# paninski-lab/lightning-pose

Hardware: AMD Instinct MI355X
Metric: training frames/sec (whole node), ResNet-50 384x384 17-kp semi-sup (higher is better)
Workload: dtype bf16; 1 GPU; C2/C3: ResNet-50 SemiSupervisedHeatmapTracker 384x384, K=17, 64 labeled + 128 unlabeled frames per GPU, heatmap_mse + temporal + pca_singleview + unimodal_mse, Adam (backbone lr=0 as at step 0), bf16-mixed; global_batch=192, parallelism=dp1, sync_batchnorm=False, decode_prune=plain kernels (chosen from the maps)

## Files before the change

include/lp_hip.h:

```cpp
#ifndef LP_HIP_H
#define LP_HIP_H

#include <stddef.h>
#include <stdint.h>

#ifdef __cplusplus
extern "C" {
#endif

typedef void* lp_stream_t;

int lp_config_reload_env(void);

enum {
    LP_OK = 0,
    LP_ERR_ARGUMENT = -1,
    LP_ERR_UNSUPPORTED = -2,
};

enum { LP_TF_NONE = 0, LP_TF_SINGLE = 1, LP_TF_PER_FRAME = 2, LP_TF_PER_VIEW = 3 };

#define LP_HIP_ABI_VERSION 148
int lp_version(void);
const char* lp_strerror(int code);


typedef struct lp_decode_tables {
    const int* row_base;
    const float* row_taps;
    const int* col_start;
    const float* col_taps;
    const int* colT_start;
    const float* colT_taps;
    int ty, tx, tc;
} lp_decode_tables;

typedef struct lp_frame_map {
    const float* transforms;
    int tf_mode;
    const float* bbox;
    int bbox_stride;
    int kp_per_view;
    float model_h, model_w;
} lp_frame_map;

int lp_decode_window(int downsample_factor, int n);


int lp_decode_fwd(const float* heat, int B, int K, int h, int w, int downsample_factor, float temperature,
                  const lp_decode_tables* tables, const lp_frame_map* frame_map, float* kp_aug, float* kp_frame, float* conf,
                  float* stats, int prune, lp_stream_t stream);

int lp_decode_bwd(const float* heat, int B, int K, int h, int w, int downsample_factor, float temperature,
                  const lp_decode_tables* tables, const lp_frame_map* frame_map, const float* stats, const float* g_kp_aug,
                  const float* g_kp_frame, float* g_heat, int accumulate, int prune, lp_stream_t stream);

int lp_frame_map_apply(const float* kp_in, int B, int K, const lp_frame_map* frame_map, int backward, float* kp_out,
                       lp_stream_t stream);


int lp_heatmap_gen(const float* keypoints, const int* visibility, int B, int K, int img_h, int img_w, int h, int w, float sigma,
                   float* out, lp_stream_t stream);
int lp_heatmap_gen_bwd(const float* keypoints, const int* visibility, int B, int K, int img_h, int img_w, int h, int w, float sigma,
                       const float* grad_out, float* grad_keypoints, lp_stream_t stream);

size_t lp_temporal_heatmap_workspace_bytes(int S, int K);
int lp_temporal_heatmap_fwd(int kind, const float* pred, const float* conf, int S, int K, int h, int w, const float* epsilon,
                            float prob_threshold, float* loss, void* workspace, lp_stream_t stream);
int lp_temporal_heatmap_bwd(int kind, const float* pred, int S, int K, int h, int w, const void* workspace, const float* gout,
                            float* gpred, int accumulate, lp_stream_t stream);

int lp_heatmap_confidence(const float* heat, const float* locs, int B, int K, int h, int w, int radius, float* out, lp_stream_t stream);

size_t lp_heatmap_mse_workspace_bytes(int B, int K);
int lp_heatmap_mse_fwd(const float* targ, const float* pred, int B, int K, int h, int w, float* loss, void* workspace,
                       lp_stream_t stream);
int lp_heatmap_mse_bwd(const float* targ, const float* pred, int B, int K, int h, int w, const void* workspace, const float* gout,
                       float* gpred, int accumulate, lp_stream_t stream);
enum { LP_HM_MSE = 0, LP_HM_KL = 1, LP_HM_JS = 2 };
int lp_heatmap_loss_fwd(int kind, const float* targ, const float* pred, int B, int K, int h, int w, float* loss, void* workspace,
                        lp_stream_t stream);
int lp_heatmap_loss_bwd(int kind, const float* targ, const float* pred, int B, int K, int h, int w, const void* workspace,
                        const float* gout, float* gpred, int accumulate, lp_stream_t stream);

int lp_unimodal_mse_fwd(const float* kp_aug, const float* pred, const float* conf, int S, int K, int img_h, int img_w, int h, int w,
                        float sigma, float prob_threshold, float* loss, void* workspace, lp_stream_t stream);
int lp_unimodal_mse_bwd(const float* kp_aug, const float* pred, int S, int K, int img_h, int img_w, int h, int w, float sigma,
                        const void* workspace, const float* gout, float* gpred, int accumulate, lp_stream_t stream);

int lp_softmax2d_fwd(const float* in, long stride_b, long stride_i, long stride_k, int B, int K, int n, float* out,
                     lp_stream_t stream);
int lp_softmax2d_bwd(const float* prob, const float* gprob, int B, int K, int n, void* gin_bf16, long stride_b, long stride_i,
                     long stride_k, lp_stream_t stream);


int lp_temporal_fwd_bwd(const float* kp, const float* conf, int S, int K, const float* eps_per_kp, float prob_threshold,
                        float* loss, float* grad_unit, lp_stream_t stream);

int lp_pca_fwd_bwd(const float* kp, int S, int K, const int* index, int rows, int points, const float* mean,
                   const float* kept_eigenvectors, int ncomp, float epsilon, float* loss, float* grad_unit, lp_stream_t stream);

int lp_rmse_fwd(const float* kp_targ, const float* kp_pred, int n_points, float* loss, lp_stream_t stream);
int lp_loss_combine(const float* const* x, const float* w, const float* a, int n, float* weighted, float* total, lp_stream_t stream);
int lp_loss_combine_bwd(const float* w, const float* a, int n, const float* g_weighted, const float* g_total, float* gx, lp_stream_t stream);

typedef struct lp_conv_geom {
    int B, Hi, Wi, Ci;
    int Ho, Wo, Co;
    int R, S, stride, pad;
} lp_conv_geom;

#define LP_CONV_KERNEL_IGEMM 0
#define LP_CONV_KERNEL_PIPE 1
#define LP_CONV_KERNEL_WGRAD 2
#define LP_CONV_KERNEL_WGRAD_PIPE 3
#define LP_CONV_KERNEL_PIPE_HALO 4
#define LP_CONV_KERNEL_STEM_WGRAD_NB 8
#define LP_CONV_KERNEL_WGRAD_NB 9
#define LP_CONV_KERNEL_RES2D 5
int lp_conv_last_kernel(void);

int lp_conv_fwd(const void* x, const void* w, const lp_conv_geom* geom, const float* bias, void* out_bf16, float* out_f32, int ldo,
                int n_store, lp_stream_t stream);
int lp_conv_dgrad(const void* dy, const void* wd, const lp_conv_geom* geom, const float* bias, const void* addend,
                  const void* relu_mask, void* dx_bf16, float* dx_f32, int ldo, int n_store, int skip_empty_classes,
                  lp_stream_t stream);
typedef struct lp_gemm_batch {
    int nb, nh;
    long long a_b, a_h, b_b, b_h, c_b, c_h;
} lp_gemm_batch;
int lp_gemm_nt(const void* a, int lda, const void* b, int ldb, void* c_bf16, float* c_f32, int ldc, int M, int N, int K, int n_store,
               const float* bias, const lp_gemm_batch* batch, lp_stream_t stream);
int lp_gemm_tn(const void* x, int ldx, const void* y, int ldy, void* out_bf16, int ldo, int M, int J, int N, const lp_gemm_batch* batch,
               lp_stream_t stream);
int lp_attn_fwd(const void* qkv_bf16, int ld_qkv, int k_off, int v_off, int B, int nh, int T, float scale, void* p_bf16, int ldp,
                void* out_bf16, int ldo, lp_stream_t stream);
int lp_attn_bwd_kv(const void* qkv_bf16, int ld_qkv, int v_off, const void* d_out_bf16, int ld_do, const void* p_bf16, int ldp, const float* d_rows,
                   int B, int nh, int T, float scale, void* ds_bf16, void* dqkv_bf16, int ld_dqkv, int dk_off, int dv_off, lp_stream_t stream);
int lp_attn_rowdot(const void* a_bf16, const void* b_bf16, int rows, int nh, int ld, float* out, lp_stream_t stream);
int lp_attn_dscores(const void* d_out, int ld_do, const void* v, int ldv, const void* p_bf16, const float* d_rows, int d_row_stride,
                    long long d_b, long long d_h, float scale, void* ds_bf16, int ldc, int M, int N, int K, const lp_gemm_batch* batch,
                    lp_stream_t stream);
typedef struct lp_fxsum {
    long long hi, lo;
} lp_fxsum;
int lp_gemm_nt_gelu_bwd(const void* a, const void* b, const void* u_bf16, void* c_bf16, int M, int N, int K, lp_fxsum* colsum,
                        lp_stream_t stream);
int lp_gemm_nt_gelu_fwd(const void* a, const void* b, const float* bias, void* c_bf16, void* act_bf16, int M, int N, int K,
                        lp_stream_t stream);
typedef struct lp_bn_fuse {
    const void* z;
    const float* mean;
    const float* invstd;
    const float* gamma;
    const float* beta;
    int mask_from_z;
    const void* relu_bits;
    lp_fxsum* sums;
    int seg_images;
    int addend_half;
} lp_bn_fuse;
int lp_conv_dgrad_bits(const void* dy, const void* wd, const lp_conv_geom* geom, const void* addend, const void* relu_bits, void* dx_bf16,
                       int skip_empty_classes, lp_stream_t stream);
int lp_bn_fold(const float* w, const float* gamma, const float* beta, const float* running_mean, const float* running_var, float eps,
               int Co, int per_co, void* w_bf16, float* bias, lp_stream_t stream);
int lp_conv_fwd_act(const void* x, const void* w, const lp_conv_geom* geom, const float* bias, const void* residual_bf16, int relu,
                    void* out_bf16, lp_stream_t stream);
int lp_conv_fwd_bn(const void* x, const void* w, const lp_conv_geom* geom, void* out_bf16, const lp_bn_fuse* bn, lp_stream_t stream);
int lp_stem_fwd_bn(const void* x4, const void* w, const lp_conv_geom* geom, void* out_bf16, const lp_bn_fuse* bn, lp_stream_t stream);
int lp_conv_dgrad_bn(const void* dy, const void* wd, const lp_conv_geom* geom, const void* addend, const void* relu_mask,
                     void* dx_bf16, const lp_bn_fuse* bn, lp_stream_t stream);
size_t lp_conv_wgrad_workspace_bytes(const lp_conv_geom* geom, int split_hint);
int lp_conv_wgrad(const void* x, const void* dy, const lp_conv_geom* geom, float* dw, int split_hint, void* workspace,
                  size_t workspace_bytes, lp_stream_t stream);
int lp_conv_wgrad_bias(const void* x, const void* dy, const lp_conv_geom* geom, float* dw, float* dbias, int split_hint, void* workspace,
                       size_t workspace_bytes, lp_stream_t stream);
int lp_stem_fwd(const void* x4, const void* w, const lp_conv_geom* geom, void* out_bf16, lp_stream_t stream);
int lp_stem_wgrad(const void* x4, const void* dy, const lp_conv_geom* geom, float* dw, int split_hint, void* workspace,
                  size_t workspace_bytes, lp_stream_t stream);

int lp_f32_conv_fwd(const float* x, const float* w, const lp_conv_geom* geom, int KH, int KW, int CiS, const float* bias,
                    const float* addend, float* out, lp_stream_t stream);
int lp_f32_conv_dgrad(const float* dy, const float* w, const lp_conv_geom* geom, int KH, int KW, int CiS, const float* bias,
                      const float* addend, float* dx, lp_stream_t stream);
int lp_f32_conv_wgrad(const float* x, const float* dy, const lp_conv_geom* geom, int KH, int KW, int CiS, float* dw, lp_stream_t stream);
int lp_f32_bn_stats(const float* x, int M, int C, float* sums, lp_stream_t stream);
size_t lp_f32_bn_stats_workspace_bytes(int M, int C);
int lp_f32_bn_stats_ordered(const float* x, int M, int C, float* sums, void* workspace, size_t workspace_bytes, lp_stream_t stream);
int lp_f32_bn_apply(const float* x, const float* mean, const float* invstd, const float* gamma, const float* beta, const float* residual,
                    int relu, int M, int C, float* y, lp_stream_t stream);
int lp_f32_bn_bwd_reduce(const float* dy, const float* y_out, const float* x, const float* mean, const float* invstd, int M, int C,
                         float* sums, float* dbeta_acc, float* dgamma_acc, lp_stream_t stream);
int lp_f32_bn_bwd_apply(const float* dy, const float* y_out, const float* x, const float* mean, const float* invstd, const float* gamma,
                        const float* sums, float count, int M, int C, float* dx, float* dres, lp_stream_t stream);
int lp_f32_maxpool_fwd(const float* x, int B, int Hi, int Wi, int C, float* y, void* argmax_u8, lp_stream_t stream);
int lp_f32_maxpool_bwd(const void* argmax_u8, const float* dy, int B, int Hi, int Wi, int C, float* dx, lp_stream_t stream);
int lp_f32_images_to_nhwc4(const float* images, int B, int H, int W, float* out, lp_stream_t stream);
int lp_f32_pixel_shuffle(const float* in, int B, int h, int w, int c_out, int ld, int inverse, float* out, lp_stream_t stream);
int lp_f32_softmax2d_bwd(const float* prob, const float* gprob, int B, int K, int n, float* gin, long stride_b, long stride_i, long stride_k,
                         lp_stream_t stream);
int lp_f32_vit_patchify(const float* images, int B, int H, int W, int patch, float* out, lp_stream_t stream);
int lp_f32_vit_tokens_fwd(const float* patch, const float* cls, const float* pos, int B, int Np, int D, float* x, lp_stream_t stream);
int lp_f32_vit_tokens_bwd(const float* dx, int B, int Np, int D, float* dpatch, float* dpos, lp_stream_t stream);
int lp_f32_vit_mv_tokens_fwd(const float* patch, const float* pos, const float* view, int B, int V, int Np, int D, float* x, lp_stream_t stream);
int lp_f32_vit_mv_tokens_bwd(const float* dx, int B, int V, int Np, int D, float* dpatch, float* dpos, float* dview, void* workspace,
                             size_t workspace_bytes, lp_stream_t stream);
int lp_f32_layernorm_fwd(const float* x, const float* delta, float* x_out, const float* gamma, const float* beta, float eps, int M, int D,
                         int drop_T, float* y, float* mean, float* rstd, lp_stream_t stream);
int lp_f32_layernorm_bwd(const float* dy, const float* x, const float* mean, const float* rstd, const float* gamma, int M, int D, int drop_T,
                         float* dx_acc, float* dgamma_acc, float* dbeta_acc, lp_stream_t stream);
int lp_f32_layernorm_ls_fwd(const float* x, const float* delta, const float* ls, float* x_out, const float* gamma, const float* beta, float eps,
                            int M, int D, int drop_T, float* y, float* mean, float* rstd, lp_stream_t stream);
int lp_f32_layernorm_ls_bwd(const float* dy, const float* x, const float* mean, const float* rstd, const float* gamma, const float* ls,
                            const float* branch, int M, int D, int drop_T, float* dx_acc, float* dx_out, float* dgamma_acc, float* dbeta_acc,
                            float* colsum_acc, float* dls_acc, lp_stream_t stream);
int lp_f32_gelu_fwd(const float* x, size_t n, float* y, lp_stream_t stream);
int lp_f32_gelu_bwd(const float* x, const float* dy, size_t n, float* dx, lp_stream_t stream);
int lp_f32_attn_fwd(const float* qkv, int ld, int k_off, int v_off, int B, int nh, int T, float scale, float* p, float* o, int ldo,
                    lp_stream_t stream);
int lp_f32_attn_bwd(const float* qkv, int ld, int k_off, int v_off, const float* dout, int ldo, const float* p, int B, int nh, int T,
                    float scale, float* ds_workspace, float* dqkv, int ldd, lp_stream_t stream);

size_t lp_bn_reduce_workspace_bytes(int M, int C);
int lp_bn_stats(const void* x, int M, int C, lp_fxsum* sums, void* workspace, size_t workspace_bytes, lp_stream_t stream);
int lp_fxsum_accumulate(const lp_fxsum* sums, int n, float* dst, lp_stream_t stream);
int lp_bn_finalize(const lp_fxsum* sums, float count, int C, float eps, float momentum, float* mean, float* invstd,
                   float* running_mean, float* running_var, lp_stream_t stream);
int lp_bn_finalize_f32(const float* sums, float count, int C, float eps, float momentum, float* mean, float* invstd,
                       float* running_mean, float* running_var, lp_stream_t stream);
int lp_bn_finalize2(const lp_fxsum* sums, float count0, float count1, int C, float eps, float momentum, float* mean, float* invstd,
                    float* running_mean, float* running_var, lp_stream_t stream);
int lp_bn_apply(const void* x, const float* mean, const float* invstd, const float* gamma, const float* beta, const void* residual,
                int relu, int M, int C, void* y, void* relu_bits, lp_stream_t stream);
int lp_bn_apply_seg(const void* x, const float* mean, const float* invstd, const float* gamma, const float* beta, const void* residual,
                    int relu, int M, int C, int seg_rows, void* y, void* relu_bits, lp_stream_t stream);
int lp_bn_apply_seg_lo(const void* x, const float* mean, const float* invstd, const float* gamma, const float* beta, const void* residual,
                       const void* residual_lo, const void* zd, const float* mean_d, const float* invstd_d, const float* gamma_d,
                       const float* beta_d, int relu, int M, int C, int seg_rows, void* y, void* y_lo, void* relu_bits, lp_stream_t stream);
int lp_bn_apply_seg_rbn(const void* x, const float* mean, const float* invstd, const float* gamma, const float* beta, const void* zd,
                        const float* mean_d, const float* invstd_d, const float* gamma_d, const float* beta_d, int relu, int M, int C,
                        int seg_rows, void* y, void* relu_bits, lp_stream_t stream);
int lp_bn_bwd_reduce(const void* dy, const void* y_out, const void* x, const float* mean, const float* invstd, int M, int C,
                     lp_fxsum* sums, void* workspace, size_t workspace_bytes, lp_stream_t stream);
int lp_bn_bwd_apply(const void* dy, const void* y_out, const void* x, const float* mean, const float* invstd, const float* gamma,
                    const lp_fxsum* sums, float count, int M, int C, void* dx, void* dres, const lp_fxsum* sums_local, float* dbeta_acc,
                    float* dgamma_acc, float* terms_ws, lp_stream_t stream);
int lp_bn_bwd_apply_seg(const void* dy, const void* y_out, const void* x, const float* mean, const float* invstd, const float* gamma,
                        const lp_fxsum* sums, float count0, float count1, int M, int C, int seg_rows, void* dx, void* dres,
                        const lp_fxsum* sums_local, float* dbeta_acc, float* dgamma_acc, float* terms_ws, lp_stream_t stream);
size_t lp_bn_bwd_ds_workspace_bytes(int M, int C);
int lp_bn_bwd_apply_seg_ds(const void* dy, const void* y_out, const void* x, const float* mean, const float* invstd, const float* gamma,
                           const lp_fxsum* sums, float count0, float count1, int M, int C, int seg_rows, void* dx, void* dres,
                           const lp_fxsum* sums_local, float* dbeta_acc, float* dgamma_acc, float* terms_ws, const void* zd,
                           const float* mean_d, const float* invstd_d, lp_fxsum* sums_d, void* workspace, size_t workspace_bytes,
                           lp_stream_t stream);
int lp_maxpool_fwd(const void* x, int B, int Hi, int Wi, int C, void* y, void* argmax_u8, lp_stream_t stream);
int lp_maxpool_bwd(const void* argmax_u8, const void* dy, int B, int Hi, int Wi, int C, void* dx, lp_stream_t stream);
int lp_bn_relu_maxpool_fwd(const void* z, const float* mean, const float* invstd, const float* gamma, const float* beta, int B, int Hi, int Wi,
                           int C, void* y, void* argmax_u8, lp_stream_t stream);
int lp_bn_pool_bwd_reduce(const void* argmax_u8, const void* dy, const void* z, const float* mean, const float* invstd, const float* gamma,
                          const float* beta, int B, int Hi, int Wi, int C, lp_fxsum* sums, lp_stream_t stream);
int lp_bn_pool_bwd_apply(const void* argmax_u8, const void* dy, const void* z, const float* mean, const float* invstd, const float* gamma,
                         const float* beta, const lp_fxsum* sums, float count, int B, int Hi, int Wi, int C, void* dx,
                         const lp_fxsum* sums_local, float* dbeta_acc, float* dgamma_acc, lp_stream_t stream);
int lp_images_to_nhwc4(const float* images_nchw, int B, int H, int W, void* out_bf16, lp_stream_t stream);
int lp_pixel_shuffle(const void* in, int B, int h, int w, int c_out, int ld, int inverse, void* out, lp_stream_t stream);

int lp_vit_patchify(const float* images_nchw, int B, int H, int W, int patch, void* out_bf16, lp_stream_t stream);
int lp_vit_tokens_fwd(const void* patch_bf16, const float* cls, const float* pos, int B, int Np, int D, float* x, lp_stream_t stream);
int lp_vit_tokens_bwd(const float* dx, int B, int Np, int D, void* dpatch_bf16, float* dpos, lp_stream_t stream);
int lp_vit_mv_tokens_fwd(const void* patch_bf16, const float* pos, const float* view, int B, int V, int Np, int D, float* x,
                         lp_stream_t stream);
size_t lp_vit_mv_tokens_bwd_workspace_bytes(int B, int V, int Np, int D);
int lp_vit_mv_tokens_bwd(const float* dx, int B, int V, int Np, int D, void* dpatch_bf16, float* dpos, float* dview, void* workspace,
                         size_t workspace_bytes, lp_stream_t stream);
#define LP_CAM_MAX_VIEWS 32
size_t lp_cam_chain_workspace_bytes(int B, int V, int K);
int lp_cam_chain_fwd(const float* points, const float* intrinsics, const float* extrinsics, const float* dist12, const float* bbox, float model_h,
                     float model_w, int B, int V, int K, float* p3d, float* p2d, lp_stream_t stream);
int lp_cam_chain_bwd(const float* points, const float* intrinsics, const float* extrinsics, const float* dist12, const float* bbox, float model_h,
                     float model_w, int B, int V, int K, const float* p3d, const float* g3d, const float* g2d, void* workspace,
                     size_t workspace_bytes, float* gpoints, lp_stream_t stream);
int lp_cam_project_fwd(const float* points_3d, const float* intrinsics, const float* extrinsics, const float* dist12, const float* bbox,
                       float model_h, float model_w, int B, int V, int K, float* p2d, lp_stream_t stream);
int lp_cam_project_bwd(const float* points_3d, const float* intrinsics, const float* extrinsics, const float* dist12, const float* bbox,
                       float model_h, float model_w, int B, int V, int K, const float* g2d, float* g3d, lp_stream_t stream);
int lp_cam_pairwise_fwd_bwd(const float* targ_3d, const float* pred_3d, int B, int P, int K, float* loss, float* grad_unit, lp_stream_t stream);
int lp_small_matmul(const float* w, const float* x, int R, int Q, int D, int transpose_w, int accumulate, float* y, lp_stream_t stream);
int lp_layernorm_fwd(const float* x, const void* delta_bf16, float* x_out, const float* gamma, const float* beta, float eps, int M,
                     int D, int drop_T, void* y_bf16, float* mean, float* rstd, lp_stream_t stream);
int lp_layernorm_bwd(const void* dy_bf16, const float* x, const float* mean, const float* rstd, const float* gamma, int M, int D,
                     int drop_T, float* dx_acc, float* dgamma_acc, float* dbeta_acc, lp_stream_t stream);
int lp_layernorm_bwd_bf16(const void* dy_bf16, const float* x, const float* mean, const float* rstd, const float* gamma, int M, int D,
                          int drop_T, float* dx_acc, void* dx_bf16, float* dgamma_acc, float* dbeta_acc, lp_stream_t stream);
int lp_gelu_fwd(const void* x_bf16, size_t n, void* y_bf16, lp_stream_t stream);
int lp_gelu_bwd(const void* x_bf16, const void* dy_bf16, size_t n, void* dx_bf16, lp_stream_t stream);
int lp_gelu_bwd_colsum(const void* x_bf16, const void* dy_bf16, int rows, int cols, void* dx_bf16, float* colsum_acc, lp_stream_t stream);
int lp_layernorm_bwd_bf16_colsum(const void* dy_bf16, const float* x, const float* mean, const float* rstd, const float* gamma, int M, int D,
                                 int drop_T, float* dx_acc, void* dx_bf16, float* dgamma_acc, float* dbeta_acc, float* colsum_acc,
                                 lp_stream_t stream);
int lp_layernorm_ls_fwd(const float* x, const void* delta_bf16, const float* ls, float* x_out, const float* gamma, const float* beta, float eps,
                        int M, int D, int drop_T, void* y_bf16, float* mean, float* rstd, lp_stream_t stream);
int lp_layernorm_ls_bwd(const void* dy_bf16, const float* x, const float* mean, const float* rstd, const float* gamma, const float* ls,
                        const void* branch_bf16, int M, int D, int drop_T, float* dx_acc, void* dx_bf16, float* dgamma_acc, float* dbeta_acc,
                        float* colsum_acc, float* dls_acc, lp_stream_t stream);
int lp_softmax_rows_fwd(void* s_bf16, int rows, int n, int ld, float scale, lp_stream_t stream);
int lp_softmax_rows_bwd(const void* p_bf16, void* dp_bf16, int rows, int n, int ld, float scale, lp_stream_t stream);
int lp_transpose_batched(const void* in_bf16, int R, int Cc, int ldi, long long in_b, long long in_h, void* out_bf16, int ldo,
                         long long out_b, long long out_h, int nb, int nh, lp_stream_t stream);

enum { LP_BORDER_RENORM = 0,
       LP_BORDER_CLAMP = 1    };

typedef struct lp_frame_norm {
    float mean[3], std[3];
} lp_frame_norm;

typedef struct lp_frame_augment {
    int has_matrix;
    float matrix[6];
    float brightness, contrast, contrast_center;
    float shot_factor;
    unsigned long long seed;
} lp_frame_augment;

int lp_frames_resize(const void* src_u8, int S, int Hs, int Ws, long long frame_stride, int row_stride, int H, int W, int border,
                     const lp_frame_norm* finish_norm, float* dst, lp_stream_t stream);
int lp_frames_resize_cubic(const void* src_u8, int S, int Hs, int Ws, long long frame_stride, int row_stride, int H, int W, int round_u8,
                           const lp_frame_norm* finish_norm, float* dst, lp_stream_t stream);
int lp_frames_augment(const float* src_hwc, int S, int H, int W, const lp_frame_augment* aug, const lp_frame_norm* norm,
                      float* dst_nchw, lp_stream_t stream);
int lp_labeled_keypoints(const float* kp_src, const float* src_hw, const float* affine, const int* hflip, const int* swap,
                         const int* vis_in, int uniform_heatmaps, int B, int K, int H, int W, float* kp_out, int* vis_out,
                         lp_stream_t stream);

enum { LP_AUG_GEOM = 1, LP_AUG_BLUR = 2, LP_AUG_DROPOUT = 4, LP_AUG_DROP_PER_CHANNEL = 8, LP_AUG_SALT = 16, LP_AUG_PEPPER = 32,
       LP_AUG_ELASTIC = 64, LP_AUG_HISTEQ = 128, LP_AUG_CLAHE = 256, LP_AUG_EMBOSS = 512, LP_AUG_CROPPAD = 1024, LP_AUG_HFLIP = 2048 };
enum { LP_AUG_OP_DROPOUT = 0, LP_AUG_OP_SALT = 1, LP_AUG_OP_PEPPER = 2, LP_AUG_OP_ELASTIC = 3 };
enum { LP_AUG_LOCAL_BLUR_COARSE = 0, LP_AUG_LOCAL_EMBOSS = 1 };
#define LP_AUG_ELASTIC_MAX_RADIUS 20

typedef struct lp_labelaug_image {
    int flags;
    int image_id;
    float geom[6];
    float blur[25];
    float emboss[9];
    int coarse_gh[3], coarse_gw[3];
    unsigned coarse_thr[3];
    float elastic_alpha;
    int clahe_clip, clahe_tiles_y, clahe_tiles_x, clahe_slot;
    int pad[4];
} lp_labelaug_image;

int lp_labelaug_geom(const void* src_u8, int B, int H, int W, const lp_labelaug_image* params, void* dst_u8, lp_stream_t stream);
int lp_labelaug_local(const void* src_u8, int B, int H, int W, const lp_labelaug_image* params, int which, const void* salt_lut,
                      unsigned long long seed, void* dst_u8, lp_stream_t stream);
int lp_labelaug_elastic_field(int B, int H, int W, const lp_labelaug_image* params, float sigma, unsigned long long seed, float* tmp,
                              float* field, lp_stream_t stream);
int lp_labelaug_elastic_apply(const void* src_u8, int B, int H, int W, const lp_labelaug_image* params, const float* field, void* dst_u8,
                              lp_stream_t stream);
int lp_labelaug_histeq(const void* src_u8, int B, int H, int W, const lp_labelaug_image* params, unsigned* ws, void* lut_out, void* dst_u8,
                       lp_stream_t stream);
int lp_labelaug_clahe(const void* src_u8, int B, int H, int W, const lp_labelaug_image* params, const int* slot_image, int n_slots,
                      int max_ty, int max_tx, void* luts, void* dst_u8, lp_stream_t stream);
int lp_labelaug_finish(const void* src_u8, int B, int Hs, int Ws, const lp_labelaug_image* params, int H, int W, const lp_frame_norm* norm,
                       float* dst, lp_stream_t stream);
int lp_labelaug_keypoints(const float* kp, int B, int K, const float* affine, const lp_labelaug_image* params, const float* field, int H,
                          int W, float* kp_out, lp_stream_t stream);

int lp_patch_mask_f32(const float* images, int BV, int C, int H, int W, int patch, int count, unsigned long long key, const float* mask_in,
                      float* out, float* mask_out, lp_stream_t stream);

#define LP_MV3D_MAX_VIEWS 8
#define LP_MV3D_MAX_KEYPOINTS 128
int lp_mv3d_plan(const float* kp, const float* src_hw, const float* bbox, const float* intrinsics, const float* extrinsics,
                 const float* dist12, const float* draws, int augment, float shift_param, int H, int W, int B, int V, int K, float* kp3d,
                 float* kp2d, float* affine, int* status, lp_stream_t stream);
int lp_mv3d_fill(const void* src_u8, int B, int Hs, int Ws, const lp_frame_norm* norm, float* fill, lp_stream_t stream);
int lp_mv3d_finish(const void* src_u8, int B, int Hs, int Ws, const float* affine, const float* fill, const lp_frame_norm* norm, int V,
                   int v, int H, int W, float* dst, lp_stream_t stream);

int lp_adam_step(float* params, const float* grads, float* exp_avg, float* exp_avg_sq, size_t n, float lr, float beta1, float beta2,
                 float eps, float weight_decay, int decoupled, int step, float grad_scale, void* params_bf16, lp_stream_t stream);
int lp_cast_bf16(const float* src, size_t n, void* dst, lp_stream_t stream);
int lp_permute_cba(const void* src, int A, int B, int C, void* dst, lp_stream_t stream);

#ifdef __cplusplus
}
#endif
#endif
```

lightning-pose_amd/_lib.py:

```python

from __future__ import annotations

import ctypes as C
import os

_HERE = os.path.dirname(os.path.abspath(__file__))
LIB_PATH = os.environ.get("LP_HIP_LIB") or os.path.join(_HERE, "liblp_hip.so")


class LpHipUnavailable(RuntimeError):
    """liblp_hip.so could not be loaded, or an op was given a non-ROCm tensor.  There is no fallback path."""


class LpHipError(RuntimeError):
    pass


class DecodeTables(C.Structure):
    _fields_ = [("row_base", C.c_void_p), ("row_taps", C.c_void_p), ("col_start", C.c_void_p),
                ("col_taps", C.c_void_p), ("colT_start", C.c_void_p), ("colT_taps", C.c_void_p),
                ("ty", C.c_int), ("tx", C.c_int), ("tc", C.c_int)]


class FrameMap(C.Structure):
    _fields_ = [("transforms", C.c_void_p), ("tf_mode", C.c_int), ("bbox", C.c_void_p), ("bbox_stride", C.c_int),
                ("kp_per_view", C.c_int), ("model_h", C.c_float), ("model_w", C.c_float)]


class ConvGeom(C.Structure):
    _fields_ = [(n, C.c_int) for n in ("B", "Hi", "Wi", "Ci", "Ho", "Wo", "Co", "R", "S", "stride", "pad")]


class BnFuse(C.Structure):
    _fields_ = [("z", C.c_void_p), ("mean", C.c_void_p), ("invstd", C.c_void_p), ("gamma", C.c_void_p), ("beta", C.c_void_p),
                ("mask_from_z", C.c_int), ("relu_bits", C.c_void_p), ("sums", C.c_void_p), ("seg_images", C.c_int), ("addend_half", C.c_int)]


class FrameNorm(C.Structure):
    _fields_ = [("mean", C.c_float * 3), ("std", C.c_float * 3)]


class FrameAugment(C.Structure):
    _fields_ = [("has_matrix", C.c_int), ("matrix", C.c_float * 6), ("brightness", C.c_float), ("contrast", C.c_float),
                ("contrast_center", C.c_float), ("shot_factor", C.c_float), ("seed", C.c_ulonglong)]


class GemmBatch(C.Structure):
    _fields_ = [("nb", C.c_int), ("nh", C.c_int)] + [(n, C.c_longlong) for n in ("a_b", "a_h", "b_b", "b_h", "c_b", "c_h")]


HM_MSE, HM_KL, HM_JS = 0, 1, 2
(CONV_KERNEL_IGEMM, CONV_KERNEL_PIPE, CONV_KERNEL_WGRAD, CONV_KERNEL_WGRAD_PIPE, CONV_KERNEL_PIPE_HALO, CONV_KERNEL_RES2D, _CONV_KERNEL_6,
 _CONV_KERNEL_7, CONV_KERNEL_STEM_WGRAD_NB, CONV_KERNEL_WGRAD_NB) = range(10)
CONV_KERNEL_LABEL = {
    CONV_KERNEL_PIPE: (("conv_igemm_kernel", "conv_pipe_kernel"),),
    CONV_KERNEL_PIPE_HALO: (("conv_igemm_kernel", "conv_pipe_kernel"), (">", ",halo>")),
    CONV_KERNEL_RES2D: (("conv_igemm_kernel<64,", "conv_res2d_kernel<"), ("conv_igemm_kernel<64>", "conv_res2d_kernel<fwd>")),
    CONV_KERNEL_WGRAD_PIPE: (("conv_wgrad_kernel", "conv_wgrad_pipe_kernel"),),
    CONV_KERNEL_WGRAD_NB: (("conv_wgrad_kernel", "conv_wgrad_nb_kernel"),),
}
BORDER_RENORM, BORDER_CLAMP = 0, 1
AUG_GEOM, AUG_BLUR, AUG_DROPOUT, AUG_DROP_PER_CHANNEL, AUG_SALT, AUG_PEPPER = 1, 2, 4, 8, 16, 32
AUG_ELASTIC, AUG_HISTEQ, AUG_CLAHE, AUG_EMBOSS, AUG_CROPPAD, AUG_HFLIP = 64, 128, 256, 512, 1024, 2048
AUG_OP_DROPOUT, AUG_OP_SALT, AUG_OP_PEPPER, AUG_OP_ELASTIC = 0, 1, 2, 3
AUG_LOCAL_BLUR_COARSE, AUG_LOCAL_EMBOSS = 0, 1
AUG_ELASTIC_MAX_RADIUS = 20
TF_NONE, TF_SINGLE, TF_PER_FRAME, TF_PER_VIEW = 0, 1, 2, 3

ABI_VERSION = 148

_P, _I, _F, _L, _Z = C.c_void_p, C.c_int, C.c_float, C.c_long, C.c_size_t

PROTOTYPES = {
    "lp_version": (_I, []),
    "lp_strerror": (C.c_char_p, [_I]),
    "lp_config_reload_env": (_I, []),
    "lp_decode_window": (_I, [_I, _I]),
    "lp_decode_fwd": (_I, [_P, _I, _I, _I, _I, _I, _F, C.POINTER(DecodeTables), C.POINTER(FrameMap), _P, _P, _P, _P, _I, _P]),
    "lp_decode_bwd": (_I, [_P, _I, _I, _I, _I, _I, _F, C.POINTER(DecodeTables), C.POINTER(FrameMap), _P, _P, _P, _P, _I, _I, _P]),
    "lp_frame_map_apply": (_I, [_P, _I, _I, C.POINTER(FrameMap), _I, _P, _P]),
    "lp_heatmap_gen": (_I, [_P, _P, _I, _I, _I, _I, _I, _I, _F, _P, _P]),
    "lp_heatmap_gen_bwd": (_I, [_P, _P, _I, _I, _I, _I, _I, _I, _F, _P, _P, _P]),
    "lp_temporal_heatmap_workspace_bytes": (_Z, [_I, _I]),
    "lp_temporal_heatmap_fwd": (_I, [_I, _P, _P, _I, _I, _I, _I, _P, _F, _P, _P, _P]),
    "lp_temporal_heatmap_bwd": (_I, [_I, _P, _I, _I, _I, _I, _P, _P, _P, _I, _P]),
    "lp_heatmap_confidence": (_I, [_P, _P, _I, _I, _I, _I, _I, _P, _P]),
    "lp_heatmap_mse_workspace_bytes": (_Z, [_I, _I]),
    "lp_heatmap_mse_fwd": (_I, [_P, _P, _I, _I, _I, _I, _P, _P, _P]),
    "lp_heatmap_mse_bwd": (_I, [_P, _P, _I, _I, _I, _I, _P, _P, _P, _I, _P]),
    "lp_heatmap_loss_fwd": (_I, [_I, _P, _P, _I, _I, _I, _I, _P, _P, _P]),
    "lp_heatmap_loss_bwd": (_I, [_I, _P, _P, _I, _I, _I, _I, _P, _P, _P, _I, _P]),
    "lp_unimodal_mse_fwd": (_I, [_P, _P, _P, _I, _I, _I, _I, _I, _I, _F, _F, _P, _P, _P]),
    "lp_unimodal_mse_bwd": (_I, [_P, _P, _I, _I, _I, _I, _I, _I, _F, _P, _P, _P, _I, _P]),
    "lp_softmax2d_fwd": (_I, [_P, _L, _L, _L, _I, _I, _I, _P, _P]),
    "lp_softmax2d_bwd": (_I, [_P, _P, _I, _I, _I, _P, _L, _L, _L, _P]),
    "lp_temporal_fwd_bwd": (_I, [_P, _P, _I, _I, _P, _F, _P, _P, _P]),
    "lp_pca_fwd_bwd": (_I, [_P, _I, _I, _P, _I, _I, _P, _P, _I, _F, _P, _P, _P]),
    "lp_rmse_fwd": (_I, [_P, _P, _I, _P, _P]),
    "lp_loss_combine": (_I, [_P, _P, _P, _I, _P, _P, _P]),
    "lp_loss_combine_bwd": (_I, [_P, _P, _I, _P, _P, _P, _P]),
    "lp_conv_fwd": (_I, [_P, _P, C.POINTER(ConvGeom), _P, _P, _P, _I, _I, _P]),
    "lp_conv_dgrad": (_I, [_P, _P, C.POINTER(ConvGeom), _P, _P, _P, _P, _P, _I, _I, _I, _P]),
    "lp_conv_dgrad_bits": (_I, [_P, _P, C.POINTER(ConvGeom), _P, _P, _P, _I, _P]),
    "lp_gemm_nt": (_I, [_P, _I, _P, _I, _P, _P, _I, _I, _I, _I, _I, _P, C.POINTER(GemmBatch), _P]),
    "lp_gemm_nt_gelu_bwd": (_I, [_P, _P, _P, _P, _I, _I, _I, _P, _P]),
    "lp_gemm_nt_gelu_fwd": (_I, [_P, _P, _P, _P, _P, _I, _I, _I, _P]),
    "lp_gemm_tn": (_I, [_P, _I, _P, _I, _P, _I, _I, _I, _I, C.POINTER(GemmBatch), _P]),
    "lp_attn_fwd": (_I, [_P, _I, _I, _I, _I, _I, _I, C.c_float, _P, _I, _P, _I, _P]),
    "lp_attn_bwd_kv": (_I, [_P, _I, _I, _P, _I, _P, _I, _P, _I, _I, _I, C.c_float, _P, _P, _I, _I, _I, _P]),
    "lp_attn_rowdot": (_I, [_P, _P, _I, _I, _I, _P, _P]),
    "lp_attn_dscores": (_I, [_P, _I, _P, _I, _P, _P, _I, C.c_longlong, C.c_longlong, C.c_float, _P, _I, _I, _I, _I, C.POINTER(GemmBatch), _P]),
    "lp_conv_fwd_bn": (_I, [_P, _P, C.POINTER(ConvGeom), _P, C.POINTER(BnFuse), _P]),
    "lp_conv_last_kernel": (_I, []),
    "lp_stem_fwd_bn": (_I, [_P, _P, C.POINTER(ConvGeom), _P, C.POINTER(BnFuse), _P]),
    "lp_conv_dgrad_bn": (_I, [_P, _P, C.POINTER(ConvGeom), _P, _P, _P, C.POINTER(BnFuse), _P]),
    "lp_bn_fold": (_I, [_P, _P, _P, _P, _P, _F, _I, _I, _P, _P, _P]),
    "lp_conv_fwd_act": (_I, [_P, _P, C.POINTER(ConvGeom), _P, _P, _I, _P, _P]),
    "lp_conv_wgrad_workspace_bytes": (_Z, [C.POINTER(ConvGeom), _I]),
    "lp_conv_wgrad": (_I, [_P, _P, C.POINTER(ConvGeom), _P, _I, _P, _Z, _P]),
    "lp_conv_wgrad_bias": (_I, [_P, _P, C.POINTER(ConvGeom), _P, _P, _I, _P, C.c_size_t, _P]),
    "lp_stem_fwd": (_I, [_P, _P, C.POINTER(ConvGeom), _P, _P]),
    "lp_stem_wgrad": (_I, [_P, _P, C.POINTER(ConvGeom), _P, _I, _P, _Z, _P]),
    "lp_bn_reduce_workspace_bytes": (_Z, [_I, _I]),
    "lp_bn_stats": (_I, [_P, _I, _I, _P, _P, _Z, _P]),
    "lp_bn_finalize": (_I, [_P, _F, _I, _F, _F, _P, _P, _P, _P, _P]),
    "lp_fxsum_accumulate": (_I, [_P, _I, _P, _P]),
    "lp_bn_finalize_f32": (_I, [_P, _F, _I, _F, _F, _P, _P, _P, _P, _P]),
    "lp_bn_finalize2": (_I, [_P, _F, _F, _I, _F, _F, _P, _P, _P, _P, _P]),
    "lp_bn_apply": (_I, [_P, _P, _P, _P, _P, _P, _I, _I, _I, _P, _P, _P]),
    "lp_bn_apply_seg": (_I, [_P, _P, _P, _P, _P, _P, _I, _I, _I, _I, _P, _P, _P]),
    "lp_bn_apply_seg_lo": (_I, [_P, _P, _P, _P, _P, _P, _P, _P, _P, _P, _P, _P, _I, _I, _I, _I, _P, _P, _P, _P]),
    "lp_bn_apply_seg_rbn": (_I, [_P, _P, _P, _P, _P, _P, _P, _P, _P, _P, _I, _I, _I, _I, _P, _P, _P]),
    "lp_bn_bwd_apply_seg": (_I, [_P, _P, _P, _P, _P, _P, _P, _F, _F, _I, _I, _I, _P, _P, _P, _P, _P, _P, _P]),
    "lp_bn_bwd_ds_workspace_bytes": (_Z, [_I, _I]),
    "lp_bn_bwd_apply_seg_ds": (_I, [_P, _P, _P, _P, _P, _P, _P, _F, _F, _I, _I, _I, _P, _P, _P, _P, _P, _P, _P, _P, _P, _P, _P, _Z, _P]),
    "lp_bn_bwd_reduce": (_I, [_P, _P, _P, _P, _P, _I, _I, _P, _P, _Z, _P]),
    "lp_bn_bwd_apply": (_I, [_P, _P, _P, _P, _P, _P, _P, _F, _I, _I, _P, _P, _P, _P, _P, _P, _P]),
    "lp_maxpool_fwd": (_I, [_P, _I, _I, _I, _I, _P, _P, _P]),
    "lp_maxpool_bwd": (_I, [_P, _P, _I, _I, _I, _I, _P, _P]),
    "lp_bn_relu_maxpool_fwd": (_I, [_P, _P, _P, _P, _P, _I, _I, _I, _I, _P, _P, _P]),
    "lp_bn_pool_bwd_reduce": (_I, [_P, _P, _P, _P, _P, _P, _P, _I, _I, _I, _I, _P, _P]),
    "lp_bn_pool_bwd_apply": (_I, [_P, _P, _P, _P, _P, _P, _P, _P, C.c_float, _I, _I, _I, _I, _P, _P, _P, _P, _P]),
    "lp_images_to_nhwc4": (_I, [_P, _I, _I, _I, _P, _P]),
    "lp_pixel_shuffle": (_I, [_P, _I, _I, _I, _I, _I, _I, _P, _P]),
    "lp_vit_patchify": (_I, [_P, _I, _I, _I, _I, _P, _P]),
    "lp_vit_tokens_fwd": (_I, [_P, _P, _P, _I, _I, _I, _P, _P]),
    "lp_vit_tokens_bwd": (_I, [_P, _I, _I, _I, _P, _P, _P]),
    "lp_vit_mv_tokens_fwd": (_I, [_P, _P, _P, _I, _I, _I, _I, _P, _P]),
    "lp_vit_mv_tokens_bwd_workspace_bytes": (_Z, [_I, _I, _I, _I]),
    "lp_vit_mv_tokens_bwd": (_I, [_P, _I, _I, _I, _I, _P, _P, _P, _P, _Z, _P]),
    "lp_cam_chain_workspace_bytes": (_Z, [_I, _I, _I]),
    "lp_cam_chain_fwd": (_I, [_P, _P, _P, _P, _P, _F, _F, _I, _I, _I, _P, _P, _P]),
    "lp_cam_chain_bwd": (_I, [_P, _P, _P, _P, _P, _F, _F, _I, _I, _I, _P, _P, _P, _P, _Z, _P, _P]),
    "lp_cam_project_fwd": (_I, [_P, _P, _P, _P, _P, _F, _F, _I, _I, _I, _P, _P]),
    "lp_cam_project_bwd": (_I, [_P, _P, _P, _P, _P, _F, _F, _I, _I, _I, _P, _P, _P]),
    "lp_cam_pairwise_fwd_bwd": (_I, [_P, _P, _I, _I, _I, _P, _P, _P]),
    "lp_small_matmul": (_I, [_P, _P, _I, _I, _I, _I, _I, _P, _P]),
    "lp_layernorm_fwd": (_I, [_P, _P, _P, _P, _P, _F, _I, _I, _I, _P, _P, _P, _P]),
    "lp_layernorm_bwd": (_I, [_P, _P, _P, _P, _P, _I, _I, _I, _P, _P, _P, _P]),
    "lp_layernorm_bwd_bf16": (_I, [_P, _P, _P, _P, _P, _I, _I, _I, _P, _P, _P, _P, _P]),
    "lp_gelu_fwd": (_I, [_P, _Z, _P, _P]),
    "lp_gelu_bwd": (_I, [_P, _P, _Z, _P, _P]),
    "lp_gelu_bwd_colsum": (_I, [_P, _P, _I, _I, _P, _P, _P]),
    "lp_layernorm_bwd_bf16_colsum": (_I, [_P, _P, _P, _P, _P, _I, _I, _I, _P, _P, _P, _P, _P, _P]),
    "lp_layernorm_ls_fwd": (_I, [_P, _P, _P, _P, _P, _P, _F, _I, _I, _I, _P, _P, _P, _P]),
    "lp_layernorm_ls_bwd": (_I, [_P, _P, _P, _P, _P, _P, _P, _I, _I, _I, _P, _P, _P, _P, _P, _P, _P]),
    "lp_softmax_rows_fwd": (_I, [_P, _I, _I, _I, _F, _P]),
    "lp_softmax_rows_bwd": (_I, [_P, _P, _I, _I, _I, _F, _P]),
    "lp_transpose_batched": (_I, [_P, _I, _I, _I, C.c_longlong, C.c_longlong, _P, _I, C.c_longlong, C.c_longlong, _I, _I, _P]),
    "lp_frames_resize": (_I, [_P, _I, _I, _I, C.c_longlong, _I, _I, _I, _I, C.POINTER(FrameNorm), _P, _P]),
    "lp_frames_resize_cubic": (_I, [_P, _I, _I, _I, C.c_longlong, _I, _I, _I, _I, C.POINTER(FrameNorm), _P, _P]),
    "lp_frames_augment": (_I, [_P, _I, _I, _I, C.POINTER(FrameAugment), C.POINTER(FrameNorm), _P, _P]),
    "lp_labeled_keypoints": (_I, [_P, _P, _P, _P, _P, _P, _I, _I, _I, _I, _I, _P, _P, _P]),
    "lp_labelaug_geom": (_I, [_P, _I, _I, _I, _P, _P, _P]),
    "lp_labelaug_local": (_I, [_P, _I, _I, _I, _P, _I, _P, C.c_ulonglong, _P, _P]),
    "lp_labelaug_elastic_field": (_I, [_I, _I, _I, _P, _F, C.c_ulonglong, _P, _P, _P]),
    "lp_labelaug_elastic_apply": (_I, [_P, _I, _I, _I, _P, _P, _P, _P]),
    "lp_labelaug_histeq": (_I, [_P, _I, _I, _I, _P, _P, _P, _P, _P]),
    "lp_labelaug_clahe": (_I, [_P, _I, _I, _I, _P, _P, _I, _I, _I, _P, _P, _P]),
    "lp_labelaug_finish": (_I, [_P, _I, _I, _I, _P, _I, _I, C.POINTER(FrameNorm), _P, _P]),
    "lp_labelaug_keypoints": (_I, [_P, _I, _I, _P, _P, _P, _I, _I, _P, _P]),
    "lp_patch_mask_f32": (_I, [_P, _I, _I, _I, _I, _I, _I, C.c_ulonglong, _P, _P, _P, _P]),
    "lp_mv3d_plan": (_I, [_P, _P, _P, _P, _P, _P, _P, _I, _F, _I, _I, _I, _I, _I, _P, _P, _P, _P, _P]),
    "lp_mv3d_fill": (_I, [_P, _I, _I, _I, C.POINTER(FrameNorm), _P, _P]),
    "lp_mv3d_finish": (_I, [_P, _I, _I, _I, _P, _P, C.POINTER(FrameNorm), _I, _I, _I, _I, _P, _P]),
    "lp_f32_conv_fwd": (_I, [_P, _P, C.POINTER(ConvGeom), _I, _I, _I, _P, _P, _P, _P]),
    "lp_f32_conv_dgrad": (_I, [_P, _P, C.POINTER(ConvGeom), _I, _I, _I, _P, _P, _P, _P]),
    "lp_f32_conv_wgrad": (_I, [_P, _P, C.POINTER(ConvGeom), _I, _I, _I, _P, _P]),
    "lp_f32_bn_stats": (_I, [_P, _I, _I, _P, _P]),
    "lp_f32_bn_stats_workspace_bytes": (C.c_size_t, [_I, _I]),
    "lp_f32_bn_stats_ordered": (_I, [_P, _I, _I, _P, _P, C.c_size_t, _P]),
    "lp_f32_bn_apply": (_I, [_P, _P, _P, _P, _P, _P, _I, _I, _I, _P, _P]),
    "lp_f32_bn_bwd_reduce": (_I, [_P, _P, _P, _P, _P, _I, _I, _P, _P, _P, _P]),
    "lp_f32_bn_bwd_apply": (_I, [_P, _P, _P, _P, _P, _P, _P, _F, _I, _I, _P, _P, _P]),
    "lp_f32_maxpool_fwd": (_I, [_P, _I, _I, _I, _I, _P, _P, _P]),
    "lp_f32_maxpool_bwd": (_I, [_P, _P, _I, _I, _I, _I, _P, _P]),
    "lp_f32_images_to_nhwc4": (_I, [_P, _I, _I, _I, _P, _P]),
    "lp_f32_pixel_shuffle": (_I, [_P, _I, _I, _I, _I, _I, _I, _P, _P]),
    "lp_f32_softmax2d_bwd": (_I, [_P, _P, _I, _I, _I, _P, _L, _L, _L, _P]),
    "lp_f32_vit_patchify": (_I, [_P, _I, _I, _I, _I, _P, _P]),
    "lp_f32_vit_tokens_fwd": (_I, [_P, _P, _P, _I, _I, _I, _P, _P]),
    "lp_f32_vit_tokens_bwd": (_I, [_P, _I, _I, _I, _P, _P, _P]),
    "lp_f32_vit_mv_tokens_fwd": (_I, [_P, _P, _P, _I, _I, _I, _I, _P, _P]),
    "lp_f32_vit_mv_tokens_bwd": (_I, [_P, _I, _I, _I, _I, _P, _P, _P, _P, _Z, _P]),
    "lp_f32_layernorm_fwd": (_I, [_P, _P, _P, _P, _P, _F, _I, _I, _I, _P, _P, _P, _P]),
    "lp_f32_layernorm_bwd": (_I, [_P, _P, _P, _P, _P, _I, _I, _I, _P, _P, _P, _P]),
    "lp_f32_layernorm_ls_fwd": (_I, [_P, _P, _P, _P, _P, _P, _F, _I, _I, _I, _P, _P, _P, _P]),
    "lp_f32_layernorm_ls_bwd": (_I, [_P, _P, _P, _P, _P, _P, _P, _I, _I, _I, _P, _P, _P, _P, _P, _P, _P]),
    "lp_f32_gelu_fwd": (_I, [_P, _Z, _P, _P]),
    "lp_f32_gelu_bwd": (_I, [_P, _P, _Z, _P, _P]),
    "lp_f32_attn_fwd": (_I, [_P, _I, _I, _I, _I, _I, _I, _F, _P, _P, _I, _P]),
    "lp_f32_attn_bwd": (_I, [_P, _I, _I, _I, _P, _I, _P, _I, _I, _I, _F, _P, _P, _I, _P]),
    "lp_adam_step": (_I, [_P, _P, _P, _P, _Z, _F, _F, _F, _F, _F, _I, _I, _F, _P, _P]),
    "lp_cast_bf16": (_I, [_P, _Z, _P, _P]),
    "lp_permute_cba": (_I, [_P, _I, _I, _I, _P, _P]),
}


def declare(lib: C.CDLL) -> C.CDLL:
    for name, (res, args) in PROTOTYPES.items():
        fn = getattr(lib, name)
        fn.restype = res
        fn.argtypes = args
    have = int(lib.lp_version())
    if have != ABI_VERSION:
        raise LpHipUnavailable(f"{getattr(lib, '_name', 'liblp_hip.so')} was built for ABI {have}, this package binds ABI {ABI_VERSION} "
                               "(include/lp_hip.h: LP_HIP_ABI_VERSION) - rebuild it: python -c 'import __graft_entry__ as g; g.build()'")
    return lib


_lib = None


def lib() -> C.CDLL:
    global _lib
    if _lib is None:
        if not os.path.exists(LIB_PATH):
            raise LpHipUnavailable(
                f"{LIB_PATH} not found - build it with `python -c 'import __graft_entry__ as g; g.build()'` "
                "(lightning-pose_amd/csrc/build.sh).  lightning_pose_amd has no CPU fallback.")
        try:
            _lib = declare(C.CDLL(LIB_PATH))
        except OSError as e:
            raise LpHipUnavailable(f"cannot load {LIB_PATH}: {e}") from e
    return _lib


def check(code: int, what: str) -> None:
    if code == 0:
        return
    msg = lib().lp_strerror(code).decode()
    if code == -1:
        raise ValueError(f"{what}: {msg}")
    if code == -2:
        raise NotImplementedError(f"{what}: {msg}")
    raise LpHipError(f"{what}: HIP error {code}: {msg}")
```

lightning-pose_amd/csrc/api.hip:

```cpp
#include "lp_common.h"

#include <stdlib.h>

#include <atomic>

extern "C" int lp_version(void) { return LP_HIP_ABI_VERSION; }

namespace lp {
static int env_int(const char* name, int dflt) {
    const char* e = getenv(name);
    return (e == nullptr || *e == 0) ? dflt : atoi(e);
}
static LpSwitches read_switches() {
    LpSwitches s;
    s.conv_pipe = env_int("LP_CONV_PIPE", 1);
    s.conv_halo = env_int("LP_CONV_HALO", 1);
    s.conv_res2d = env_int("LP_CONV_RES2D", 1);
    s.infer_pipe = env_int("LP_INFER_PIPE", 1);
    s.gemm_pipe = env_int("LP_GEMM_PIPE", 1);
    s.wgrad_pipe = env_int("LP_WGRAD_PIPE", 1);
    s.wgrad_nb = env_int("LP_WGRAD_NB", 1);
    s.stem_2d = env_int("LP_STEM_2D", 1);
    s.stem_wgrad_nb = env_int("LP_STEM_WGRAD_NB", 1);
    s.pool_v2 = env_int("LP_POOL_V2", 1);
    s.bn_bwd_wgs_per_cu = env_int("LP_BN_BWD_WGS_PER_CU", 5);
    if (s.bn_bwd_wgs_per_cu < 1 || s.bn_bwd_wgs_per_cu > 5) s.bn_bwd_wgs_per_cu = 5;
    s.conv_max_wgs = env_int("LP_CONV_MAX_WGS", 0);
    return s;
}
static std::atomic<const LpSwitches*> g_switches{new LpSwitches(read_switches())};
const LpSwitches& lp_switches() { return *g_switches.load(std::memory_order_acquire); }
}

extern "C" int lp_config_reload_env(void) {
    lp::g_switches.store(new lp::LpSwitches(lp::read_switches()), std::memory_order_release);
    return LP_OK;
}

extern "C" const char* lp_strerror(int code) {
    if (code == LP_OK) return "ok";
    if (code == LP_ERR_ARGUMENT) return "invalid argument (null pointer or non-positive dimension)";
    if (code == LP_ERR_UNSUPPORTED) return "shape not covered by the instantiated kernels";
    if (code > 0) return hipGetErrorString((hipError_t)code);
    return "unknown lp_hip error";
}
```

lightning-pose_amd/csrc/conv.hip:

```cpp
#include <stdlib.h>

#include "lp_common.h"

namespace lp {

constexpr int kBM = 128;
constexpr int kBK = 64;
constexpr int kLD = kBK + 8;

struct ConvGeom {
    int B, Hi, Wi, Ci;
    int Ho, Wo, Co;
    int R, S, stride, pad;
};

struct ConvEpilogue {
    unsigned short* out_bf16;
    float* out_f32;
    int ldo;
    int n_store;
    const float* bias;
    const unsigned short* addend;
    const unsigned short* relu_mask;
    const unsigned char* relu_bits;
// ... 620 lines not shown
    unsigned voffA = ~0u, voffB[RB];
    if (fast) {
        const int p0 = m_begin + pgA * 4;
        const int pc = p0 < M ? p0 : 0;
        const int rem = pc - fdiv(pc, div_hw) * hw;
        fho = fdiv(rem, div_wo);
        fwo = rem - fho * g.Wo;
        if (jv) voffA = (unsigned)((p0 + (tr - g.pad) * g.Wi + (ts - g.pad)) * pitch_x + tcn) * 2u + zx;
        lo_h = max(0, g.pad - tr);
        span_h = min(g.Ho, g.Hi + g.pad - tr) - lo_h;
        lo_w = max(0, g.pad - ts);
        span_w = min(g.Wo, g.Wi + g.pad - ts) - lo_w;
#pragma unroll
        for (int i = 0; i < RB; ++i) voffB[i] = nv ? (unsigned)((m_begin + pgB * RB + i) * pitch_y + nB) * 2u + zy : ~0u;
    }
    const unsigned jinv = jv ? 0u : ~0u;

    auto load_fast = [&](auto nm_c, int mk, u16x8 (&ra)[4], u16x8 (&rb)[RB]) {
        constexpr bool NM = decltype(nm_c)::value;
        const unsigned step = (unsigned)(mk - m_begin);
        const unsigned soffA = step * ci2, soffB = step * (unsigned)pitch_y * 2u;
        if (NM) {
            const bool ragged = mk + kBK > m_end;
#pragma unroll
            for (int i = 0; i < 4; ++i) {
                const unsigned rinv = (ragged && mk + pgA * 4 + i >= m_end) ? ~0u : 0u;
                ra[i] = buf_load16(rsrc_x, (voffA + i * ci2) | jinv | rinv, soffA);
            }
#pragma unroll
            for (int i = 0; i < RB; ++i) {
                const unsigned rinv = (ragged && mk + pgB * RB + i >= m_end) ? ~0u : 0u;
                rb[i] = buf_load16(rsrc_dy, voffB[i] | rinv, soffB);
            }
        } else {
#pragma unroll
            for (int i = 0; i < 4; ++i) {
                int wo = fwo + i, ho = fho;
                if (wo >= g.Wo) {
                    wo -= g.Wo;
                    ho = (ho + 1 == g.Ho) ? 0 : ho + 1;
                }
                const bool ok = (unsigned)(ho - lo_h) < (unsigned)span_h && (unsigned)(wo - lo_w) < (unsigned)span_w;
                ra[i] = buf_load16(rsrc_x, (voffA + soffA + i * ci2) | (ok ? 0u : ~0u) | jinv, 0u);
            }
            fwo += rw;
            fho += qw;
            if (fwo >= g.Wo) {
                fwo -= g.Wo;
                ++fho;
            }
            if (fho >= g.Ho) fho -= g.Ho;
            if (fho >= g.Ho) fho -= g.Ho;
#pragma unroll
            for (int i = 0; i < RB; ++i) rb[i] = buf_load16(rsrc_dy, voffB[i], soffB);
        }
    };

    auto load_generic = [&](int mk, u16x8 (&ra)[4], u16x8 (&rb)[RB]) {
#pragma unroll
        for (int i = 0; i < 4; ++i) {
            const int m = mk + pgA * 4 + i;
            bool ok = jv && m < m_end;
            const int mm = ok ? m : 0;
            const int b = fdiv(mm, div_hw), rem = mm - b * hw;
            const int ho = fdiv(rem, div_wo), wo = rem - ho * g.Wo;
            const int hi = ho * g.stride - g.pad + tr, wi = wo * g.stride - g.pad + ts;
            if (STEM) {
                const bool okr = ok && tr < g.R && hi >= 0 && hi < g.Hi;
                const size_t base = ((size_t)(b * g.Hi + hi) * g.Wi + wi) * 4;
                ra[i] = load4x2(X + base, okr && wi >= 0 && wi < g.Wi, X + base + 4, okr && ts + 1 < g.S && wi + 1 >= 0 && wi + 1 < g.Wi);
            } else {
                ok = ok && hi >= 0 && hi < g.Hi && wi >= 0 && wi < g.Wi;
                ra[i] = ok ? load8(X + ((size_t)(b * g.Hi + hi) * g.Wi + wi) * g.Ci + tcn) : zero8();
            }
        }
#pragma unroll
        for (int i = 0; i < RB; ++i) {
            const int m = mk + pgB * RB + i;
            rb[i] = (nv && m < m_end) ? load8(DY + (size_t)m * g.Co + nB) : zero8();
        }
    };
    auto load_step = [&](int mk) {
        if (fast && (direct || mk + kBK <= m_end)) {
            if (nomask) load_fast(std::true_type{}, mk, ra, rb);
            else load_fast(std::false_type{}, mk, ra, rb);
        } else load_generic(mk, ra, rb);
    };
    auto store_step = [&](int buf, const u16x8 (&ra)[4], const u16x8 (&rb)[RB]) {
#pragma unroll
        for (int i = 0; i < 4; ++i) *reinterpret_cast<u16x8*>(&sA[buf][(pgA * 4 + i) * LDA + jc * 8]) = ra[i];
#pragma unroll
        for (int i = 0; i < RB; ++i) *reinterpret_cast<u16x8*>(&sB[buf][(pgB * RB + i) * LDB + nc * 8]) = rb[i];
        if (want_cs) {
#pragma unroll
            for (int i = 0; i < RB; ++i)
#pragma unroll
                for (int q = 0; q < 8; ++q) cs[q] += bf16_to_f32(rb[i][q]);
        }
    };

    const int fq = lane >> 4, fi = lane & 15;
    const int frow = (fq >> 1) * 8 + (fi >> 2), fcol = (fq & 1) * 16 + (fi & 3) * 4;
    auto frag = [&](const unsigned short* tile_, int ld, int ch0, int kk) -> bf16x8 {
        const unsigned short* p = tile_ + (kk * 16 + frow) * ld + ch0 + fcol;
        const s16x4_t lo = lds_read_tr16(p), hi = lds_read_tr16(p + 4 * ld);
        typedef __attribute__((ext_vector_type(8))) short s16x8_t;
        const s16x8_t v = {lo[0], lo[1], lo[2], lo[3], hi[0], hi[1], hi[2], hi[3]};
        return __builtin_bit_cast(bf16x8, v);
    };
    auto mma_step = [&](int buf) {
        bf16x8 a[2][2], b[2][NT];
        auto fetch = [&](int kk, int set) {
#pragma unroll
            for (int mt = 0; mt < 2; ++mt) a[set][mt] = frag(sA[buf], LDA, wm * 64 + mt * 32, kk);
#pragma unroll
            for (int nt = 0; nt < NT; ++nt) b[set][nt] = frag(sB[buf], LDB, wn * (NT * 32) + nt * 32, kk);
        };
        fetch(0, 0);
#pragma unroll
        for (int kk = 0; kk < kBK / 16; ++kk) {
            if (kk + 1 < kBK / 16) fetch(kk + 1, (kk + 1) & 1);
            __builtin_amdgcn_sched_barrier(0);
#pragma unroll
            for (int mt = 0; mt < 2; ++mt)
#pragma unroll
                for (int nt = 0; nt < NT; ++nt)
                    acc[mt][nt] = __builtin_amdgcn_mfma_f32_32x32x16_bf16(a[kk & 1][mt], b[kk & 1][nt], acc[mt][nt], 0, 0, 0);
            __builtin_amdgcn_sched_barrier(0);
        }
    };

    const int KT = (m_end - m_begin + kBK - 1) / kBK;
    const bool deep = kWgradDeep && fast && KT >= 2 && (direct || (m_end - m_begin) % kBK == 0);
    auto deep_loop = [&](auto nm) {
        load_fast(nm, m_begin, ra, rb);
        load_fast(nm, m_begin + kBK, ra2, rb2);
        store_step(0, ra, rb);
        __syncthreads();
        int kt = 0;
        for (; kt + 3 < KT; kt += 2) {
            load_fast(nm, m_begin + (kt + 2) * kBK, ra, rb);
            mma_step(0);
            store_step(1, ra2, rb2);
            __syncthreads();
            load_fast(nm, m_begin + (kt + 3) * kBK, ra2, rb2);
            mma_step(1);
            store_step(0, ra, rb);
            __syncthreads();
        }
        const bool three = kt + 2 < KT;
        if (three) load_fast(nm, m_begin + (kt + 2) * kBK, ra, rb);
        mma_step(0);
        store_step(1, ra2, rb2);
        __syncthreads();
        mma_step(1);
        if (three) {
            store_step(0, ra, rb);
            __syncthreads();
            mma_step(0);
        }
        __syncthreads();
    };
    if (deep) {
        if (nomask) deep_loop(std::true_type{});
        else deep_loop(std::false_type{});
    } else if (KT > 0) {
        load_step(m_begin);
        store_step(0, ra, rb);
        __syncthreads();
        for (int kt = 0; kt < KT; ++kt) {
            const int cur = kt & 1;
            if (kt + 1 < KT) load_step(m_begin + (kt + 1) * kBK);
            mma_step(cur);
            if (kt + 1 < KT) store_step(cur ^ 1, ra, rb);
            __syncthreads();
        }
    }

    if (want_cs) {
        float* red = reinterpret_cast<float*>(&sA[0][0]);
#pragma unroll
        for (int q = 0; q < 8; ++q) red[pgB * BN + nc * 8 + q] = cs[q];
        __syncthreads();
        if (tid < BN && n0 + tid < g.Co) {
            float t = 0.f;
            for (int r = 0; r < 256 / NCH; ++r) t += red[r * BN + tid];
            atomicAdd(&tn.col_sums[n0 + tid], t);
        }
    }
    if (direct) {
        const int col = lane & 31, rg = lane >> 5;
#pragma unroll
        for (int mt = 0; mt < 2; ++mt)
#pragma unroll
            for (int nt = 0; nt < NT; ++nt) {
                const int n = n0 + wn * (NT * 32) + nt * 32 + col;
#pragma unroll
                for (int e = 0; e < 16; ++e) {
                    const int jr = j0 + wm * 64 + mt * 32 + (e & 3) + 8 * (e >> 2) + 4 * rg;
                    if (jr < Kw && n < g.Co) tn.out[zo + (size_t)jr * tn.ldo + n] = f32_to_bf16(acc[mt][nt][e]);
                }
            }
        return;
    }
    float* dst = ws + ((((size_t)slice * tiles + tile) * 4 + wave) * (2 * NT * 16)) * 64 + lane;
#pragma unroll
    for (int mt = 0; mt < 2; ++mt)
#pragma unroll
        for (int nt = 0; nt < NT; ++nt)
#pragma unroll
            for (int e = 0; e < 16; ++e) dst[((mt * NT + nt) * 16 + e) * 64] = acc[mt][nt][e];
}

template <int BN>
__global__ __launch_bounds__(256) void wgrad_reduce_kernel(const float* __restrict__ ws, int slices, int tiles, int tiles_n, int Kw,
                                                           int Co, float* __restrict__ dW) {
    constexpr int NT = BN / 64;
    constexpr int PER_TILE = 4 * 2 * NT * 16 * 64;
    const size_t total = (size_t)tiles * PER_TILE;
    for (size_t i = (size_t)blockIdx.x * 256 + threadIdx.x; i < total; i += (size_t)gridDim.x * 256) {
        float sum = 0.f;
        for (int sl = 0; sl < slices; ++sl) sum += ws[(size_t)sl * total + i];
        const int lane = (int)(i & 63);
        size_t t = i >> 6;
        const int e = (int)(t & 15);
        t >>= 4;
        const int nt = (int)(t % NT);
        t /= NT;
        const int mt = (int)(t & 1);
        t >>= 1;
        const int wave = (int)(t & 3);
        const int tile = (int)(t >> 2);
        const int wm = wave >> 1, wn = wave & 1;
        const int j = (tile / tiles_n) * kBM + wm * 64 + mt * 32 + (e & 3) + 8 * (e >> 2) + 4 * (lane >> 5);
        const int n = (tile % tiles_n) * BN + wn * (NT * 32) + nt * 32 + (lane & 31);
        if (j < Kw && n < Co) dW[(size_t)n * Kw + j] += sum;
    }
}

template <int BN>
__global__ __launch_bounds__(256) void wgrad_reduce_sliced_kernel(const float* __restrict__ ws, int slices, int tiles, int tiles_n,
                                                                  int Kw, int Co, float* __restrict__ dW) {
    constexpr int NT = BN / 64;
    constexpr int PER_TILE = 4 * 2 * NT * 16 * 64;
    __shared__ float part[4][64];
    const size_t total = (size_t)tiles * PER_TILE;
    const int lane = threadIdx.x & 63, w = threadIdx.x >> 6;
    const size_t i = (size_t)blockIdx.x * 64 + lane;
    float s0 = 0.f, s1 = 0.f, s2 = 0.f, s3 = 0.f;
    int sl = w;
    for (; sl + 12 < slices; sl += 16) {
        s0 += ws[(size_t)sl * total + i];
        s1 += ws[(size_t)(sl + 4) * total + i];
        s2 += ws[(size_t)(sl + 8) * total + i];
        s3 += ws[(size_t)(sl + 12) * total + i];
    }
    for (; sl < slices; sl += 4) s0 += ws[(size_t)sl * total + i];
    part[w][lane] = (s0 + s1) + (s2 + s3);
    __syncthreads();
    if (w == 0) {
        const float sum = (part[0][lane] + part[1][lane]) + (part[2][lane] + part[3][lane]);
        size_t t = i >> 6;
        const int e = (int)(t & 15);
        t >>= 4;
        const int nt = (int)(t % NT);
        t /= NT;
        const int mt = (int)(t & 1);
        t >>= 1;
        const int wave = (int)(t & 3);
        const int tile = (int)(t >> 2);
        const int wm = wave >> 1, wn = wave & 1;
        const int j = (tile / tiles_n) * kBM + wm * 64 + mt * 32 + (e & 3) + 8 * (e >> 2) + 4 * (lane >> 5);
        const int n = (tile % tiles_n) * BN + wn * (NT * 32) + nt * 32 + (lane & 31);
        if (j < Kw && n < Co) dW[(size_t)n * Kw + j] += sum;
    }
}

template <int BN>
static void launch_wgrad_reduce(const float* ws, int slices, int tiles, int tiles_n, int Kw, int Co, float* dw, hipStream_t st) {
    constexpr int PER_TILE = 4 * 2 * (BN / 64) * 16 * 64;
    if (slices >= 16) {
        hipLaunchKernelGGL((wgrad_reduce_sliced_kernel<BN>), dim3(tiles * (PER_TILE / 64)), dim3(256), 0, st, ws, slices, tiles, tiles_n, Kw,
                           Co, dw);
    } else {
        const int blocks = tiles * (PER_TILE / 256);
        hipLaunchKernelGGL((wgrad_reduce_kernel<BN>), dim3(blocks < 4096 ? blocks : 4096), dim3(256), 0, st, ws, slices, tiles, tiles_n, Kw,
                           Co, dw);
    }
}

static long long seg_split_rows(int seg_images, int B, long long rows_per_image, long long M) {
    if (seg_images <= 0) return M;
    if (seg_images >= B) return -1;
    const long long r = (long long)seg_images * rows_per_image;
    return (r % kBM == 0) ? r : -1;
}

static void bn_fuse_begin(ConvEpilogue& ep, const lp_bn_fuse* bn) {
    ep.stats_sums = bn->sums;
    ep.seg_images = bn->seg_images;
}

static thread_local int g_last_conv_kernel = LP_CONV_KERNEL_IGEMM;

struct ConvRoute {
    int kernel;
    int bn;
    int mode;
    int ek;
};
constexpr int kNoKernel = -1;

struct ConvProblem {
    int mode;
    int ek;
    const void *x, *w;
    ConvGeom g;
    Lattice lat;
    int M, N, K;
    long long seg_rows;
    ConvEpilogue ep;
    int LpSwitches::*gate;
    bool dense;
    bool igemm_form;
    int igemm_cols;
    bool gemm;
    GemmExt gx;
    int nz;
    unsigned x_bytes, w_bytes;
};

static int conv_ck(const ConvProblem& p) { return p.mode == kModeDgrad ? p.g.Co : p.g.Ci; }

static bool pipe_shape_ok(const ConvEpilogue& ep, int M, int N, int K, int ck, long long seg_rows, bool bias_ok) {
    if (ep.out_bf16 == nullptr || ep.out_f32 != nullptr || (ep.bias != nullptr && !bias_ok) || ep.ldo != N || ep.n_store != N) return false;
    if (K <= 0 || ck % kBK != 0 || N % (N > 64 ? 128 : 64) != 0 || M <= 0) return false;
    if (ep.seg_images > 0 && seg_rows % kPM != 0) return false;
    return true;
}

static int pipe_dgrad_kind(const ConvEpilogue& ep) {
    if (ep.bn_z != nullptr) {
        if (ep.stats_sums == nullptr || ep.relu_mask != nullptr) return -1;
        if (ep.mask_from_z && !ep.addend && !ep.relu_bits) return kEkZ;
        if (!ep.mask_from_z && ep.addend && ep.relu_bits) return kEkAZB;
        return -1;
    }
    if (ep.stats_sums != nullptr) return -1;
    if (ep.relu_bits != nullptr) return ep.relu_mask == nullptr ? kEkPB : -1;
    return kEkPlain;
}

static bool halo_shape_ok(const ConvGeom& g, int M, int ck, int cap_rows) {
    if (g.R != 3 || g.S != 3 || g.stride != 1 || g.pad != 1 || g.Hi != g.Ho || g.Wi != g.Wo || ck % kBK != 0) return false;
    struct Memo { int B, H, W, cap; bool ok; };
    static thread_local Memo memo[8];
    static thread_local int memo_n = 0;
    for (int i = 0; i < memo_n; ++i)
        if (memo[i].B == g.B && memo[i].H == g.Hi && memo[i].W == g.Wi && memo[i].cap == cap_rows) return memo[i].ok;
    const long long W = g.Wi, H = g.Hi, Wp = W + 2;
    auto padded = [&](long long m) {
        const long long r = m / W, b = r / H;
        return (r + 1 + 2 * b) * Wp + (m - r * W) + 1;
    };
    bool ok = true;
    for (long long m0 = 0; m0 < M && ok; m0 += kPM) {
        const long long last = m0 + kPM - 1 < M ? m0 + kPM - 1 : M - 1;
        ok = padded(last) - padded(m0) + 2 * (W + 3) + 1 <= cap_rows;
    }
    if (memo_n < 8) memo[memo_n++] = Memo{g.B, g.Hi, g.Wi, cap_rows, ok};
    return ok;
}

static bool res2d_shape_ok(const ConvGeom& g, int ck, int N) {
    return g.R == 3 && g.S == 3 && g.stride == 1 && g.pad == 1 && g.Hi == g.Ho && g.Wi == g.Wo && ck == 64 && N == 64 && g.Hi % 16 == 0 &&
           g.Wi % 16 == 0;
}

static bool stem2d_shape_ok(const ConvGeom& g) { return g.Ho % 16 == 0 && g.Wo % 16 == 0 && g.Hi == 2 * g.Ho && g.Wi == 2 * g.Wo; }

static bool admits_pipe(const ConvProblem& p) {
    if (p.ek < 0 || !p.dense) return false;
    if (p.ek == kEkAZB && !(p.lat.hstep == 1 && p.lat.wstep == 1)) return false;
    if ((p.ek == kEkGeluFwd || p.ek == kEkGeluBwd) && p.N % 128 != 0) return false;
    return pipe_shape_ok(p.ep, p.M, p.N, p.K, conv_ck(p), p.seg_rows, p.mode != kModeDgrad);
}

static bool admits_halo(const ConvProblem& p) {
    return (p.ek == kEkNone || p.ek == kEkInfer || p.ek == kEkZ) && halo_shape_ok(p.g, p.M, conv_ck(p), p.N > 64 ? 384 : 512);
}

static bool admits_res2d(const ConvProblem& p) {
    if (!res2d_shape_ok(p.g, conv_ck(p), p.N)) return false;
    if (p.mode == kModeInfer) return p.ep.addend == nullptr;
    return (p.ek == kEkNone || p.ek == kEkZ) && p.ep.bias == nullptr && admits_pipe(p);
}

static ConvRoute route_conv(const ConvProblem& p, const LpSwitches& sw) {
    const bool pipe = sw.conv_pipe != 0 && (p.gate == nullptr || sw.*p.gate != 0);
    if (p.mode == kModeStem) return ConvRoute{pipe && stem2d_shape_ok(p.g) ? LP_CONV_KERNEL_RES2D : LP_CONV_KERNEL_IGEMM, 64, p.mode, p.ek};
    if (pipe && sw.conv_res2d != 0 && admits_res2d(p)) return ConvRoute{LP_CONV_KERNEL_RES2D, 64, p.mode, p.ek};
    if (pipe && admits_pipe(p))
        return ConvRoute{sw.conv_halo != 0 && admits_halo(p) ? LP_CONV_KERNEL_PIPE_HALO : LP_CONV_KERNEL_PIPE, p.N > 64 ? 128 : 64, p.mode, p.ek};
    return ConvRoute{p.igemm_form ? LP_CONV_KERNEL_IGEMM : kNoKernel, p.igemm_cols > 64 ? 128 : 64, p.mode, p.ek};
}

static int conv_max_wgs(int per_cu) {
    if (lp_switches().conv_max_wgs > 0) return lp_switches().conv_max_wgs;
    static int cus = [] {
        int dev = 0, c = 0;
        if (hipGetDevice(&dev) != hipSuccess || hipDeviceGetAttribute(&c, hipDeviceAttributeMultiprocessorCount, dev) != hipSuccess || c <= 0) c = 256;
        return c;
    }();
    return per_cu * cus;
}

template <int BN, int MODE>
static void launch_igemm(const ConvProblem& p, hipStream_t st) {
    const ConvGeom& g = p.g;
    const int tm = (p.M + kBM - 1) / kBM, tn = (p.N + BN - 1) / BN, per_z = tm * tn, ntiles = per_z * p.nz;
    const int grid = ntiles < conv_max_wgs(2) ? ntiles : conv_max_wgs(2);
    const int ck = MODE == kModeDgrad ? g.Co : g.Ci;
    unsigned x_bytes = (unsigned)(2ull * (MODE == kModeDgrad ? (size_t)g.B * g.Ho * g.Wo * g.Co : (size_t)g.B * g.Hi * g.Wi * g.Ci));
    unsigned w_bytes = (unsigned)(2ull * (size_t)p.N * (MODE == kModeStem ? (size_t)p.K : (size_t)g.R * g.S * ck));
    GemmExt gx{ck, MODE == kModeStem ? p.K : g.R * g.S * ck, 1, per_z, 0u, 0u, 0u, 0u, 0u, 0u};
    if (p.gemm) {
        gx = p.gx;
        gx.tiles_per_z = per_z;
        x_bytes = p.x_bytes;
        w_bytes = p.w_bytes;
    }
    hipLaunchKernelGGL((conv_igemm_kernel<BN, MODE>), dim3(grid), dim3(256), 0, st, (const unsigned short*)p.x, (const unsigned short*)p.w,
                       x_bytes, w_bytes, g, p.lat, gx, make_fastdiv(p.lat.nh * p.lat.nw), make_fastdiv(p.lat.nw), p.M, p.N, p.K, tn, ntiles, p.ep);
}

template <int MODE, bool INFER = false>
static void launch_res2d(const ConvProblem& p, hipStream_t st) {
    const ConvGeom& g = p.g;
    const int ntiles = g.B * (g.Hi / 16) * (g.Wi / 16);
    const int grid = ntiles < conv_max_wgs(1) ? ntiles : conv_max_wgs(1);
    const unsigned x_bytes = (unsigned)(2ull * g.B * g.Hi * g.Wi * 64), w_bytes = (unsigned)(2ull * 64 * 9 * 64);
    hipLaunchKernelGGL((conv_res2d_kernel<MODE, INFER>), dim3(grid), dim3(512), 0, st, (const unsigned short*)p.x, (const unsigned short*)p.w, x_bytes,
                       w_bytes, g.B, g.Hi, g.Wi, ntiles, p.ep);
}

static void launch_stem2d(const ConvProblem& p, hipStream_t st) {
    const ConvGeom& g = p.g;
    const int ntiles = g.B * (g.Ho / 16) * (g.Wo / 16);
    const int grid = ntiles < 2 * conv_max_wgs(1) ? ntiles : 2 * conv_max_wgs(1);
    hipLaunchKernelGGL(conv_stem2d_kernel, dim3(grid), dim3(512), 0, st, (const unsigned short*)p.x, (const unsigned short*)p.w,
                       (unsigned)(2ull * g.B * g.Hi * g.Wi * 4), g.B, g.Ho, g.Wo, ntiles, p.ep);
}

template <int BN, int MODE, int EK, bool HALO = false>
static void launch_pipe(const ConvProblem& p, hipStream_t st) {
    const ConvGeom& g = p.g;
    const int tm = (p.M + kPM - 1) / kPM, tn = p.N / BN, ntiles = tm * tn;
    const int grid = ntiles < conv_max_wgs(1) ? ntiles : conv_max_wgs(1);
    const int ck = MODE == kModeDgrad ? g.Co : g.Ci;
    const unsigned x_bytes = (unsigned)(2ull * (MODE == kModeDgrad ? (size_t)g.B * g.Ho * g.Wo * g.Co : (size_t)g.B * g.Hi * g.Wi * g.Ci));
    const unsigned w_bytes = (unsigned)(2ull * (size_t)p.N * g.R * g.S * ck);
    const HaloDivs hd{make_fastdiv(g.Hi), make_fastdiv(g.Wi + 2), make_fastdiv(g.Hi + 2)};
    hipLaunchKernelGGL((conv_pipe_kernel<BN, MODE, EK, HALO>), dim3(grid), dim3(512), 0, st, (const unsigned short*)p.x, (const unsigned short*)p.w,
                       x_bytes, w_bytes, g, p.lat, make_fastdiv(p.lat.nh * p.lat.nw), make_fastdiv(p.lat.nw), p.M, p.N, p.K, tn, ntiles, p.ep, hd);
}

template <int BN>
static void launch_conv_bn(const ConvRoute& r, const ConvProblem& p, hipStream_t st) {
    if (r.kernel == LP_CONV_KERNEL_IGEMM) {
        switch (r.mode) {
            case kModeFwd: return launch_igemm<BN, kModeFwd>(p, st);
            case kModeDgrad: return launch_igemm<BN, kModeDgrad>(p, st);
            case kModeInfer: return launch_igemm<BN, kModeInfer>(p, st);
            default: return launch_igemm<BN, kModeAttn>(p, st);
        }
    }
    const bool halo = r.kernel == LP_CONV_KERNEL_PIPE_HALO;
    switch (r.ek) {
        case kEkNone: return halo ? launch_pipe<BN, kModeFwd, kEkNone, true>(p, st) : launch_pipe<BN, kModeFwd, kEkNone>(p, st);
        case kEkInfer: return halo ? launch_pipe<BN, kModeFwd, kEkInfer, true>(p, st) : launch_pipe<BN, kModeFwd, kEkInfer>(p, st);
        case kEkZ: return halo ? launch_pipe<BN, kModeDgrad, kEkZ, true>(p, st) : launch_pipe<BN, kModeDgrad, kEkZ>(p, st);
        case kEkAZB: return launch_pipe<BN, kModeDgrad, kEkAZB>(p, st);
        case kEkPB: return launch_pipe<BN, kModeDgrad, kEkPB>(p, st);
        default: return launch_pipe<BN, kModeDgrad, kEkPlain>(p, st);
    }
}

static void launch_conv(const ConvRoute& r, const ConvProblem& p, hipStream_t st) {
    g_last_conv_kernel = r.kernel;
    if (r.kernel == LP_CONV_KERNEL_RES2D) {
        switch (r.mode) {
            case kModeStem: return launch_stem2d(p, st);
            case kModeInfer: return launch_res2d<kModeFwd, true>(p, st);
            case kModeDgrad: return launch_res2d<kModeDgrad>(p, st);
            default: return launch_res2d<kModeFwd>(p, st);
        }
    }
    if (r.mode == kModeStem) return launch_igemm<64, kModeStem>(p, st);
    if (r.ek == kEkGeluFwd) return launch_pipe<128, kModeFwd, kEkGeluFwd>(p, st);
    if (r.ek == kEkGeluBwd) return launch_pipe<128, kModeFwd, kEkGeluBwd>(p, st);
    if (r.bn == 128) launch_conv_bn<128>(r, p, st);
    else launch_conv_bn<64>(r, p, st);
}

static int run_conv(const ConvProblem& p, lp_stream_t stream) {
    const ConvRoute r = route_conv(p, lp_switches());
    if (r.kernel == kNoKernel) return LP_ERR_UNSUPPORTED;
    launch_conv(r, p, (hipStream_t)stream);
    return launch_status();
}

static ConvProblem conv_problem(int mode, const void* x, const void* w, const ConvGeom& g, int rows_h, int rows_w, int N, int K) {
    ConvProblem p{};
    p.mode = mode, p.ek = -1, p.x = x, p.w = w, p.g = g;
    p.lat = Lattice{0, 1, rows_h, 0, 1, rows_w, 0, 1, g.R, 0, 1, g.S};
    p.M = g.B * rows_h * rows_w, p.N = N, p.K = K, p.seg_rows = p.M;
    p.dense = true, p.igemm_form = true, p.igemm_cols = N, p.nz = 1;
    return p;
}

static int gemm_problem(ConvProblem& p, int mode, const void* a, int lda, const void* b, int ldb, int ldc, int c_align, int M, int N, int K,
                        const lp_gemm_batch* batch) {
    if (K % kBK != 0 || lda % 8 != 0 || ldb % 8 != 0 || ldc % c_align != 0) return LP_ERR_UNSUPPORTED;
    const lp_gemm_batch z = batch ? *batch : lp_gemm_batch{1, 1, 0, 0, 0, 0, 0, 0};
    LP_REQUIRE(z.nb > 0 && z.nh > 0 && z.a_b >= 0 && z.a_h >= 0 && z.b_b >= 0 && z.b_h >= 0 && z.c_b >= 0 && z.c_h >= 0);
    const long long a_elems = (z.nb - 1) * z.a_b + (z.nh - 1) * z.a_h + (long long)(M - 1) * lda + K;
    const long long b_elems = (z.nb - 1) * z.b_b + (z.nh - 1) * z.b_h + (long long)(N - 1) * ldb + K;
    const long long c_elems = (z.nb - 1) * z.c_b + (z.nh - 1) * z.c_h + (long long)M * ldc;
    if (a_elems >= (1LL << 31) || b_elems >= (1LL << 31) || c_elems >= (1LL << 32)) return LP_ERR_UNSUPPORTED;
    if ((z.a_b | z.a_h | z.b_b | z.b_h) % 8 != 0 || (z.c_b | z.c_h) % c_align != 0) return LP_ERR_UNSUPPORTED;
    p = conv_problem(mode, a, b, ConvGeom{1, 1, M, K, 1, M, N, 1, 1, 1, 0}, 1, M, N, K);
    p.dense = z.nb * z.nh == 1 && lda == K && ldb == K && ldc == N;
    p.gemm = true, p.nz = z.nb * z.nh, p.x_bytes = (unsigned)(2 * a_elems), p.w_bytes = (unsigned)(2 * b_elems);
    p.gx = GemmExt{lda, ldb, z.nh, 0, (unsigned)(2 * z.a_b), (unsigned)(2 * z.a_h), (unsigned)(2 * z.b_b), (unsigned)(2 * z.b_h), (unsigned)z.c_b,
                   (unsigned)z.c_h};
    return LP_OK;
}

}
#include "conv_stem_wgrad.h"
#include "conv_wgrad_nb.h"
namespace lp {

constexpr int kWgradWgs = 512;

struct WgradRoute {
    bool ok;
    int kernel;
    int split, per;
    size_t ws_floats;
    int bn, tiles_a, tiles_b;
    bool swap, tuned;
    int Ka, Cb;
    int kh, PT, lead;
};

static void slice_pixels(WgradRoute& p, int units, int ksteps, int split, int cap) {
    if (split > cap) split = cap;
    if (split < 1) split = 1;
    p.per = ((ksteps + split - 1) / split) * kBK;
    p.split = (units + p.per - 1) / p.per;
}

static WgradRoute plan_wgrad(int M, int Kw, int Co, int split_hint) {
    WgradRoute p{};
    p.kernel = LP_CONV_KERNEL_WGRAD;
    p.bn = Co > 64 ? 128 : 64;
    p.tiles_a = (Kw + kBM - 1) / kBM;
    p.tiles_b = p.bn == 128 ? (Co + 127) / 128 : 1;
    const int tiles = p.tiles_a * p.tiles_b, ksteps = (M + kBK - 1) / kBK;
    slice_pixels(p, M, ksteps, split_hint > 0 ? split_hint : kWgradWgs / tiles, ksteps < 65535 ? ksteps : 65535);
    p.ws_floats = (size_t)p.split * tiles * 4 * 2 * (p.bn / 64) * 16 * 64;
    p.ok = true;
    return p;
}

static WgradRoute plan_stem_wgrad_nb(const ConvGeom& g, int split_hint) {
    WgradRoute p{};
    if (g.Wo % 64 != 0 || g.Hi != 2 * g.Ho || g.Wi != 2 * g.Wo || 128ull * g.B * g.Ho * g.Wo >= (1ull << 31) ||
        8ull * g.B * g.Hi * g.Wi >= (1ull << 31))
        return p;
    p.kernel = LP_CONV_KERNEL_STEM_WGRAD_NB;
    p.bn = 64, p.tiles_a = 2, p.tiles_b = 1;
    const int M = g.B * g.Ho * g.Wo, ksteps = M / kBK;
    slice_pixels(p, M, ksteps, split_hint > 0 ? split_hint : 768, ksteps);
    p.ws_floats = (size_t)p.split * 2 * 4 * 2 * 16 * 64;
    p.ok = true;
    return p;
}

static WgradRoute plan_wgrad_pipe(const ConvGeom& g, int split_hint) {
    WgradRoute p{};
    const int M = g.B * g.Ho * g.Wo, Kw = g.R * g.S * g.Ci;
    const bool one = g.R == 1 && g.S == 1 && g.stride == 1 && g.pad == 0 && g.Hi == g.Ho && g.Wi == g.Wo;
    if (g.Ci % 8 != 0 || g.Co % 64 != 0 || M < 4 * kBK) return p;
    p.kernel = LP_CONV_KERNEL_WGRAD_PIPE;
    p.swap = one && Kw % 256 != 0 && g.Co % 256 == 0 && Kw % 64 == 0;
    p.Ka = p.swap ? g.Co : Kw;
    p.Cb = p.swap ? Kw : g.Co;
    p.bn = p.Cb % 128 == 0 ? 128 : 64;
    if (p.Cb % p.bn != 0) return p;
    p.tiles_a = (p.Ka + 255) / 256;
    p.tiles_b = p.Cb / p.bn;
    p.tuned = (long long)p.tiles_a * 256 * 8 <= (long long)p.Ka * 9 && (long long)p.Ka * p.Cb >= 120LL * (p.Ka + p.Cb);
    const int tiles = p.tiles_a * p.tiles_b;
    const int cus = conv_max_wgs(1);
    const int ksteps = (M + kBK - 1) / kBK;
    int split = split_hint;
    if (split <= 0) {
        double best = 1e30;
        for (int s = 1; s <= 2 * cus && s <= ksteps / 2; ++s) {
            if (s != 1 && (tiles * s) % cus > 0 && (tiles * (s + 1) + cus - 1) / cus == (tiles * s + cus - 1) / cus) continue;
            const double rounds = (double)((tiles * s + cus - 1) / cus), per = (double)((ksteps + s - 1) / s);
            const double cost = rounds * per + 0.04 * (p.bn / 128.0) * s * tiles + 2.0 * rounds;
            if (cost < best) best = cost, split = s;
        }
    }
    slice_pixels(p, M, ksteps, split, ksteps / 2);
    p.ws_floats = (size_t)p.split * tiles * 256 * p.bn;
    p.ok = true;
    return p;
}

static WgradRoute plan_wgrad_nb(const ConvGeom& g, int split_hint) {
    WgradRoute p{};
    if (g.R != 3 || g.S != 3 || g.stride != 1 || g.pad != 1 || g.Hi != g.Ho || g.Wi != g.Wo || g.Ci % 64 != 0 || g.Co % 64 != 0) return p;
    if (g.Wi > 126) return p;
    const long long pt = (long long)g.B * (g.Hi + 1) * (g.Wi + 1);
    if (pt + 64 * 8 >= (1LL << 31)) return p;
    p.kernel = LP_CONV_KERNEL_WGRAD_NB;
    p.PT = (int)pt;
    p.lead = 1 + (g.Wi + 1) / 64;
    p.bn = g.Co % 128 == 0 ? 128 : 64;
    p.kh = p.bn == 64 ? 2 : 1;
    p.tiles_a = g.Ci / 64;
    p.tiles_b = g.Co / p.bn;
    const int tiles = p.tiles_a * p.tiles_b;
    const int ksteps = (p.PT + kBK - 1) / kBK;
    int split = split_hint;
    if (split <= 0) {
        const int cus = conv_max_wgs(1);
        const double step_us = 0.96 * p.bn / 128.0;
        double best = 1e30;
        for (int s = 1; s <= ksteps && s * tiles <= 2 * cus; ++s) {
            const double rounds = (double)((tiles * s + cus - 1) / cus), per = (double)((ksteps + s - 1) / s);
            const double cost = rounds * (per * step_us + 15.0) + 0.06 * s * tiles;
            if (cost < best) best = cost, split = s;
        }
    }
    slice_pixels(p, p.PT, ksteps, split, ksteps < 65535 ? ksteps : 65535);
    p.ws_floats = (size_t)p.split * p.kh * tiles * 9 * 64 * p.bn;
    p.ok = true;
    return p;
}

static bool is_stem(const ConvGeom& g) { return g.R == 7 && g.S == 7 && g.stride == 2 && g.pad == 3 && g.Ci == 4 && g.Co == 64; }

struct WgradCandidates {
    int n;
    WgradRoute r[3];
};

static WgradCandidates wgrad_candidates(const ConvGeom& g, bool stem, int split_hint) {
    WgradCandidates c{};
    const int M = g.B * g.Ho * g.Wo;
    auto add = [&c](const WgradRoute& p) {
        if (p.ok) c.r[c.n++] = p;
    };
    if (stem) {
        if (lp_switches().stem_wgrad_nb != 0) add(plan_stem_wgrad_nb(g, split_hint));
        add(plan_wgrad(M, 256, 64, split_hint));
    } else {
        add(plan_wgrad_nb(g, split_hint));
        add(plan_wgrad_pipe(g, split_hint));
        add(plan_wgrad(M, g.R * g.S * g.Ci, g.Co, split_hint));
    }
    return c;
}

static const WgradRoute& route_wgrad(const WgradCandidates& c, const LpSwitches& sw, bool dbias) {
    const bool pipe = !dbias && sw.conv_pipe != 0;
    for (int i = 0; i < c.n - 1; ++i) {
        const WgradRoute& r = c.r[i];
        if (r.kernel == LP_CONV_KERNEL_WGRAD_NB && !(pipe && sw.wgrad_pipe == 1 && sw.wgrad_nb != 0)) continue;
        if (r.kernel == LP_CONV_KERNEL_WGRAD_PIPE && !(pipe && sw.wgrad_pipe != 0 && (sw.wgrad_pipe == 2 || r.tuned))) continue;
        return r;
    }
    return c.r[c.n - 1];
}

template <int BN>
static void launch_wgrad(const WgradRoute& p, const void* x, const void* dy, const ConvGeom& g, float* dw, float* dbias, float* ws, hipStream_t st) {
    const int M = g.B * g.Ho * g.Wo, Kw = g.R * g.S * g.Ci, tiles = p.tiles_a * p.tiles_b;
    const unsigned x_bytes = (unsigned)(2ull * g.B * g.Hi * g.Wi * g.Ci), dy_bytes = (unsigned)(2ull * M * g.Co);
    TnExt ext{};
    ext.col_sums = dbias;
    const auto kernel = dbias ? conv_wgrad_kernel<BN, false, true> : conv_wgrad_kernel<BN, false, false>;
    hipLaunchKernelGGL(kernel, dim3(tiles * p.split), dim3(256), 0, st, (const unsigned short*)x, (const unsigned short*)dy, x_bytes, dy_bytes, g,
                       M, Kw, tiles, p.tiles_b, p.per, make_fastdiv(g.Ho * g.Wo), make_fastdiv(g.Wo), ws, ext);
    launch_wgrad_reduce<BN>(ws, p.split, tiles, p.tiles_b, Kw, g.Co, dw, st);
}

template <int BN>
static void launch_wgrad_pipe(const WgradRoute& p, const void* x, const void* dy, const ConvGeom& g, float* dw, float* ws, hipStream_t st) {
    const int M = g.B * g.Ho * g.Wo, Kw = g.R * g.S * g.Ci;
    const unsigned x_bytes = (unsigned)(2ull * g.B * g.Hi * g.Wi * g.Ci), dy_bytes = (unsigned)(2ull * M * g.Co);
    WgradPipeGeom wg{};
    const void *pa = x, *qb = dy;
    unsigned pa_bytes = x_bytes, qb_bytes = dy_bytes;
    if (p.swap) {
        wg = WgradPipeGeom{g.B, g.Ho, g.Wo, g.Ho, g.Wo, g.Co, 1, 1, 1, 0, p.Ka, p.Cb, 1};
        pa = dy, qb = x, pa_bytes = dy_bytes, qb_bytes = x_bytes;
    } else {
        const int plain = g.R == 1 && g.S == 1 && g.stride == 1 && g.pad == 0 && g.Hi == g.Ho && g.Wi == g.Wo;
        wg = WgradPipeGeom{g.B, g.Hi, g.Wi, g.Ho, g.Wo, g.Ci, g.R, g.S, g.stride, g.pad, p.Ka, p.Cb, plain};
    }
    const int tiles = p.tiles_a * p.tiles_b;
    const int sa = p.swap ? Kw : 1, sb = p.swap ? 1 : Kw;
    hipLaunchKernelGGL((conv_wgrad_pipe_kernel<BN>), dim3(tiles * p.split), dim3(512), 0, st, (const unsigned short*)pa, (const unsigned short*)qb,
                       pa_bytes, qb_bytes, wg, M, tiles, p.tiles_b, p.per, make_fastdiv(g.Ho * g.Wo), make_fastdiv(g.Wo), ws);
    hipLaunchKernelGGL((wgrad_pipe_reduce_kernel<BN>), dim3(tiles * 256 * BN / 64), dim3(256), 0, st, ws, p.split, tiles, p.tiles_b, p.Ka, p.Cb,
                       sa, sb, dw);
}

template <int BN>
static void launch_wgrad_nb(const WgradRoute& p, const void* x, const void* dy, const ConvGeom& g, float* dw, float* ws, hipStream_t st) {
    const unsigned x_bytes = (unsigned)(2ull * g.B * g.Hi * g.Wi * g.Ci), dy_bytes = (unsigned)(2ull * g.B * g.Ho * g.Wo * g.Co);
    const WgradNbGeom ng{g.B, g.Hi, g.Wi, g.Ci, g.Co, p.PT, p.lead};
    const int tiles = p.tiles_a * p.tiles_b;
    hipLaunchKernelGGL((conv_wgrad_nb_kernel<BN>), dim3(tiles * p.split), dim3(512), 0, st, (const unsigned short*)x, (const unsigned short*)dy,
                       x_bytes, dy_bytes, ng, tiles, p.tiles_b, p.per, make_fastdiv(g.Wi + 1), make_fastdiv(g.Hi + 1), ws);
    hipLaunchKernelGGL((wgrad_nb_reduce_kernel<BN>), dim3(tiles * 9 * BN), dim3(256), 0, st, ws, p.split * p.kh, tiles, p.tiles_b, g.Ci, dw);
}

static bool geom_ok(const lp_conv_geom* c) {
    return c && c->B > 0 && c->Hi > 0 && c->Wi > 0 && c->Ci > 0 && c->Ho > 0 && c->Wo > 0 && c->Co > 0 && c->R > 0 && c->S > 0 &&
           c->stride > 0 && c->pad >= 0;
}

static ConvGeom to_geom(const lp_conv_geom* c) {
    ConvGeom g{c->B, c->Hi, c->Wi, c->Ci, c->Ho, c->Wo, c->Co, c->R, c->S, c->stride, c->pad};
    return g;
}

}

static int conv_fwd_impl(const void* x, const void* w, const lp_conv_geom* geom, const float* bias, void* out_bf16, float* out_f32, int ldo,
                         int n_store, const lp_bn_fuse* bn, lp_stream_t stream) {
    using namespace lp;
    LP_REQUIRE(x && w && geom_ok(geom) && (out_bf16 || out_f32) && ldo > 0);
    ConvGeom g = to_geom(geom);
    if (g.Ci % kBK != 0 || g.R * g.S > 32 || (long long)g.B * g.Hi * g.Wi * g.Ci >= (1LL << 31) ||
        (long long)g.B * g.Ho * g.Wo * ldo >= (1LL << 32))
        return LP_ERR_UNSUPPORTED;
    ConvProblem p = conv_problem(kModeFwd, x, w, g, g.Ho, g.Wo, g.Co, g.R * g.S * g.Ci);
    p.ek = kEkNone;
    p.ep = ConvEpilogue{(unsigned short*)out_bf16, out_f32, ldo, n_store > 0 ? n_store : p.N, bias};
    if (bn) {
        LP_REQUIRE(bn->sums && bn->seg_images >= 0);
        if (p.N % 8 != 0) return LP_ERR_UNSUPPORTED;
        p.seg_rows = seg_split_rows(bn->seg_images, g.B, (long long)g.Ho * g.Wo, p.M);
        if (p.seg_rows < 0) return LP_ERR_UNSUPPORTED;
        bn_fuse_begin(p.ep, bn);
    }
    return run_conv(p, stream);
}

extern "C" int lp_conv_last_kernel(void) { return lp::g_last_conv_kernel; }

extern "C" int lp_conv_fwd(const void* x, const void* w, const lp_conv_geom* geom, const float* bias, void* out_bf16, float* out_f32,
                           int ldo, int n_store, lp_stream_t stream) {
    return conv_fwd_impl(x, w, geom, bias, out_bf16, out_f32, ldo, n_store, nullptr, stream);
}

extern "C" int lp_conv_fwd_act(const void* x, const void* w, const lp_conv_geom* geom, const float* bias, const void* residual_bf16, int relu,
                               void* out_bf16, lp_stream_t stream) {
    using namespace lp;
    LP_REQUIRE(x && w && geom_ok(geom) && out_bf16);
    ConvGeom g = to_geom(geom);
    if (g.Ci % kBK != 0 || g.Co % 8 != 0 || g.R * g.S > 32 || (long long)g.B * g.Hi * g.Wi * g.Ci >= (1LL << 31) ||
        (long long)g.B * g.Ho * g.Wo * g.Co >= (1LL << 32))
        return LP_ERR_UNSUPPORTED;
    ConvProblem p = conv_problem(kModeInfer, x, w, g, g.Ho, g.Wo, g.Co, g.R * g.S * g.Ci);
    p.ek = kEkInfer, p.gate = &LpSwitches::infer_pipe;
    p.ep.out_bf16 = (unsigned short*)out_bf16, p.ep.ldo = p.N, p.ep.n_store = p.N, p.ep.bias = bias;
    p.ep.addend = (const unsigned short*)residual_bf16, p.ep.relu_fwd = relu != 0;
    return run_conv(p, stream);
}

extern "C" int lp_conv_fwd_bn(const void* x, const void* w, const lp_conv_geom* geom, void* out_bf16, const lp_bn_fuse* bn,
                              lp_stream_t stream) {
    LP_REQUIRE(bn && geom && out_bf16);
    return conv_fwd_impl(x, w, geom, nullptr, out_bf16, nullptr, geom->Co, 0, bn, stream);
}

extern "C" int lp_gemm_nt(const void* a, int lda, const void* b, int ldb, void* c_bf16, float* c_f32, int ldc, int M, int N, int K,
                          int n_store, const float* bias, const lp_gemm_batch* batch, lp_stream_t stream) {
    using namespace lp;
    LP_REQUIRE(a && b && (c_bf16 || c_f32) && M > 0 && N > 0 && K > 0 && lda >= K && ldb >= K && ldc > 0);
    ConvProblem p;
    if (const int rc = gemm_problem(p, kModeFwd, a, lda, b, ldb, ldc, 1, M, N, K, batch)) return rc;
    p.ek = kEkNone, p.gate = &LpSwitches::gemm_pipe;
    p.ep = ConvEpilogue{(unsigned short*)c_bf16, c_f32, ldc, n_store > 0 ? n_store : N, bias};
    p.igemm_cols = p.ep.n_store;
    return run_conv(p, stream);
}

extern "C" int lp_gemm_nt_gelu_fwd(const void* a, const void* b, const float* bias, void* c_bf16, void* act_bf16, int M, int N, int K,
                                   lp_stream_t stream) {
    using namespace lp;
    LP_REQUIRE(a && b && c_bf16 && act_bf16 && M > 0 && N > 0 && K > 0);
    ConvProblem p;
    if (const int rc = gemm_problem(p, kModeFwd, a, K, b, K, N, 1, M, N, K, nullptr)) return rc;
    p.ek = kEkGeluFwd, p.igemm_form = false;
    p.ep = ConvEpilogue{(unsigned short*)c_bf16, nullptr, N, N, bias};
    p.ep.out2_bf16 = (unsigned short*)act_bf16;
    return run_conv(p, stream);
}

extern "C" int lp_gemm_nt_gelu_bwd(const void* a, const void* b, const void* u_bf16, void* c_bf16, int M, int N, int K, lp_fxsum* colsum,
                                   lp_stream_t stream) {
    using namespace lp;
    LP_REQUIRE(a && b && u_bf16 && c_bf16 && M > 0 && N > 0 && K > 0);
    ConvProblem p;
    if (const int rc = gemm_problem(p, kModeFwd, a, K, b, K, N, 1, M, N, K, nullptr)) return rc;
    p.ek = kEkGeluBwd, p.igemm_form = false;
    p.ep = ConvEpilogue{(unsigned short*)c_bf16, nullptr, N, N, nullptr};
    p.ep.addend = (const unsigned short*)u_bf16;
    p.ep.stats_sums = colsum;
    return run_conv(p, stream);
}

extern "C" int lp_attn_dscores(const void* d_out, int ld_do, const void* v, int ldv, const void* p_bf16, const float* d_rows, int d_row_stride,
                               long long d_b, long long d_h, float scale, void* ds_bf16, int ldc, int M, int N, int K,
                               const lp_gemm_batch* batch, lp_stream_t stream) {
    using namespace lp;
    LP_REQUIRE(d_out && v && p_bf16 && d_rows && ds_bf16 && batch && M > 0 && N > 0 && K > 0 && ld_do >= K && ldv >= K && ldc >= N &&
               d_row_stride > 0 && d_b >= 0 && d_h >= 0);
    ConvProblem p;
    if (const int rc = gemm_problem(p, kModeAttn, d_out, ld_do, v, ldv, ldc, 8, M, N, K, batch)) return rc;
    const long long d_elems = (batch->nb - 1) * d_b + (batch->nh - 1) * d_h + (long long)(M - 1) * d_row_stride + 1;
    if (d_elems >= (1LL << 32)) return LP_ERR_UNSUPPORTED;
    p.ep.out_bf16 = (unsigned short*)ds_bf16;
    p.ep.ldo = ldc;
    p.ep.n_store = ldc;
    p.ep.attn_p = (const unsigned short*)p_bf16;
    p.ep.attn_d = d_rows;
    p.ep.attn_scale = scale;
    p.igemm_cols = ldc;
    p.gx.d_zb = (unsigned)d_b, p.gx.d_zh = (unsigned)d_h, p.gx.d_row = (unsigned)d_row_stride;
    return run_conv(p, stream);
}

static int conv_dgrad_impl(const void* dy, const void* wd, const lp_conv_geom* geom, const float* bias, const void* addend,
                           const void* relu_mask, void* dx_bf16, float* dx_f32, int ldo, int n_store, int skip_empty_classes,
                           const lp_bn_fuse* bn, lp_stream_t stream, const void* relu_bits = nullptr) {
    using namespace lp;
    LP_REQUIRE(dy && wd && geom_ok(geom) && (dx_bf16 || dx_f32) && ldo > 0);
    ConvGeom g = to_geom(geom);
    if (g.Co % kBK != 0 || (g.stride != 1 && g.stride != 2) || g.R * g.S > 32 || (long long)g.B * g.Ho * g.Wo * g.Co >= (1LL << 31) ||
        (long long)g.B * g.Hi * g.Wi * ldo >= (1LL << 32))
        return LP_ERR_UNSUPPORTED;
    const int N = g.Ci;
    ConvProblem p = conv_problem(kModeDgrad, dy, wd, g, g.Hi, g.Wi, N, g.R * g.S * g.Co);
    ConvEpilogue& ep = p.ep;
    ep = ConvEpilogue{(unsigned short*)dx_bf16, dx_f32, ldo, n_store > 0 ? n_store : N, bias, (const unsigned short*)addend,
                      (const unsigned short*)relu_mask};
    if (relu_bits != nullptr) {
        LP_REQUIRE(bn == nullptr && relu_mask == nullptr && dx_bf16 && !dx_f32 && ldo == N && ep.n_store == N);
        if (N % 8 != 0) return LP_ERR_UNSUPPORTED;
        ep.relu_bits = (const unsigned char*)relu_bits;
    }
    if (bn) {
        LP_REQUIRE(bn->z && bn->mean && bn->invstd && bn->sums && dx_bf16 && !dx_f32 && !skip_empty_classes &&
                   ldo == N && ep.n_store == N && (!bn->mask_from_z || (bn->gamma && bn->beta)));
        if (N % 8 != 0) return LP_ERR_UNSUPPORTED;
        LP_REQUIRE(!(bn->relu_bits && (relu_mask || bn->mask_from_z)) && bn->seg_images >= 0);
        bn_fuse_begin(ep, bn);
        ep.bn_z = (const unsigned short*)bn->z;
        ep.bn_mean = bn->mean;
        ep.bn_invstd = bn->invstd;
        ep.bn_gamma = bn->gamma;
        ep.bn_beta = bn->beta;
        ep.mask_from_z = bn->mask_from_z;
        ep.relu_bits = (const unsigned char*)bn->relu_bits;
        ep.addend_half = bn->addend_half;
        LP_REQUIRE(!ep.addend_half || (addend && bn->relu_bits && g.stride == 1));
    }
    p.ek = pipe_dgrad_kind(ep);
    struct DgradLaunch {
        Lattice lat;
        int M, K;
        long long seg_rows;
        ConvRoute route;
    };
    DgradLaunch plan[4];
    int n = 0;
    auto add = [&](const Lattice& lat) {
        const int M = g.B * lat.nh * lat.nw;
        if (M <= 0) return;
        plan[n++] = DgradLaunch{lat, M, lat.nr * lat.ns * g.Co, bn ? seg_split_rows(bn->seg_images, g.B, (long long)lat.nh * lat.nw, M) : M, {}};
    };
    if (g.stride == 1) {
        add(p.lat);
    } else {
        for (int ph = 0; ph < 2; ++ph)
            for (int pw = 0; pw < 2; ++pw) {
                const int h0 = ((ph - g.pad) % 2 + 2) % 2, w0 = ((pw - g.pad) % 2 + 2) % 2;
                const int nh = h0 < g.Hi ? (g.Hi - h0 + 1) / 2 : 0, nw = w0 < g.Wi ? (g.Wi - w0 + 1) / 2 : 0;
                const int nr = ph < g.R ? (g.R - ph + 1) / 2 : 0, ns = pw < g.S ? (g.S - pw + 1) / 2 : 0;
                if (skip_empty_classes && nr * ns == 0) continue;
                add(Lattice{h0, 2, nh, w0, 2, nw, ph, 2, nr, pw, 2, ns});
            }
    }
    auto problem_of = [&p](const DgradLaunch& e) {
        p.lat = e.lat, p.M = e.M, p.K = e.K, p.seg_rows = e.seg_rows;
    };
    for (int i = 0; i < n; ++i) {
        if (plan[i].seg_rows < 0) return LP_ERR_UNSUPPORTED;
        problem_of(plan[i]);
        plan[i].route = route_conv(p, lp_switches());
    }
    for (int i = 0; i < n; ++i) {
        problem_of(plan[i]);
        launch_conv(plan[i].route, p, (hipStream_t)stream);
    }
    return launch_status();
}

extern "C" int lp_conv_dgrad(const void* dy, const void* wd, const lp_conv_geom* geom, const float* bias, const void* addend,
                             const void* relu_mask, void* dx_bf16, float* dx_f32, int ldo, int n_store, int skip_empty_classes,
                             lp_stream_t stream) {
    return conv_dgrad_impl(dy, wd, geom, bias, addend, relu_mask, dx_bf16, dx_f32, ldo, n_store, skip_empty_classes, nullptr, stream);
}

extern "C" int lp_conv_dgrad_bits(const void* dy, const void* wd, const lp_conv_geom* geom, const void* addend, const void* relu_bits,
                                  void* dx_bf16, int skip_empty_classes, lp_stream_t stream) {
    LP_REQUIRE(relu_bits && geom);
    return conv_dgrad_impl(dy, wd, geom, nullptr, addend, nullptr, dx_bf16, nullptr, geom->Ci, 0, skip_empty_classes, nullptr, stream, relu_bits);
}

extern "C" int lp_conv_dgrad_bn(const void* dy, const void* wd, const lp_conv_geom* geom, const void* addend, const void* relu_mask,
                                void* dx_bf16, const lp_bn_fuse* bn, lp_stream_t stream) {
    LP_REQUIRE(bn && geom);
    return conv_dgrad_impl(dy, wd, geom, nullptr, addend, relu_mask, dx_bf16, nullptr, geom->Ci, 0, 0, bn, stream);
}

extern "C" size_t lp_conv_wgrad_workspace_bytes(const lp_conv_geom* geom, int split_hint) {
    using namespace lp;
    if (!geom_ok(geom)) return 0;
    const ConvGeom g = to_geom(geom);
    const WgradCandidates c = wgrad_candidates(g, is_stem(g), split_hint);
    size_t fl = 0;
    for (int i = 0; i < c.n; ++i)
        if (c.r[i].ws_floats > fl) fl = c.r[i].ws_floats;
    return fl * sizeof(float);
}

static int conv_wgrad_impl(const void* x, const void* dy, const lp_conv_geom* geom, float* dw, float* dbias, int split_hint, void* workspace,
                           size_t workspace_bytes, lp_stream_t stream) {
    using namespace lp;
    LP_REQUIRE(x && dy && geom_ok(geom) && dw && workspace);
    ConvGeom g = to_geom(geom);
    if (g.Ci % 8 != 0 || g.Co % 8 != 0 || (long long)g.B * g.Hi * g.Wi * g.Ci >= (1LL << 31) ||
        (long long)g.B * g.Ho * g.Wo * g.Co >= (1LL << 31))
        return LP_ERR_UNSUPPORTED;
    const WgradCandidates c = wgrad_candidates(g, false, split_hint);
    const WgradRoute& p = route_wgrad(c, lp_switches(), dbias != nullptr);
    LP_REQUIRE(workspace_bytes >= p.ws_floats * sizeof(float));
    hipStream_t st = (hipStream_t)stream;
    float* ws = (float*)workspace;
    g_last_conv_kernel = p.kernel;
    if (p.kernel == LP_CONV_KERNEL_WGRAD_NB) {
        if (p.bn == 128) launch_wgrad_nb<128>(p, x, dy, g, dw, ws, st);
        else launch_wgrad_nb<64>(p, x, dy, g, dw, ws, st);
    } else if (p.kernel == LP_CONV_KERNEL_WGRAD_PIPE) {
        if (p.bn == 128) launch_wgrad_pipe<128>(p, x, dy, g, dw, ws, st);
        else launch_wgrad_pipe<64>(p, x, dy, g, dw, ws, st);
    } else {
        if (p.bn == 128) launch_wgrad<128>(p, x, dy, g, dw, dbias, ws, st);
        else launch_wgrad<64>(p, x, dy, g, dw, dbias, ws, st);
    }
    return launch_status();
}

extern "C" int lp_conv_wgrad(const void* x, const void* dy, const lp_conv_geom* geom, float* dw, int split_hint, void* workspace,
                             size_t workspace_bytes, lp_stream_t stream) {
    return conv_wgrad_impl(x, dy, geom, dw, nullptr, split_hint, workspace, workspace_bytes, stream);
}

extern "C" int lp_conv_wgrad_bias(const void* x, const void* dy, const lp_conv_geom* geom, float* dw, float* dbias, int split_hint,
                                  void* workspace, size_t workspace_bytes, lp_stream_t stream) {
    LP_REQUIRE(dbias);
    return conv_wgrad_impl(x, dy, geom, dw, dbias, split_hint, workspace, workspace_bytes, stream);
}

extern "C" int lp_gemm_tn(const void* x, int ldx, const void* y, int ldy, void* out_bf16, int ldo, int M, int J, int N,
                          const lp_gemm_batch* batch, lp_stream_t stream) {
    using namespace lp;
    LP_REQUIRE(x && y && out_bf16 && M > 0 && J > 0 && N > 0 && ldx >= J && ldy >= N && ldo >= N);
    if (ldx % 8 != 0 || ldy % 8 != 0 || N % 8 != 0) return LP_ERR_UNSUPPORTED;
    const int nb = batch ? batch->nb : 1, nh = batch ? batch->nh : 1;
    LP_REQUIRE(nb > 0 && nh > 0);
    const long long a_b = batch ? batch->a_b : 0, a_h = batch ? batch->a_h : 0, b_b = batch ? batch->b_b : 0, b_h = batch ? batch->b_h : 0;
    const long long c_b = batch ? batch->c_b : 0, c_h = batch ? batch->c_h : 0;
    LP_REQUIRE(a_b >= 0 && a_h >= 0 && b_b >= 0 && b_h >= 0 && c_b >= 0 && c_h >= 0);
    if ((a_b | a_h | b_b | b_h) % 8 != 0) return LP_ERR_UNSUPPORTED;
    const int Jr = (J + 7) / 8 * 8;
    LP_REQUIRE(Jr <= ldx);
    const long long x_elems = (nb - 1) * a_b + (nh - 1) * a_h + (long long)(M - 1) * ldx + Jr;
    const long long y_elems = (nb - 1) * b_b + (nh - 1) * b_h + (long long)(M - 1) * ldy + N;
    const long long o_elems = (nb - 1) * c_b + (nh - 1) * c_h + (long long)J * ldo;
    if (x_elems >= (1LL << 31) || y_elems >= (1LL << 31) || o_elems >= (1LL << 32)) return LP_ERR_UNSUPPORTED;
    ConvGeom g{1, 1, M, Jr, 1, M, N, 1, 1, 1, 0};
    const int tj = (Jr + kBM - 1) / kBM;
    TnExt tn{(unsigned short*)out_bf16, ldx, ldy, ldo, nh, (unsigned)(2 * a_b), (unsigned)(2 * a_h), (unsigned)(2 * b_b), (unsigned)(2 * b_h),
             (unsigned)c_b, (unsigned)c_h};
    hipStream_t st = (hipStream_t)stream;
    const int nz = nb * nh;
    if (N > 64) {
        const int tn_ = (N + 127) / 128;
        hipLaunchKernelGGL((conv_wgrad_kernel<128, false>), dim3(tj * tn_ * nz), dim3(256), 0, st, (const unsigned short*)x,
                           (const unsigned short*)y, (unsigned)(2 * x_elems), (unsigned)(2 * y_elems), g, M, J, tj * tn_, tn_, M,
                           make_fastdiv(M), make_fastdiv(M), (float*)nullptr, tn);
    } else {
        hipLaunchKernelGGL((conv_wgrad_kernel<64, false>), dim3(tj * nz), dim3(256), 0, st, (const unsigned short*)x,
                           (const unsigned short*)y, (unsigned)(2 * x_elems), (unsigned)(2 * y_elems), g, M, J, tj, 1, M, make_fastdiv(M),
                           make_fastdiv(M), (float*)nullptr, tn);
    }
    return launch_status();
}

static int stem_fwd_impl(const void* x4, const void* w, const lp_conv_geom* geom, void* out_bf16, const lp_bn_fuse* bn,
                         lp_stream_t stream) {
    using namespace lp;
    LP_REQUIRE(x4 && w && geom_ok(geom) && out_bf16);
    ConvGeom g = to_geom(geom);
    if (!is_stem(g)) return LP_ERR_UNSUPPORTED;
    ConvProblem p = conv_problem(kModeStem, x4, w, g, g.Ho, g.Wo, 64, 256);
    p.gate = &LpSwitches::stem_2d;
    p.ep = ConvEpilogue{(unsigned short*)out_bf16, nullptr, 64, 64};
    if (bn) {
        LP_REQUIRE(bn->sums && bn->seg_images >= 0);
        if (seg_split_rows(bn->seg_images, g.B, (long long)g.Ho * g.Wo, p.M) < 0) return LP_ERR_UNSUPPORTED;
        bn_fuse_begin(p.ep, bn);
    }
    return run_conv(p, stream);
}

extern "C" int lp_stem_fwd(const void* x4, const void* w, const lp_conv_geom* geom, void* out_bf16, lp_stream_t stream) {
    return stem_fwd_impl(x4, w, geom, out_bf16, nullptr, stream);
}

extern "C" int lp_stem_fwd_bn(const void* x4, const void* w, const lp_conv_geom* geom, void* out_bf16, const lp_bn_fuse* bn,
                              lp_stream_t stream) {
    LP_REQUIRE(bn);
    return stem_fwd_impl(x4, w, geom, out_bf16, bn, stream);
}

extern "C" int lp_stem_wgrad(const void* x4, const void* dy, const lp_conv_geom* geom, float* dw, int split_hint, void* workspace,
                             size_t workspace_bytes, lp_stream_t stream) {
    using namespace lp;
    LP_REQUIRE(x4 && dy && geom_ok(geom) && dw && workspace);
    ConvGeom g = to_geom(geom);
    if (!is_stem(g)) return LP_ERR_UNSUPPORTED;
    const WgradCandidates c = wgrad_candidates(g, true, split_hint);
    const WgradRoute& p = route_wgrad(c, lp_switches(), false);
    LP_REQUIRE(workspace_bytes >= p.ws_floats * sizeof(float));
    const int M = g.B * g.Ho * g.Wo, Kw = 256;
    const unsigned short *xs = (const unsigned short*)x4, *dys = (const unsigned short*)dy;
    const FastDiv dhw = make_fastdiv(g.Ho * g.Wo), dwo = make_fastdiv(g.Wo);
    hipStream_t st = (hipStream_t)stream;
    float* ws = (float*)workspace;
    g_last_conv_kernel = p.kernel;
    if (p.kernel == LP_CONV_KERNEL_STEM_WGRAD_NB)
        hipLaunchKernelGGL(stem_wgrad_nb_kernel, dim3(p.split), dim3(256), 0, st, xs, dys, (unsigned)(8ull * g.B * g.Hi * g.Wi),
                           (unsigned)(128ull * M), g, M, p.per, dhw, dwo, ws);
    else
        hipLaunchKernelGGL((conv_wgrad_kernel<64, true>), dim3(p.tiles_a * p.split), dim3(256), 0, st, xs, dys, 0u, 0u, g, M, Kw, p.tiles_a, 1,
                           p.per, dhw, dwo, ws, TnExt{});
    launch_wgrad_reduce<64>(ws, p.split, p.tiles_a, 1, Kw, 64, dw, st);
    return launch_status();
}
```

lightning-pose_amd/csrc/conv_pipe.h:

```cpp
#pragma once

#include <type_traits>

namespace lp {

#ifndef LP_HALO_KEY_ROW
#define LP_HALO_KEY_ROW 0
#endif
#ifndef LP_HALO_STAGES
#define LP_HALO_STAGES 3
#endif
#ifndef LP_FWD_CORNER_PAD
#define LP_FWD_CORNER_PAD 0
#endif
#ifndef LP_PIPE_SPREAD
#define LP_PIPE_SPREAD 1
#endif
constexpr bool kSpread = LP_PIPE_SPREAD != 0;
constexpr int kPM = 256;
constexpr int kPRowB = 128;

#if defined(__HIP_DEVICE_COMPILE__)
#define LP_WAIT_VM(n) asm volatile("s_waitcnt vmcnt(" #n ")" ::: "memory")
#define LP_RAW_BARRIER()                   \
    do {                                   \
        asm volatile("" ::: "memory");     \
        __builtin_amdgcn_s_barrier();      \
        asm volatile("" ::: "memory");     \
    } while (0)
#define LP_WAIT_LGKM_TOUCH3(n, a, b, c) asm volatile("s_waitcnt lgkmcnt(" #n ")" : "+v"(a), "+v"(b), "+v"(c)::"memory")
#define LP_WAIT_LGKM_TOUCH4(n, a, b, c, d) asm volatile("s_waitcnt lgkmcnt(" #n ")" : "+v"(a), "+v"(b), "+v"(c), "+v"(d)::"memory")
#else
#define LP_WAIT_VM(n) ((void)0)
#define LP_RAW_BARRIER() __syncthreads()
#define LP_WAIT_LGKM_TOUCH3(n, a, b, c) ((void)0)
#define LP_WAIT_LGKM_TOUCH4(n, a, b, c, d) ((void)0)
#endif

__device__ __forceinline__ void store8(unsigned short* p, u16x8 v) { *reinterpret_cast<u16x8*>(p) = v; }

enum { kEkNone = 0, kEkZ = 1, kEkAZB = 2, kEkPlain = 3, kEkInfer = 4, kEkPB = 5, kEkGeluBwd = 6, kEkGeluFwd = 7 };

struct HaloDivs {
    FastDiv h, wp, hp;
};

template <int BN, int MODE, int EK, bool HALO = false>
__global__ __launch_bounds__(512) void conv_pipe_kernel(const unsigned short* __restrict__ X, const unsigned short* __restrict__ Wt,
                                                        unsigned x_bytes, unsigned w_bytes, ConvGeom g, Lattice lat, FastDiv div_img,
                                                        FastDiv div_row, int M, int N, int K, int tiles_n, int ntiles, ConvEpilogue ep,
                                                        HaloDivs hd) {
    static_assert((MODE == kModeFwd && (EK == kEkNone || EK == kEkInfer || EK == kEkGeluBwd || EK == kEkGeluFwd)) ||
                      (MODE == kModeDgrad && EK != kEkNone && EK != kEkInfer && EK != kEkGeluBwd && EK != kEkGeluFwd),
                  "trunk convolutions only");
    constexpr int NT = BN / 64;
    constexpr int NBL = BN / 64;
    constexpr int kStageA = HALO ? 0 : kPM * kPRowB, kStageB = BN * kPRowB, kStage = kStageA + kStageB;
    constexpr int kHaloRows = BN == 64 ? 512 : 384;
    constexpr int kHaloB = kHaloRows * kPRowB, NA = kHaloRows / 64;
    constexpr int NST = HALO ? LP_HALO_STAGES : 3;
    static_assert(NST == 3 || NST == 4, "ring depth");
    __shared__ __attribute__((aligned(16))) unsigned char smem[NST * kStage + (HALO ? 2 * kHaloB : 0)];
    unsigned char* const halo0 = smem + NST * kStage;

    const int tid = threadIdx.x, lane = tid & 63;
    const int wave = __builtin_amdgcn_readfirstlane(tid >> 6);
    const int wm = wave & 3, wn = wave >> 2;

    const buf_rsrc rsrc_x = make_buf_rsrc(X, x_bytes), rsrc_w = make_buf_rsrc(Wt, w_bytes);
    const int rows_y = lat.nh, rows_x = lat.nw;
    const int full_h = (MODE == kModeDgrad) ? g.Hi : g.Ho;
    const int full_w = (MODE == kModeDgrad) ? g.Wi : g.Wo;
    const int ck = (MODE == kModeDgrad) ? g.Co : g.Ci;
    const int src_h = (MODE == kModeDgrad) ? g.Ho : g.Hi;
    const int src_w = (MODE == kModeDgrad) ? g.Wo : g.Wi;
    const bool halved = (MODE == kModeDgrad) && g.stride == 2;
    const int KT = K / kBK;
    const int ldw = g.R * g.S * ck;

    const int rloc = lane >> 3, slot = lane & 7;
    const int lrow = wave * 8 + rloc;
    const int lchunk = slot ^ ((lrow >> 1) & 7);
    int py[4], px[4];
    unsigned rowoff[4], vmask[4], voff[4], wrow[NBL];
    int tir = 0, tis = 0, tc = 0;
    unsigned wtap = 0;
    int ld_vt = blockIdx.x, ld_kt = 0;

    auto setup = [&](int vt) {
        if (vt >= ntiles) {
#pragma unroll
            for (int i = 0; i < 4; ++i) vmask[i] = 0u, rowoff[i] = 0u;
#pragma unroll
            for (int i = 0; i < NBL; ++i) wrow[i] = ~0u;
            tir = tis = tc = 0;
            return;
        }
        const int tile = xcd_remap(vt, ntiles);
        const int tm_ = tile / tiles_n;
        const int m0 = tm_ * kPM, n0 = (tile - tm_ * tiles_n) * BN;
#pragma unroll
        for (int i = 0; i < (HALO ? 0 : 4); ++i) {
            const int m = m0 + lrow + 64 * i;
            const bool pv = m < M;
            const int mm = pv ? m : 0;
            const int b = fdiv(mm, div_img);
            const int rem = mm - b * rows_y * rows_x;
            const int iy = fdiv(rem, div_row);
            const int y = lat.h0 + lat.hstep * iy, xq = lat.w0 + lat.wstep * (rem - iy * rows_x);
            if (MODE == kModeDgrad) {
                py[i] = y + g.pad;
                px[i] = xq + g.pad;
            } else {
                py[i] = y * g.stride - g.pad;
                px[i] = xq * g.stride - g.pad;
            }
            const int oy = halved ? (py[i] >> 1) : py[i], ox = halved ? (px[i] >> 1) : px[i];
            rowoff[i] = (unsigned)(((b * src_h + oy) * src_w + ox) * ck + lchunk * 8) * 2u;
            unsigned mask = 0;
            if (pv) {
                for (int ir = 0; ir < lat.nr; ++ir)
                    for (int it = 0; it < lat.ns; ++it) {
                        const int r = lat.r0 + lat.rstep * ir, t = lat.s0 + lat.sstep * it;
                        bool ok;
                        if (MODE == kModeDgrad) {
                            const int th = py[i] - r, tw = px[i] - t;
                            if (halved) ok = th >= 0 && tw >= 0 && !((th | tw) & 1) && (th >> 1) < g.Ho && (tw >> 1) < g.Wo;
                            else ok = th >= 0 && th < g.Ho && tw >= 0 && tw < g.Wo;
                        } else {
                            const int sy = py[i] + r, sx = px[i] + t;
                            ok = sy >= 0 && sy < g.Hi && sx >= 0 && sx < g.Wi;
                        }
                        mask |= (ok ? 1u : 0u) << (ir * lat.ns + it);
                    }
            }
            vmask[i] = mask;
        }
#pragma unroll
        for (int i = 0; i < NBL; ++i) wrow[i] = (unsigned)((n0 + lrow + 64 * i) * ldw + lchunk * 8) * 2u;
        tir = tis = tc = 0;
    };

    unsigned is_soff_a = 0, is_soff_b = 0, is_w[NBL];
    unsigned char* is_dst = smem;
    auto prep_step = [&](int st) {
        if (HALO) {
            const int tr = tir / 3, ts = tir - tr * 3;
            is_soff_b = (unsigned)(((tr * g.S + ts) * ck + tc) * 2);
#pragma unroll
            for (int i = 0; i < NBL; ++i) is_w[i] = wrow[i];
            is_dst = smem + st * kStage + wave * (8 * kPRowB);
            if (++tir == 9) tir = 0, tc += kBK;
            return;
        }
        if (tc == 0) {
            const int tr = lat.r0 + lat.rstep * tir, ts = lat.s0 + lat.sstep * tis;
            const int qr = halved ? (tr >> 1) : tr, qs = halved ? (ts >> 1) : ts;
            const unsigned tapoff_b = (unsigned)(((MODE == kModeDgrad) ? -(qr * src_w + qs) : (qr * src_w + qs)) * ck) * 2u;
            const int tap = tir * lat.ns + tis;
            wtap = (unsigned)((tr * g.S + ts) * ck) * 2u;
#pragma unroll
            for (int i = 0; i < 4; ++i) {
                const unsigned ok = (vmask[i] >> tap) & 1u;
                voff[i] = (rowoff[i] + tapoff_b) | (ok - 1u);
            }
        }
        is_soff_a = (unsigned)tc * 2u;
        is_soff_b = wtap + is_soff_a;
#pragma unroll
        for (int i = 0; i < NBL; ++i) is_w[i] = wrow[i];
        is_dst = smem + st * kStage + wave * (8 * kPRowB);
        tc += kBK;
        if (tc >= ck) {
            tc = 0;
            if (++tis == lat.ns) {
                tis = 0;
                ++tir;
            }
        }
    };
    auto issue_load = [&](int i) {
        if (HALO) buf_load16_lds(rsrc_w, is_dst + (i % NBL) * (64 * kPRowB), is_w[i % NBL], is_soff_b);
        else if (i < 4) buf_load16_lds(rsrc_x, is_dst + i * (64 * kPRowB), voff[i], is_soff_a);
        else buf_load16_lds(rsrc_w, is_dst + kStageA + (i - 4) * (64 * kPRowB), is_w[i - 4], is_soff_b);
    };
    auto advance_tile = [&]() {
        if (++ld_kt == KT) {
            ld_kt = 0;
            ld_vt += gridDim.x;
            setup(ld_vt);
        }
    };
    auto load_step = [&](int st) {
        prep_step(st);
#pragma unroll
        for (int i = 0; i < (HALO ? NBL : 4 + NBL); ++i) issue_load(i);
        advance_tile();
    };

    const int hW = g.Wi, hH = g.Hi, hWp = g.Wi + 2, hHp = g.Hi + 2;
    unsigned hvoff[HALO ? NA : 1];
    int hl_vt = blockIdx.x, hl_slice = 0, hl_buf = 0;
    auto padded = [&](int m) {
        const int rm = fdiv(m, div_row), bm = fdiv(rm, hd.h);
        return (rm + 1 + 2 * bm) * hWp + (m - rm * hW) + 1;
    };
    auto padded_row = [&](int m) {
        const int rm = fdiv(m, div_row), bm = fdiv(rm, hd.h);
        return rm + 1 + 2 * bm;
    };
    auto halo_setup = [&](int vt) {
        if (vt >= ntiles) {
#pragma unroll
            for (int i = 0; i < (HALO ? NA : 0); ++i) hvoff[i] = ~0u;
            return;
        }
        const int tile = xcd_remap(vt, ntiles);
        const int m0h = (tile / tiles_n) * kPM;
        const int pbase = padded(m0h) - (hW + 3), rr0 = padded_row(m0h) - 1;
#pragma unroll
        for (int i = 0; i < (HALO ? NA : 0); ++i) {
            const int j = i * 64 + lrow, pp = pbase + j, pc = pp < 0 ? 0 : pp;
            const int rr = fdiv(pc, hd.wp), xx = pc - rr * hWp;
            const int bb = fdiv(rr, hd.hp), yy = rr - bb * hHp;
            const bool ok = pp >= 0 && xx >= 1 && xx <= hW && yy >= 1 && yy <= hH && bb < g.B;
            const int u = LP_HALO_KEY_ROW ? j : j - 2 * (rr - rr0);
            const int chunk = slot ^ ((u >> 1) & 7);
            hvoff[i] = ok ? (unsigned)((((bb * hH + yy - 1) * hW + xx - 1) * ck + chunk * 8) * 2) : ~0u;
        }
    };
    auto halo_issue = [&](int i) {
        buf_load16_lds(rsrc_x, halo0 + hl_buf * kHaloB + i * (64 * kPRowB) + wave * (8 * kPRowB), hvoff[HALO ? i : 0], (unsigned)(hl_slice * (kBK * 2)));
    };
    auto halo_advance = [&]() {
        hl_buf ^= 1;
        if ((hl_slice + 1) * kBK >= ck) {
            hl_slice = 0;
            hl_vt += gridDim.x;
            halo_setup(hl_vt);
        } else {
            ++hl_slice;
        }
    };

    const int fr = lane & 31, fg = lane >> 5;
    const int fsw = (fr >> 1) & 7;
    unsigned koff[4];
#pragma unroll
    for (int kk = 0; kk < 4; ++kk) koff[kk] = (unsigned)(((kk * 2 + fg) ^ fsw) * 16);
    const unsigned a_row = (unsigned)((wm * 64 + fr) * kPRowB);
    const unsigned b_row = (unsigned)(kStageA + (wn * (NT * 32) + fr) * kPRowB);

    f32x16 acc[2][NT];
#ifndef LP_PIPE_FRAG_SETS
#define LP_PIPE_FRAG_SETS 2
#endif
    constexpr int NS = (MODE == kModeFwd) ? LP_PIPE_FRAG_SETS : 2;
    int ploc[2] = {0, 0}, uloc[2] = {0, 0}, mh_buf = 0, mh_tap = 0;
    auto mma_stage = [&](int st, const bool spread) {
        const unsigned char* sb = smem + st * kStage;
        bf16x8 a[NS][2], b[NS][NT];
        const unsigned char* ha[2] = {smem, smem};
        unsigned hk[2][4] = {};
        if (HALO) {
            const int tr = mh_tap / 3, ts = mh_tap - tr * 3;
            const int dp = (tr - 1) * hWp + (ts - 1), du = (tr - 1) * hW + (ts - 1);
#pragma unroll
            for (int mt = 0; mt < 2; ++mt) {
                const int row = ploc[mt] + (MODE == kModeDgrad ? -dp : dp);
                const int sw = LP_HALO_KEY_ROW ? (row >> 1) & 7 : ((uloc[mt] + (MODE == kModeDgrad ? -du : du)) >> 1) & 7;
                ha[mt] = halo0 + mh_buf * kHaloB + row * kPRowB;
#pragma unroll
                for (int kk = 0; kk < 4; ++kk) hk[mt][kk] = (unsigned)(((kk * 2 + fg) ^ sw) * 16);
            }
        }
        auto fetch = [&](int kk, int set) {
#pragma unroll
            for (int mt = 0; mt < 2; ++mt) {
                if (HALO) a[set][mt] = __builtin_bit_cast(bf16x8, *reinterpret_cast<const u16x8*>(ha[mt] + hk[mt][kk]));
                else a[set][mt] = __builtin_bit_cast(bf16x8, *reinterpret_cast<const u16x8*>(sb + a_row + mt * (32 * kPRowB) + koff[kk]));
            }
#pragma unroll
            for (int nt = 0; nt < NT; ++nt)
                b[set][nt] = __builtin_bit_cast(bf16x8, *reinterpret_cast<const u16x8*>(sb + b_row + nt * (32 * kPRowB) + koff[kk]));
        };
#pragma unroll
        for (int kk = 0; kk < NS - 1; ++kk) fetch(kk, kk);
#pragma unroll
        for (int kk = 0; kk < kBK / 16; ++kk) {
            if (kk + NS - 1 < kBK / 16) fetch(kk + NS - 1, (kk + NS - 1) % NS);
            __builtin_amdgcn_sched_barrier(0);
#pragma unroll
            for (int mt = 0; mt < 2; ++mt)
#pragma unroll
                for (int nt = 0; nt < NT; ++nt)
                    acc[mt][nt] = __builtin_amdgcn_mfma_f32_32x32x16_bf16(b[kk % NS][nt], a[kk % NS][mt], acc[mt][nt], 0, 0, 0);
            if (spread && HALO) {
                if (kk == 0) {
                    switch (mh_tap) {
                    case 0: halo_issue(0); break;
                    case 1: halo_issue(1); break;
                    case 2: halo_issue(2); break;
                    case 3: halo_issue(3); break;
                    case 4: halo_issue(4); break;
                    case 5: halo_issue(5); break;
                    case 6: if (NA > 6) halo_issue(NA > 6 ? 6 : 0); break;
                    case 7: if (NA > 7) halo_issue(NA > 7 ? 7 : 0); break;
                    default: break;
                    }
                } else if (kk == 1) {
                    issue_load(0);
                } else if (kk == 2) {
                    if (NBL == 2) issue_load(1);
                }
            } else if (spread) {
                constexpr int NL = 4 + NBL;
                if (kk == 0) {
                    issue_load(0);
                    issue_load(1);
                } else if (kk == 1) {
                    issue_load(2);
                    if (NL == 6) issue_load(3);
                } else if (kk == 2) {
                    issue_load(NL == 6 ? 4 : 3);
                } else {
                    issue_load(NL - 1);
                }
            }
            __builtin_amdgcn_sched_barrier(0);
        }
    };

    constexpr bool kFwd = (MODE == kModeFwd);
    constexpr int CP = NT * 4;
    constexpr int RP = 64 / CP;
    const int pc = lane % CP, prow = lane / CP;
    float s0[8], s1[8];
#pragma unroll
    for (int q = 0; q < 8; ++q) s0[q] = s1[q] = 0.f;
    int st_n0 = -1, st_seg_off = 0;
    const bool want_stats = ep.stats_sums != nullptr;
    constexpr bool bwd = (EK == kEkZ || EK == kEkAZB);
    auto stats_flush = [&](float* scratch) {
        if (st_n0 >= 0) {
#pragma unroll
            for (int q = 0; q < 8; ++q) {
#pragma unroll
                for (int msk = CP; msk < 64; msk <<= 1) {
                    s0[q] += __shfl_xor(s0[q], msk, 64);
                    s1[q] += __shfl_xor(s1[q], msk, 64);
                }
            }
            __syncthreads();
            if (lane < CP) {
#pragma unroll
                for (int q = 0; q < 8; ++q) {
                    scratch[(wave * 2 + 0) * (NT * 32) + lane * 8 + q] = s0[q];
                    scratch[(wave * 2 + 1) * (NT * 32) + lane * 8 + q] = s1[q];
                }
            }
            __syncthreads();
            if (tid < 2 * BN) {
                const int comp = tid / BN, cl = tid % BN;
                const int wn_ = cl / (NT * 32), c = cl % (NT * 32);
                float t = 0.f;
#pragma unroll
                for (int w4 = 0; w4 < 4; ++w4) t += scratch[((wn_ * 4 + w4) * 2 + comp) * (NT * 32) + c];
                if (bwd && comp == 1) t *= ep.bn_invstd[st_seg_off + st_n0 + cl];
                stats_emit(ep, 2 * st_seg_off + comp * N + st_n0 + cl, t);
            }
            __syncthreads();
        }
#pragma unroll
        for (int q = 0; q < 8; ++q) s0[q] = s1[q] = 0.f;
    };

    auto epilogue_fwd = [&](const int m0, const int n0, unsigned char* stg_all) {
        const int nbase = n0 + wn * (NT * 32);
        constexpr bool infer = EK == kEkInfer;
        constexpr bool gelub = EK == kEkGeluBwd;
        constexpr bool kPad = LP_FWD_CORNER_PAD != 0;
        constexpr int ROWB = NT * 64 + (kPad ? 16 : 0);
        unsigned char* stg = stg_all + wave * (32 * ROWB);
        const int wkey = kPad ? 0 : NT == 2 ? (fr & 15) : ((fr >> 1) & 7);
        u16x8 radd[2][32 / RP] = {};
        if ((infer || gelub) && ep.addend != nullptr) {
#pragma unroll
            for (int mt = 0; mt < 2; ++mt)
#pragma unroll
                for (int ps = 0; ps < 32 / RP; ++ps) {
                    const int m = m0 + wm * 64 + mt * 32 + ps * RP + prow;
                    if (m < M)
                        radd[mt][ps] = load8(ep.addend + (unsigned)out_row(m, lat, div_img, div_row, full_h, full_w) * (unsigned)ep.ldo +
                                             (unsigned)(nbase + pc * 8));
                }
        }
        if (ep.bias != nullptr) {
#pragma unroll
            for (int nt = 0; nt < NT; ++nt)
#pragma unroll
                for (int j = 0; j < 4; ++j) {
                    const f32x4 bv = *reinterpret_cast<const f32x4*>(ep.bias + nbase + nt * 32 + 8 * j + 4 * fg);
#pragma unroll
                    for (int mt = 0; mt < 2; ++mt)
#pragma unroll
                        for (int e = 0; e < 4; ++e) acc[mt][nt][4 * j + e] += bv[e];
                }
        }
#pragma unroll
        for (int mt = 0; mt < 2; ++mt) {
#pragma unroll
            for (int nt = 0; nt < NT; ++nt)
#pragma unroll
                for (int j = 0; j < 4; ++j) {
                    typedef __attribute__((ext_vector_type(2))) unsigned u32x2_t;
                    const u32x2_t p = {pack_bf16x2(acc[mt][nt][4 * j], acc[mt][nt][4 * j + 1]),
                                       pack_bf16x2(acc[mt][nt][4 * j + 2], acc[mt][nt][4 * j + 3])};
                    *reinterpret_cast<u32x2_t*>(stg + fr * ROWB + ((((nt * 4 + j) * 2 + fg) ^ wkey) << 3)) = p;
                }
            __builtin_amdgcn_wave_barrier();
#pragma unroll
            for (int ps = 0; ps < 32 / RP; ++ps) {
                const int row = ps * RP + prow;
                const int rkey = kPad ? 0 : NT == 2 ? (row & 15) : ((row >> 1) & 7);
                u16x8 w;
                {
                    typedef __attribute__((ext_vector_type(4))) unsigned u32x4_t;
                    const u32x4_t q = *reinterpret_cast<const u32x4_t*>(stg + row * ROWB + ((pc ^ (rkey >> 1)) << 4));
                    const bool sw = (rkey & 1) != 0;
                    const u32x4_t o = {sw ? q[2] : q[0], sw ? q[3] : q[1], sw ? q[0] : q[2], sw ? q[1] : q[3]};
                    w = __builtin_bit_cast(u16x8, o);
                }
                const int m = m0 + wm * 64 + mt * 32 + row;
                if (m < M) {
                    const unsigned off = (unsigned)out_row(m, lat, div_img, div_row, full_h, full_w) * (unsigned)ep.ldo + (unsigned)(nbase + pc * 8);
                    if (infer) {
                        float v[8];
#pragma unroll
                        for (int q = 0; q < 8; ++q) v[q] = bf16_to_f32(w[q]);
                        if (ep.addend != nullptr) {
#pragma unroll
                            for (int q = 0; q < 8; ++q) v[q] += bf16_to_f32(radd[mt][ps][q]);
                        }
                        if (ep.relu_fwd) {
#pragma unroll
                            for (int q = 0; q < 8; ++q) v[q] = fmaxf(v[q], 0.f);
                        }
                        w = pack_bf16x8(v);
                    }
                    if (gelub) {
                        float v[8], u8[8];
#pragma unroll
                        for (int q = 0; q < 8; ++q) v[q] = bf16_to_f32(w[q]), u8[q] = bf16_to_f32(radd[mt][ps][q]);
                        gelu8_bwd(v, u8);
                        w = pack_bf16x8(v);
                    }
                    store8(ep.out_bf16 + off, w);
                    if (EK == kEkGeluFwd) {
                        float v[8];
#pragma unroll
                        for (int q = 0; q < 8; ++q) v[q] = bf16_to_f32(w[q]);
                        gelu8(v);
                        store8(ep.out2_bf16 + off, pack_bf16x8(v));
                    }
                    if (want_stats) {
#pragma unroll
                        for (int q = 0; q < 8; ++q) {
                            const float vr = bf16_to_f32(w[q]);
                            s0[q] += vr;
                            s1[q] = fmaf(vr, vr, s1[q]);
                        }
                    }
                }
            }
            __builtin_amdgcn_wave_barrier();
        }
    };

    constexpr int PH = 16 / RP;
    constexpr int NPC = 2 * PH;
    constexpr bool kLa = (EK == kEkAZB || EK == kEkPlain || EK == kEkPB), kLz = (EK != kEkNone && EK != kEkInfer && EK != kEkPB && EK != kEkGeluBwd && EK != kEkGeluFwd),
                   kLb = (EK == kEkAZB || EK == kEkPB);
    constexpr bool kKeepOff = EK != kEkAZB;
    struct ReadBack {
        unsigned off[kKeepOff ? NPC : 1];
        u16x8 la[kLa ? NPC : 1];
        u16x8 lz[kLz ? NPC : 1];
        unsigned lb[kLb ? NPC : 1];
    };
    float mu[8], sc[8], be[8];
    auto rb_issue = [&](ReadBack& rb, const int mt, const int m0, const int n0) {
        const int nbase = n0 + wn * (NT * 32);
#pragma unroll
        for (int p = 0; p < NPC; ++p) {
            const int m = m0 + wm * 64 + mt * 32 + (p / PH) * 16 + (p % PH) * RP + prow;
            const bool rv = m < M;
            const unsigned off_p = rv ? (unsigned)(kKeepOff ? out_row(m, lat, div_img, div_row, full_h, full_w) : m) * (unsigned)ep.ldo + (unsigned)(nbase + pc * 8) : ~0u;
            if (kKeepOff) rb.off[kKeepOff ? p : 0] = off_p;
            const unsigned o = rv ? off_p : (unsigned)(nbase + pc * 8);
            if (EK == kEkAZB && ep.addend_half) {
                const int mm = rv ? m : 0;
                const int bi = fdiv(mm, div_img), rem = mm - bi * div_img.d;
                const int yy = fdiv(rem, div_row), xx = rem - yy * div_row.d;
                const bool on = rv && !((yy | xx) & 1);
                const unsigned oa = (unsigned)((bi * ((full_h + 1) >> 1) + (yy >> 1)) * ((full_w + 1) >> 1) + (xx >> 1)) * (unsigned)ep.ldo + (unsigned)(nbase + pc * 8);
                rb.la[kLa ? p : 0] = on ? load8_stream(ep.addend + oa) : zero8();
            } else if (EK == kEkAZB || ((EK == kEkPlain || EK == kEkPB) && ep.addend)) rb.la[kLa ? p : 0] = load8_stream(ep.addend + o);
            if (bwd) rb.lz[kLz ? p : 0] = load8(ep.bn_z + o);
            if (EK == kEkPlain && ep.relu_mask) rb.lz[kLz ? p : 0] = load8_stream(ep.relu_mask + o);
            if (EK == kEkAZB || EK == kEkPB) rb.lb[kLb ? p : 0] = ep.relu_bits[o >> 3];
        }
    };
    auto rb_process = [&](const ReadBack& rb, const int mt, unsigned char* stg_all, const int m0, const int n0) {
        constexpr int ROWF = NT * 128 + 16;
        unsigned char* stg = stg_all + wave * (16 * ROWF);
#pragma unroll
        for (int h = 0; h < 2; ++h) {
            if ((fr >> 4) == h) {
#pragma unroll
                for (int nt = 0; nt < NT; ++nt)
#pragma unroll
                    for (int j = 0; j < 4; ++j) {
                        const f32x4 p4 = {acc[mt][nt][4 * j], acc[mt][nt][4 * j + 1], acc[mt][nt][4 * j + 2], acc[mt][nt][4 * j + 3]};
                        *reinterpret_cast<f32x4*>(stg + (fr & 15) * ROWF + (nt * 32 + 8 * j + 4 * fg) * 4) = p4;
                    }
            }
            __builtin_amdgcn_wave_barrier();
            f32x4 lo_[PH], hi_[PH];
#pragma unroll
            for (int ps = 0; ps < PH; ++ps) {
                lo_[ps] = *reinterpret_cast<const f32x4*>(stg + (ps * RP + prow) * ROWF + pc * 32);
                hi_[ps] = *reinterpret_cast<const f32x4*>(stg + (ps * RP + prow) * ROWF + pc * 32 + 16);
            }
            __builtin_amdgcn_wave_barrier();
#pragma unroll
            for (int ps = 0; ps < PH; ++ps) {
                const int p = h * PH + ps;
                unsigned off_p;
                if (kKeepOff) {
                    off_p = rb.off[kKeepOff ? p : 0];
                } else {
                    const int m = m0 + wm * 64 + mt * 32 + h * 16 + ps * RP + prow;
                    off_p = m < M ? (unsigned)m * (unsigned)ep.ldo + (unsigned)(n0 + wn * (NT * 32) + pc * 8) : ~0u;
                }
                if (off_p != ~0u) {
                    float v[8] = {lo_[ps][0], lo_[ps][1], lo_[ps][2], lo_[ps][3], hi_[ps][0], hi_[ps][1], hi_[ps][2], hi_[ps][3]};
                    if (EK == kEkAZB || ((EK == kEkPlain || EK == kEkPB) && ep.addend)) {
#pragma unroll
                        for (int q = 0; q < 8; ++q) v[q] += bf16_to_f32(rb.la[kLa ? p : 0][q]);
                    }
                    float zc[8];
                    if (bwd) {
#pragma unroll
                        for (int q = 0; q < 8; ++q) zc[q] = bf16_to_f32(rb.lz[kLz ? p : 0][q]) - mu[q];
                        if (EK == kEkZ) {
#pragma unroll
                            for (int q = 0; q < 8; ++q)
                                if (!(fmaf(zc[q], sc[q], be[q]) > 0x1p-134f)) v[q] = 0.f;
                        }
                    }
                    if (EK == kEkPlain && ep.relu_mask) {
#pragma unroll
                        for (int q = 0; q < 8; ++q)
                            if (!bf16_positive(rb.lz[kLz ? p : 0][q])) v[q] = 0.f;
                    }
                    if (EK == kEkAZB || EK == kEkPB) {
#pragma unroll
                        for (int q = 0; q < 8; ++q)
                            if (!((rb.lb[kLb ? p : 0] >> q) & 1u)) v[q] = 0.f;
                    }
                    const u16x8 w = pack_bf16x8(v);
                    store8(ep.out_bf16 + off_p, w);
                    if (want_stats) {
#pragma unroll
                        for (int q = 0; q < 8; ++q) {
                            const float vr = bf16_to_f32(w[q]);
                            s0[q] += vr;
                            s1[q] = fmaf(vr, bwd ? zc[q] : vr, s1[q]);
                        }
                    }
                }
            }
        }
    };

    if (HALO) {
        halo_setup(hl_vt);
#pragma unroll
        for (int i = 0; i < (HALO ? NA : 0); ++i) halo_issue(i);
        halo_advance();
    }
    setup(ld_vt);
#pragma unroll
    for (int st = 0; st < NST - 1; ++st) load_step(st);
    int cur = 0;
    ReadBack rb0, rb1;
    auto free_lds = [&]() -> unsigned char* { return HALO ? halo0 + (mh_buf ^ 1) * kHaloB : smem + (cur == 0 ? NST - 1 : cur - 1) * kStage; };
    for (int vt = blockIdx.x; vt < ntiles; vt += gridDim.x) {
        const int tile = xcd_remap(vt, ntiles);
        const int tm_ = tile / tiles_n;
        const int m0 = tm_ * kPM, n0 = (tile - tm_ * tiles_n) * BN;
        const int seg_off = (ep.seg_images > 0 && m0 >= ep.seg_images * rows_y * rows_x) ? N : 0;
        if (HALO) {
            const int pbase = padded(m0) - (hW + 3), rr0 = padded_row(m0) - 1;
#pragma unroll
            for (int mt = 0; mt < 2; ++mt) {
                const int m = m0 + wm * 64 + mt * 32 + fr, mc = m < M ? m : M - 1;
                ploc[mt] = padded(mc) - pbase;
                uloc[mt] = ploc[mt] - 2 * (padded_row(mc) - rr0);
            }
        }
        if (n0 != st_n0 || seg_off != st_seg_off) {
            if (want_stats) stats_flush(reinterpret_cast<float*>(free_lds()));
            st_n0 = n0;
            st_seg_off = seg_off;
            if (bwd) {
#pragma unroll
                for (int q = 0; q < 8; ++q) {
                    const int n = n0 + wn * (NT * 32) + pc * 8 + q;
                    mu[q] = ep.bn_mean[seg_off + n];
                    if (EK == kEkZ) {
                        sc[q] = ep.bn_invstd[seg_off + n] * ep.bn_gamma[n];
                        be[q] = ep.bn_beta[n];
                    }
                }
            }
        }
#pragma unroll
        for (int mt = 0; mt < 2; ++mt)
#pragma unroll
            for (int nt = 0; nt < NT; ++nt)
#pragma unroll
                for (int e = 0; e < 16; ++e) acc[mt][nt][e] = 0.f;
        for (int kt = 0; kt < KT; ++kt) {
            if (HALO && NBL == 2 && NST == 4) LP_WAIT_VM(4);
            else if (HALO && NST == 4) LP_WAIT_VM(2);
            else if (HALO && NBL == 2) LP_WAIT_VM(2);
            else if (HALO) LP_WAIT_VM(1);
            else if (NBL == 2) LP_WAIT_VM(6);
            else LP_WAIT_VM(5);
            LP_RAW_BARRIER();
            if (!kFwd && kt == KT - 1) rb_issue(rb0, 0, m0, n0);
            const int nxt = cur == 0 ? NST - 1 : cur - 1;
            if (kSpread || HALO) {
                prep_step(nxt);
                mma_stage(cur, true);
                advance_tile();
            } else {
                load_step(nxt);
                mma_stage(cur, false);
            }
            cur = cur == NST - 1 ? 0 : cur + 1;
            if (HALO && ++mh_tap == 9) {
                mh_tap = 0;
                mh_buf ^= 1;
                halo_advance();
            }
        }
        unsigned char* stg_all = free_lds();
        LP_RAW_BARRIER();
        if (kFwd) {
            epilogue_fwd(m0, n0, stg_all);
        } else {
            rb_issue(rb1, 1, m0, n0);
            rb_process(rb0, 0, stg_all, m0, n0);
            rb_process(rb1, 1, stg_all, m0, n0);
        }
    }
    if (want_stats) stats_flush(reinterpret_cast<float*>(free_lds()));
    LP_WAIT_VM(0);
}

struct WgradPipeGeom {
    int B, Hi, Wi, Ho, Wo;
    int Ca, R, S, stride, pad;
    int Ka, Cb;
    int plain;
};

template <int BN>
__global__ __launch_bounds__(512) void conv_wgrad_pipe_kernel(const unsigned short* __restrict__ Pa, const unsigned short* __restrict__ Qb,
                                                              unsigned pa_bytes, unsigned qb_bytes, WgradPipeGeom g, int M, int tiles,
                                                              int tiles_b, int m_per_split, FastDiv div_hw, FastDiv div_wo,
                                                              float* __restrict__ ws) {
    constexpr int NT = BN / 64;
    constexpr int kRowA = 512, kRowB = BN * 2;
    constexpr int kStageA = kBK * kRowA, kStageB = kBK * kRowB, kStage = kStageA + kStageB;
    constexpr int NLB = BN / 64;
    __shared__ __attribute__((aligned(16))) unsigned char smem[3 * kStage];

    const int tid = threadIdx.x, lane = tid & 63;
    const int wave = __builtin_amdgcn_readfirstlane(tid >> 6);
    const int wm = wave & 3, wn = wave >> 2;
    const int work = xcd_remap(blockIdx.x, gridDim.x);
    const int slice = work / tiles, tile = work - slice * tiles;
    const int a0 = (tile / tiles_b) * 256, b0 = (tile % tiles_b) * BN;
    const int m_begin = slice * m_per_split, m_end = min(M, m_begin + m_per_split);
    const int KT = (m_end - m_begin + kBK - 1) / kBK;
    const buf_rsrc rsrc_a = make_buf_rsrc(Pa, pa_bytes), rsrc_b = make_buf_rsrc(Qb, qb_bytes);

    const int arow = wave * 2 + (lane >> 5);
    const int achunk = (lane & 31) ^ ((arow & 3) << 2);
    const int ja = a0 + achunk * 8;
    const bool ja_ok = ja < g.Ka;
    const int tap = (ja_ok ? ja : 0) / g.Ca;
    const int tcn = (ja_ok ? ja : 0) - tap * g.Ca;
    const int tr = tap / g.S, ts = tap - tr * g.S;
    const int brow = (BN == 128) ? wave * 4 + (lane >> 4) : wave * 8 + (lane >> 3);
    const int bchunk = (BN == 128) ? ((lane & 15) ^ ((brow & 3) << 2)) : ((lane & 7) ^ (((brow >> 1) & 1) << 2));
    const unsigned boff = (unsigned)(b0 + bchunk * 8) * 2u;
    const int hw = g.Ho * g.Wo;

    unsigned is_a[4], is_b[NLB];
    unsigned char* is_dst = smem;
    const bool same = !g.plain && g.stride == 1 && g.Hi == g.Ho && g.Wi == g.Wo && hw >= kBK;
    const int qb64 = kBK / hw, qh64 = (kBK - qb64 * hw) / g.Wo, qw64 = kBK - qb64 * hw - qh64 * g.Wo;
    const int lo_h = max(0, g.pad - tr), span_h = min(g.Ho, g.Hi + g.pad - tr) - lo_h;
    const int lo_w = max(0, g.pad - ts), span_w = min(g.Wo, g.Wi + g.pad - ts) - lo_w;
    const unsigned tap_off = (unsigned)(((tr - g.pad) * g.Wi + (ts - g.pad)) * g.Ca + tcn) * 2u;
    int rho[4], rwo[4];
    if (same) {
#pragma unroll
        for (int p = 0; p < 4; ++p) {
            const int m = m_begin + p * 16 + arow;
            const int mm = m < M ? m : 0;
            const int rem = mm - fdiv(mm, div_hw) * hw;
            rho[p] = fdiv(rem, div_wo);
            rwo[p] = rem - rho[p] * g.Wo;
        }
    }
    auto prep_step = [&](int st, int kt) {
        const int mk = m_begin + kt * kBK;
#pragma unroll
        for (int p = 0; p < 4; ++p) {
            const int m = mk + p * 16 + arow;
            unsigned off;
            bool ok = ja_ok && m < m_end && kt < KT;
            if (g.plain) {
                off = (unsigned)(m * g.Ca + tcn) * 2u;
            } else if (same) {
                ok = ok && (unsigned)(rho[p] - lo_h) < (unsigned)span_h && (unsigned)(rwo[p] - lo_w) < (unsigned)span_w;
                off = (unsigned)m * (unsigned)(g.Ca * 2) + tap_off;
                rwo[p] += qw64;
                const int c = rwo[p] >= g.Wo ? 1 : 0;
                rwo[p] -= c ? g.Wo : 0;
                rho[p] += qh64 + c;
                rho[p] -= rho[p] >= g.Ho ? g.Ho : 0;
            } else {
                const int mm = ok ? m : 0;
                const int b = fdiv(mm, div_hw), rem = mm - b * hw;
                const int ho = fdiv(rem, div_wo), wo = rem - ho * g.Wo;
                const int hi = ho * g.stride - g.pad + tr, wi = wo * g.stride - g.pad + ts;
                ok = ok && hi >= 0 && hi < g.Hi && wi >= 0 && wi < g.Wi;
                off = (unsigned)(((b * g.Hi + hi) * g.Wi + wi) * g.Ca + tcn) * 2u;
            }
            is_a[p] = ok ? off : ~0u;
        }
#pragma unroll
        for (int q = 0; q < NLB; ++q) {
            const int m = mk + q * 32 + brow;
            is_b[q] = (m < m_end && kt < KT) ? (unsigned)m * (unsigned)(g.Cb * 2) + boff : ~0u;
        }
        is_dst = smem + st * kStage;
    };
    auto issue_load = [&](int i) {
        if (i < 4) buf_load16_lds(rsrc_a, is_dst + (i * 16 + wave * 2) * kRowA, is_a[i], 0u);
        else if (BN == 128) buf_load16_lds(rsrc_b, is_dst + kStageA + ((i - 4) * 32 + wave * 4) * kRowB, is_b[i - 4], 0u);
        else buf_load16_lds(rsrc_b, is_dst + kStageA + (wave * 8) * kRowB, is_b[0], 0u);
    };

    const int fq = lane >> 4, fi = lane & 15;
    const int frow = (fq >> 1) * 8 + (fi >> 2), fcol = (fq & 1) * 16 + (fi & 3) * 4;
    const int swa = (frow & 3) << 2;
    const int swb = (BN == 128) ? ((frow & 3) << 2) : (((frow >> 1) & 1) << 2);
    unsigned foa[2], fob[NT];
#pragma unroll
    for (int mt = 0; mt < 2; ++mt) {
        const int e0 = wm * 64 + mt * 32 + fcol;
        foa[mt] = (unsigned)(frow * kRowA + (((e0 >> 3) ^ swa) << 4) + (e0 & 7) * 2);
    }
#pragma unroll
    for (int nt = 0; nt < NT; ++nt) {
        const int e0 = wn * (NT * 32) + nt * 32 + fcol;
        fob[nt] = (unsigned)(kStageA + frow * kRowB + (((e0 >> 3) ^ swb) << 4) + (e0 & 7) * 2);
    }
    f32x16 acc[2][NT];
#pragma unroll
    for (int mt = 0; mt < 2; ++mt)
#pragma unroll
        for (int nt = 0; nt < NT; ++nt)
#pragma unroll
            for (int e = 0; e < 16; ++e) acc[mt][nt][e] = 0.f;

    auto mma_stage = [&](int st) {
        const unsigned char* sb = smem + st * kStage;
        bf16x8 a[2][2], b[2][NT];
        const unsigned char* pa[2];
        const unsigned char* pb[NT];
#pragma unroll
        for (int mt = 0; mt < 2; ++mt) pa[mt] = sb + foa[mt];
#pragma unroll
        for (int nt = 0; nt < NT; ++nt) pb[nt] = sb + fob[nt];
        auto fetch = [&](auto kk_c, int set) {
            constexpr int kk = decltype(kk_c)::value;
            typedef __attribute__((ext_vector_type(8))) short s16x8_t;
#pragma unroll
            for (int mt = 0; mt < 2; ++mt) {
                const s16x4_t lo = lds_read_tr16_async_off<kk * 16 * kRowA>(pa[mt]), hi = lds_read_tr16_async_off<kk * 16 * kRowA + 4 * kRowA>(pa[mt]);
                const s16x8_t v = {lo[0], lo[1], lo[2], lo[3], hi[0], hi[1], hi[2], hi[3]};
                a[set][mt] = __builtin_bit_cast(bf16x8, v);
            }
#pragma unroll
            for (int nt = 0; nt < NT; ++nt) {
                const s16x4_t lo = lds_read_tr16_async_off<kk * 16 * kRowB>(pb[nt]), hi = lds_read_tr16_async_off<kk * 16 * kRowB + 4 * kRowB>(pb[nt]);
                const s16x8_t v = {lo[0], lo[1], lo[2], lo[3], hi[0], hi[1], hi[2], hi[3]};
                b[set][nt] = __builtin_bit_cast(bf16x8, v);
            }
        };
        auto ready = [&](int set, bool last) {
            if (NT == 2) {
                if (last) LP_WAIT_LGKM_TOUCH4(0, a[set][0], a[set][1], b[set][0], b[set][NT - 1]);
                else LP_WAIT_LGKM_TOUCH4(8, a[set][0], a[set][1], b[set][0], b[set][NT - 1]);
            } else {
                if (last) LP_WAIT_LGKM_TOUCH3(0, a[set][0], a[set][1], b[set][0]);
                else LP_WAIT_LGKM_TOUCH3(6, a[set][0], a[set][1], b[set][0]);
            }
        };
        auto slice = [&](auto kk_c) {
            constexpr int kk = decltype(kk_c)::value;
            if constexpr (kk + 1 < kBK / 16) fetch(std::integral_constant<int, kk + 1>{}, (kk + 1) & 1);
            __builtin_amdgcn_sched_barrier(0);
            ready(kk & 1, kk + 1 == kBK / 16);
#pragma unroll
            for (int mt = 0; mt < 2; ++mt)
#pragma unroll
                for (int nt = 0; nt < NT; ++nt)
                    acc[mt][nt] = __builtin_amdgcn_mfma_f32_32x32x16_bf16(a[kk & 1][mt], b[kk & 1][nt], acc[mt][nt], 0, 0, 0);
            constexpr int NL = 4 + NLB;
            if (kk == 0) {
                issue_load(0);
                issue_load(1);
            } else if (kk == 1) {
                issue_load(2);
                if (NL == 6) issue_load(3);
            } else if (kk == 2) {
                issue_load(NL == 6 ? 4 : 3);
            } else {
                issue_load(NL - 1);
            }
            __builtin_amdgcn_sched_barrier(0);
        };
        fetch(std::integral_constant<int, 0>{}, 0);
        slice(std::integral_constant<int, 0>{});
        slice(std::integral_constant<int, 1>{});
        slice(std::integral_constant<int, 2>{});
        slice(std::integral_constant<int, 3>{});
    };

    prep_step(0, 0);
#pragma unroll
    for (int i = 0; i < 4 + NLB; ++i) issue_load(i);
    prep_step(1, 1);
#pragma unroll
    for (int i = 0; i < 4 + NLB; ++i) issue_load(i);
    int cur = 0;
    for (int kt = 0; kt < KT; ++kt) {
        if (NLB == 2) LP_WAIT_VM(6);
        else LP_WAIT_VM(5);
        LP_RAW_BARRIER();
        prep_step(cur == 0 ? 2 : cur - 1, kt + 2);
        mma_stage(cur);
        cur = cur == 2 ? 0 : cur + 1;
    }
    LP_WAIT_VM(0);
    float* dst = ws + ((((size_t)slice * tiles + tile) * 8 + wave) * (2 * NT * 16)) * 64 + lane;
#pragma unroll
    for (int mt = 0; mt < 2; ++mt)
#pragma unroll
        for (int nt = 0; nt < NT; ++nt)
#pragma unroll
            for (int e = 0; e < 16; ++e) dst[((mt * NT + nt) * 16 + e) * 64] = acc[mt][nt][e];
}

template <int BN>
__global__ __launch_bounds__(256) void wgrad_pipe_reduce_kernel(const float* __restrict__ ws, int slices, int tiles, int tiles_b, int Ka, int Cb,
                                                                int sa, int sb, float* __restrict__ dW) {
    constexpr int NT = BN / 64;
    constexpr int PER_TILE = 8 * 2 * NT * 16 * 64;
    __shared__ float part[4][64];
    const size_t total = (size_t)tiles * PER_TILE;
    const int lane = threadIdx.x & 63, w = threadIdx.x >> 6;
    const size_t i = (size_t)blockIdx.x * 64 + lane;
    float s0 = 0.f, s1 = 0.f;
    int sl = w;
    for (; sl + 4 < slices; sl += 8) {
        s0 += ws[(size_t)sl * total + i];
        s1 += ws[(size_t)(sl + 4) * total + i];
    }
    for (; sl < slices; sl += 4) s0 += ws[(size_t)sl * total + i];
    part[w][lane] = s0 + s1;
    __syncthreads();
    if (w == 0) {
        const float sum = (part[0][lane] + part[1][lane]) + (part[2][lane] + part[3][lane]);
        size_t t = i >> 6;
        const int e = (int)(t & 15);
        t >>= 4;
        const int nt = (int)(t % NT);
        t /= NT;
        const int mt = (int)(t & 1);
        t >>= 1;
        const int wave = (int)(t & 7);
        const int tile = (int)(t >> 3);
        const int wm = wave & 3, wn = wave >> 2;
        const int a = (tile / tiles_b) * 256 + wm * 64 + mt * 32 + (e & 3) + 8 * (e >> 2) + 4 * (lane >> 5);
        const int b = (tile % tiles_b) * BN + wn * (NT * 32) + nt * 32 + (lane & 31);
        if (a < Ka && b < Cb) dW[(size_t)a * sa + (size_t)b * sb] += sum;
    }
}

}
```

lightning-pose_amd/csrc/lp_common.h:

```cpp
#pragma once

#include <hip/hip_runtime.h>
#include <stdint.h>

#include "../../include/lp_hip.h"

namespace lp {

constexpr int kWave = 64;

typedef __attribute__((ext_vector_type(8))) __bf16 bf16x8;
typedef __attribute__((ext_vector_type(8))) unsigned short u16x8;
typedef __attribute__((ext_vector_type(4))) unsigned short u16x4;
typedef __attribute__((ext_vector_type(4))) float f32x4;
typedef __attribute__((ext_vector_type(16))) float f32x16;

__device__ __forceinline__ float bf16_to_f32(unsigned short b) { return __uint_as_float(((unsigned)b) << 16); }

#if defined(__HIP_DEVICE_COMPILE__)
typedef __attribute__((ext_vector_type(2))) __bf16 bf16x2_t;
typedef __attribute__((ext_vector_type(2))) float f32x2_t;
__device__ __forceinline__ unsigned short f32_to_bf16(float f) { return __builtin_bit_cast(unsigned short, (__bf16)f); }
__device__ __forceinline__ unsigned pack_bf16x2(float lo, float hi) {
    const f32x2_t v = {lo, hi};
    return __builtin_bit_cast(unsigned, __builtin_convertvector(v, bf16x2_t));
}
#else
__device__ __forceinline__ unsigned short f32_to_bf16(float f) {
    unsigned u = __float_as_uint(f);
    if ((u & 0x7fffffffu) > 0x7f800000u) return (unsigned short)((u >> 16) | 0x40u);
    u += 0x7fffu + ((u >> 16) & 1u);
    return (unsigned short)(u >> 16);
}
__device__ __forceinline__ unsigned pack_bf16x2(float lo, float hi) { return (unsigned)f32_to_bf16(lo) | ((unsigned)f32_to_bf16(hi) << 16); }
#endif

typedef float f32x2_t __attribute__((ext_vector_type(2)));
__device__ __forceinline__ float fast_rcp(float d) {
#if defined(__HIP_DEVICE_COMPILE__)
    return __builtin_amdgcn_rcpf(d);
#else
    return 1.0f / d;
#endif
}
__device__ __forceinline__ f32x2_t fma2(f32x2_t a, f32x2_t b, f32x2_t c) {
#if defined(__HIP_DEVICE_COMPILE__)
    return __builtin_elementwise_fma(a, b, c);
#else
    return f32x2_t{fmaf(a.x, b.x, c.x), fmaf(a.y, b.y, c.y)};
#endif
}
__device__ __forceinline__ f32x2_t fma2(f32x2_t a, f32x2_t b, float c) { return fma2(a, b, f32x2_t{c, c}); }
__device__ __forceinline__ f32x2_t gelu_f2(f32x2_t x) {
    const f32x2_t z = f32x2_t{fabsf(x.x), fabsf(x.y)} * 0.70710678118654752f;
    const f32x2_t d = fma2(z, f32x2_t{0.5f, 0.5f}, 1.f);
    const f32x2_t t = {fast_rcp(d.x), fast_rcp(d.y)};
    f32x2_t p = fma2(t, f32x2_t{0.17087277f, 0.17087277f}, -0.82215223f);
    p = fma2(p, t, 1.48851587f);
    p = fma2(p, t, -1.13520398f);
    p = fma2(p, t, 0.27886807f);
    p = fma2(p, t, -0.18628806f);
    p = fma2(p, t, 0.09678418f);
    p = fma2(p, t, 0.37409196f);
    p = fma2(p, t, 1.00002368f);
    p = fma2(p, t, -1.26551223f);
    const f32x2_t a = fma2(-z, z, p);
    const f32x2_t tail = t * 0.5f * f32x2_t{__expf(a.x), __expf(a.y)};
    const f32x2_t up = 1.f - tail;
    return x * f32x2_t{x.x < 0.f ? tail.x : up.x, x.y < 0.f ? tail.y : up.y};
}
__device__ __forceinline__ f32x2_t gelu_df2(f32x2_t x) {
    const f32x2_t z = f32x2_t{fabsf(x.x), fabsf(x.y)} * (0.3275911f * 0.70710678118654752f);
    const f32x2_t d = z + 1.f;
    const f32x2_t t = {fast_rcp(d.x), fast_rcp(d.y)};
    const f32x2_t h = x * x * -0.5f;
    const f32x2_t e = {__expf(h.x), __expf(h.y)};
    f32x2_t p = fma2(t, f32x2_t{1.061405429f, 1.061405429f}, -1.453152027f);
    p = fma2(p, t, 1.421413741f);
    p = fma2(p, t, -0.284496736f);
    p = fma2(p, t, 0.254829592f);
    const f32x2_t tail = p * t * 0.5f * e;
    const f32x2_t up = 1.f - tail;
    const f32x2_t phi = {x.x < 0.f ? tail.x : up.x, x.y < 0.f ? tail.y : up.y};
    return fma2(x * 0.3989422804014327f, e, phi);
}
__device__ __forceinline__ void gelu8(float (&v)[8]) {
#pragma unroll
    for (int i = 0; i < 8; i += 2) {
        const f32x2_t g = gelu_f2(f32x2_t{v[i], v[i + 1]});
        v[i] = g.x, v[i + 1] = g.y;
    }
}
__device__ __forceinline__ void gelu8_bwd(float (&d)[8], const float (&u)[8]) {
#pragma unroll
    for (int i = 0; i < 8; i += 2) {
        const f32x2_t g = f32x2_t{d[i], d[i + 1]} * gelu_df2(f32x2_t{u[i], u[i + 1]});
        d[i] = g.x, d[i + 1] = g.y;
    }
}

__device__ __forceinline__ u16x8 pack_bf16x8(const float (&f)[8]) {
    typedef __attribute__((ext_vector_type(4))) unsigned u32x4_t;
    const u32x4_t p = {pack_bf16x2(f[0], f[1]), pack_bf16x2(f[2], f[3]), pack_bf16x2(f[4], f[5]), pack_bf16x2(f[6], f[7])};
    return __builtin_bit_cast(u16x8, p);
}

__device__ __forceinline__ bool bf16_positive(unsigned short y) { return (short)y > 0; }

#if defined(__HIP_DEVICE_COMPILE__)
typedef __amdgpu_buffer_rsrc_t buf_rsrc;
__device__ __forceinline__ buf_rsrc make_buf_rsrc(const void* p, unsigned bytes) {
    return __builtin_amdgcn_make_buffer_rsrc(const_cast<void*>(p), 0, bytes, 0x00020000);
}
__device__ __forceinline__ u16x8 buf_load16(buf_rsrc r, unsigned voff, unsigned soff) {
    typedef __attribute__((ext_vector_type(4))) unsigned u32x4_t;
    const u32x4_t v = __builtin_amdgcn_raw_buffer_load_b128(r, voff, soff, 0);
    return __builtin_bit_cast(u16x8, v);
}
__device__ __forceinline__ u16x8 buf_load16_nt(buf_rsrc r, unsigned voff, unsigned soff) {
    typedef __attribute__((ext_vector_type(4))) unsigned u32x4_t;
    const u32x4_t v = __builtin_amdgcn_raw_buffer_load_b128(r, voff, soff, 2);
    return __builtin_bit_cast(u16x8, v);
}
__device__ __forceinline__ void buf_load16_lds(buf_rsrc r, void* lds_wave_base, unsigned voff, unsigned soff) {
    __builtin_amdgcn_raw_ptr_buffer_load_lds(r, (__attribute__((address_space(3))) void*)lds_wave_base, 16, voff, soff, 0, 0);
}
#else
struct buf_rsrc {
    const char* p;
    unsigned bytes;
};
__device__ __forceinline__ buf_rsrc make_buf_rsrc(const void* p, unsigned bytes) { return buf_rsrc{(const char*)p, bytes}; }
__device__ __forceinline__ u16x8 buf_load16(buf_rsrc r, unsigned voff, unsigned soff) {
    u16x8 v = {0, 0, 0, 0, 0, 0, 0, 0};
    if (voff < r.bytes && (unsigned long long)voff + 16 <= r.bytes) v = *reinterpret_cast<const u16x8*>(r.p + voff + soff);
    return v;
}
__device__ __forceinline__ u16x8 buf_load16_nt(buf_rsrc r, unsigned voff, unsigned soff) { return buf_load16(r, voff, soff); }
#if !defined(__HIP__)
__device__ __forceinline__ void buf_load16_lds(buf_rsrc r, void* lds_wave_base, unsigned voff, unsigned soff) {
    *reinterpret_cast<u16x8*>(static_cast<char*>(lds_wave_base) + (threadIdx.x & 63) * 16) = buf_load16(r, voff, soff);
}
#else
__device__ __forceinline__ void buf_load16_lds(buf_rsrc, void*, unsigned, unsigned) {}
#endif
#endif

typedef __attribute__((ext_vector_type(4))) short s16x4_t;
#if defined(__HIP_DEVICE_COMPILE__)
__device__ __forceinline__ s16x4_t lds_read_tr16(const unsigned short* p) {
    return __builtin_amdgcn_ds_read_tr16_b64_v4i16((__attribute__((address_space(3))) s16x4_t*)p);
}
__device__ __forceinline__ s16x4_t lds_read_tr16_async(const unsigned short* p) {
    s16x4_t v;
    const unsigned a = (unsigned)(size_t)(__attribute__((address_space(3))) const unsigned short*)p;
    asm volatile("ds_read_b64_tr_b16 %0, %1" : "=v"(v) : "v"(a) : "memory");
    return v;
}
template <int OFF>
__device__ __forceinline__ s16x4_t lds_read_tr16_async_off(const unsigned char* p) {
    static_assert(OFF >= 0 && OFF < 65536, "16-bit offset field");
    s16x4_t v;
    const unsigned a = (unsigned)(size_t)(__attribute__((address_space(3))) const unsigned char*)p;
    asm volatile("ds_read_b64_tr_b16 %0, %1 offset:%2" : "=v"(v) : "v"(a), "n"(OFF) : "memory");
    return v;
}
#elif defined(__HIP__)
__device__ __forceinline__ s16x4_t lds_read_tr16(const unsigned short*) { return s16x4_t{0, 0, 0, 0}; }
__device__ __forceinline__ s16x4_t lds_read_tr16_async(const unsigned short*) { return s16x4_t{0, 0, 0, 0}; }
template <int OFF>
__device__ __forceinline__ s16x4_t lds_read_tr16_async_off(const unsigned char*) { return s16x4_t{0, 0, 0, 0}; }
#else
__device__ __forceinline__ s16x4_t lds_read_tr16(const unsigned short* p) {
    const int lane = threadIdx.x & 63, base = lane & ~15, c = lane & 15;
    s16x4_t r;
    for (int e = 0; e < 4; ++e) {
        const unsigned short* q = __shfl(p, base + 4 * e + (c >> 2), 64);
        r[e] = (short)q[c & 3];
    }
    return r;
}
__device__ __forceinline__ s16x4_t lds_read_tr16_async(const unsigned short* p) { return lds_read_tr16(p); }
template <int OFF>
__device__ __forceinline__ s16x4_t lds_read_tr16_async_off(const unsigned char* p) { return lds_read_tr16(reinterpret_cast<const unsigned short*>(p + OFF)); }
#endif

#if defined(__HIP_DEVICE_COMPILE__)
#define LP_OPAQUE(x) asm volatile("" : "+v"(x))
#else
#define LP_OPAQUE(x) asm volatile("" : "+r"(x))
#endif

#ifndef LP_UNIFORM_LOADS
#define LP_UNIFORM_LOADS 1
#endif
#if defined(__HIP_DEVICE_COMPILE__) && LP_UNIFORM_LOADS
template <typename T>
using uniform_ptr = const __attribute__((address_space(4))) T*;
template <typename T>
__device__ __forceinline__ uniform_ptr<T> as_uniform(const T* p) {
    return (uniform_ptr<T>)(unsigned long long)p;
}
#else
template <typename T>
using uniform_ptr = const T*;
template <typename T>
__host__ __device__ inline uniform_ptr<T> as_uniform(const T* p) {
    return p;
}
#endif

__device__ __forceinline__ float wave_sum(float v) {
#pragma unroll
    for (int m = 32; m >= 1; m >>= 1) v += __shfl_xor(v, m, 64);
    return v;
}

__device__ __forceinline__ float wave_max(float v) {
#pragma unroll
    for (int m = 32; m >= 1; m >>= 1) v = fmaxf(v, __shfl_xor(v, m, 64));
    return v;
}

template <int NW>
__device__ __forceinline__ float block_sum(float v, float* scratch) {
    v = wave_sum(v);
    const int lane = threadIdx.x & 63, wave = threadIdx.x >> 6;
    if (lane == 0) scratch[wave] = v;
    __syncthreads();
    float t = 0.f;
#pragma unroll
    for (int i = 0; i < NW; ++i) t += scratch[i];
    __syncthreads();
    return t;
}

template <int NW>
__device__ __forceinline__ float block_max(float v, float* scratch) {
    v = wave_max(v);
    const int lane = threadIdx.x & 63, wave = threadIdx.x >> 6;
    if (lane == 0) scratch[wave] = v;
    __syncthreads();
    float t = scratch[0];
#pragma unroll
    for (int i = 1; i < NW; ++i) t = fmaxf(t, scratch[i]);
    __syncthreads();
    return t;
}

constexpr long long kFxPoison = 5LL << 60;
constexpr long long kFxPoisonSeen = 1LL << 59;
__device__ __forceinline__ void fx_add(lp_fxsum* p, float t) {
    double td = (double)t;
    if (!(fabs(td) <= 0x1p127 * 2.0)) {
        atomicMax(&p->lo, kFxPoison);
        return;
    }
    td = fmin(fmax(td, -0x1p49), 0x1p49);
    const double h = rint(td * 0x1p12);
    const long long hi = (long long)h;
    const long long lo = (long long)rint((td - h * 0x1p-12) * 0x1p60);
    atomicAdd(reinterpret_cast<unsigned long long*>(&p->hi), (unsigned long long)hi);
    atomicAdd(reinterpret_cast<unsigned long long*>(&p->lo), (unsigned long long)lo);
}
__device__ __forceinline__ float fx_value(const lp_fxsum* p) {
    const long long lo = p->lo;
    if (lo >= kFxPoisonSeen || lo <= -kFxPoisonSeen) return __int_as_float(0x7fc00000);
    return (float)((double)p->hi * 0x1p-12 + (double)lo * 0x1p-60);
}

struct LpSwitches {
    int conv_pipe, conv_halo, conv_res2d, infer_pipe, gemm_pipe, wgrad_pipe, wgrad_nb, stem_2d, stem_wgrad_nb, pool_v2, conv_max_wgs, bn_bwd_wgs_per_cu;
};
const LpSwitches& lp_switches();

inline int launch_status() {
    hipError_t e = hipGetLastError();
    return e == hipSuccess ? LP_OK : (int)e;
}

}

#define LP_REQUIRE(cond)                    \
    do {                                    \
        if (!(cond)) return LP_ERR_ARGUMENT; \
    } while (0)
```

Before: 4674 frames/s.

## Keep the 1x1 conv weight panel resident in LDS across pipe-kernel tiles

Adds a weight-resident variant of the pipelined conv kernel for 1x1 stride-1 trunk convolutions. The whole K x BN weight panel is loaded into a 64 KiB LDS panel once per output-column block and reused for every pixel tile, so the ring stages only stream activations. This removes the repeated per-stage weight loads. It is enabled by default for dgrad and for shapes with N >= K, and adds a swizzled readback layout for the data-gradient epilogue. In exchange, the larger LDS footprint can lower occupancy, and a full panel reload with a vmcnt(0) wait happens whenever a block's column tile changes.

After: 4787 frames/s (median of 6 runs). 1.02x the previous value.

```diff
diff --git a/include/lp_hip.h b/include/lp_hip.h
--- a/include/lp_hip.h
+++ b/include/lp_hip.h
@@ -20,7 +20,7 @@
 
 enum { LP_TF_NONE = 0, LP_TF_SINGLE = 1, LP_TF_PER_FRAME = 2, LP_TF_PER_VIEW = 3 };
 
-#define LP_HIP_ABI_VERSION 148
+#define LP_HIP_ABI_VERSION 149
 int lp_version(void);
 const char* lp_strerror(int code);
 
@@ -119,6 +119,7 @@
 #define LP_CONV_KERNEL_WGRAD_NB 9
 #define LP_CONV_KERNEL_RES2D 5
 int lp_conv_last_kernel(void);
+int lp_conv_last_resident(void);
 
 int lp_conv_fwd(const void* x, const void* w, const lp_conv_geom* geom, const float* bias, void* out_bf16, float* out_f32, int ldo,
                 int n_store, lp_stream_t stream);
diff --git a/lightning-pose_amd/_lib.py b/lightning-pose_amd/_lib.py
--- a/lightning-pose_amd/_lib.py
+++ b/lightning-pose_amd/_lib.py
@@ -67,7 +67,7 @@
 AUG_ELASTIC_MAX_RADIUS = 20
 TF_NONE, TF_SINGLE, TF_PER_FRAME, TF_PER_VIEW = 0, 1, 2, 3
 
-ABI_VERSION = 148
+ABI_VERSION = 149
 
 _P, _I, _F, _L, _Z = C.c_void_p, C.c_int, C.c_float, C.c_long, C.c_size_t
 
@@ -112,6 +112,7 @@
     "lp_attn_dscores": (_I, [_P, _I, _P, _I, _P, _P, _I, C.c_longlong, C.c_longlong, C.c_float, _P, _I, _I, _I, _I, C.POINTER(GemmBatch), _P]),
     "lp_conv_fwd_bn": (_I, [_P, _P, C.POINTER(ConvGeom), _P, C.POINTER(BnFuse), _P]),
     "lp_conv_last_kernel": (_I, []),
+    "lp_conv_last_resident": (_I, []),
     "lp_stem_fwd_bn": (_I, [_P, _P, C.POINTER(ConvGeom), _P, C.POINTER(BnFuse), _P]),
     "lp_conv_dgrad_bn": (_I, [_P, _P, C.POINTER(ConvGeom), _P, _P, _P, C.POINTER(BnFuse), _P]),
     "lp_bn_fold": (_I, [_P, _P, _P, _P, _P, _F, _I, _I, _P, _P, _P]),
diff --git a/lightning-pose_amd/csrc/api.hip b/lightning-pose_amd/csrc/api.hip
--- a/lightning-pose_amd/csrc/api.hip
+++ b/lightning-pose_amd/csrc/api.hip
@@ -15,6 +15,7 @@
     LpSwitches s;
     s.conv_pipe = env_int("LP_CONV_PIPE", 1);
     s.conv_halo = env_int("LP_CONV_HALO", 1);
+    s.pipe_wres = env_int("LP_PIPE_WRES", 1);
     s.conv_res2d = env_int("LP_CONV_RES2D", 1);
     s.infer_pipe = env_int("LP_INFER_PIPE", 1);
     s.gemm_pipe = env_int("LP_GEMM_PIPE", 1);
diff --git a/lightning-pose_amd/csrc/conv.hip b/lightning-pose_amd/csrc/conv.hip
--- a/lightning-pose_amd/csrc/conv.hip
+++ b/lightning-pose_amd/csrc/conv.hip
@@ -946,12 +946,14 @@
 }
 
 static thread_local int g_last_conv_kernel = LP_CONV_KERNEL_IGEMM;
+static thread_local int g_last_conv_resident = 0;
 
 struct ConvRoute {
     int kernel;
     int bn;
     int mode;
     int ek;
+    bool wres;
 };
 constexpr int kNoKernel = -1;
 
@@ -1034,6 +1036,14 @@
     return (p.ek == kEkNone || p.ek == kEkInfer || p.ek == kEkZ) && halo_shape_ok(p.g, p.M, conv_ck(p), p.N > 64 ? 384 : 512);
 }
 
+static bool admits_wres(const ConvProblem& p) {
+    if (!(p.ek == kEkNone || p.ek == kEkZ || p.ek == kEkAZB || p.ek == kEkPlain || p.ek == kEkPB)) return false;
+    if (p.g.R != 1 || p.g.S != 1 || p.g.stride != 1 || p.g.pad != 0 || p.lat.hstep != 1 || p.lat.wstep != 1 || p.K != conv_ck(p)) return false;
+    return (long long)p.K * (p.N > 64 ? 128 : 64) * 2 <= 64 * 1024;
+}
+
+static bool wres_tuned(const ConvProblem& p) { return p.mode == kModeDgrad || p.N >= p.K; }
+
 static bool admits_res2d(const ConvProblem& p) {
     if (!res2d_shape_ok(p.g, conv_ck(p), p.N)) return false;
     if (p.mode == kModeInfer) return p.ep.addend == nullptr;
@@ -1042,11 +1052,14 @@
 
 static ConvRoute route_conv(const ConvProblem& p, const LpSwitches& sw) {
     const bool pipe = sw.conv_pipe != 0 && (p.gate == nullptr || sw.*p.gate != 0);
-    if (p.mode == kModeStem) return ConvRoute{pipe && stem2d_shape_ok(p.g) ? LP_CONV_KERNEL_RES2D : LP_CONV_KERNEL_IGEMM, 64, p.mode, p.ek};
-    if (pipe && sw.conv_res2d != 0 && admits_res2d(p)) return ConvRoute{LP_CONV_KERNEL_RES2D, 64, p.mode, p.ek};
-    if (pipe && admits_pipe(p))
-        return ConvRoute{sw.conv_halo != 0 && admits_halo(p) ? LP_CONV_KERNEL_PIPE_HALO : LP_CONV_KERNEL_PIPE, p.N > 64 ? 128 : 64, p.mode, p.ek};
-    return ConvRoute{p.igemm_form ? LP_CONV_KERNEL_IGEMM : kNoKernel, p.igemm_cols > 64 ? 128 : 64, p.mode, p.ek};
+    if (p.mode == kModeStem) return ConvRoute{pipe && stem2d_shape_ok(p.g) ? LP_CONV_KERNEL_RES2D : LP_CONV_KERNEL_IGEMM, 64, p.mode, p.ek, false};
+    if (pipe && sw.conv_res2d != 0 && admits_res2d(p)) return ConvRoute{LP_CONV_KERNEL_RES2D, 64, p.mode, p.ek, false};
+    if (pipe && admits_pipe(p)) {
+        if (sw.conv_halo != 0 && admits_halo(p)) return ConvRoute{LP_CONV_KERNEL_PIPE_HALO, p.N > 64 ? 128 : 64, p.mode, p.ek, false};
+        const bool wres = sw.pipe_wres != 0 && admits_wres(p) && (sw.pipe_wres == 2 || wres_tuned(p));
+        return ConvRoute{LP_CONV_KERNEL_PIPE, p.N > 64 ? 128 : 64, p.mode, p.ek, wres};
+    }
+    return ConvRoute{p.igemm_form ? LP_CONV_KERNEL_IGEMM : kNoKernel, p.igemm_cols > 64 ? 128 : 64, p.mode, p.ek, false};
 }
 
 static int conv_max_wgs(int per_cu) {
@@ -1096,7 +1109,7 @@
                        (unsigned)(2ull * g.B * g.Hi * g.Wi * 4), g.B, g.Ho, g.Wo, ntiles, p.ep);
 }
 
-template <int BN, int MODE, int EK, bool HALO = false>
+template <int BN, int MODE, int EK, bool HALO = false, bool WRES = false>
 static void launch_pipe(const ConvProblem& p, hipStream_t st) {
     const ConvGeom& g = p.g;
     const int tm = (p.M + kPM - 1) / kPM, tn = p.N / BN, ntiles = tm * tn;
@@ -1105,7 +1118,7 @@
     const unsigned x_bytes = (unsigned)(2ull * (MODE == kModeDgrad ? (size_t)g.B * g.Ho * g.Wo * g.Co : (size_t)g.B * g.Hi * g.Wi * g.Ci));
     const unsigned w_bytes = (unsigned)(2ull * (size_t)p.N * g.R * g.S * ck);
     const HaloDivs hd{make_fastdiv(g.Hi), make_fastdiv(g.Wi + 2), make_fastdiv(g.Hi + 2)};
-    hipLaunchKernelGGL((conv_pipe_kernel<BN, MODE, EK, HALO>), dim3(grid), dim3(512), 0, st, (const unsigned short*)p.x, (const unsigned short*)p.w,
+    hipLaunchKernelGGL((conv_pipe_kernel<BN, MODE, EK, HALO, WRES>), dim3(grid), dim3(512), 0, st, (const unsigned short*)p.x, (const unsigned short*)p.w,
                        x_bytes, w_bytes, g, p.lat, make_fastdiv(p.lat.nh * p.lat.nw), make_fastdiv(p.lat.nw), p.M, p.N, p.K, tn, ntiles, p.ep, hd);
 }
 
@@ -1119,6 +1132,15 @@
             default: return launch_igemm<BN, kModeAttn>(p, st);
         }
     }
+    if (r.wres) {
+        switch (r.ek) {
+            case kEkNone: return launch_pipe<BN, kModeFwd, kEkNone, false, true>(p, st);
+            case kEkZ: return launch_pipe<BN, kModeDgrad, kEkZ, false, true>(p, st);
+            case kEkAZB: return launch_pipe<BN, kModeDgrad, kEkAZB, false, true>(p, st);
+            case kEkPB: return launch_pipe<BN, kModeDgrad, kEkPB, false, true>(p, st);
+            default: return launch_pipe<BN, kModeDgrad, kEkPlain, false, true>(p, st);
+        }
+    }
     const bool halo = r.kernel == LP_CONV_KERNEL_PIPE_HALO;
     switch (r.ek) {
         case kEkNone: return halo ? launch_pipe<BN, kModeFwd, kEkNone, true>(p, st) : launch_pipe<BN, kModeFwd, kEkNone>(p, st);
@@ -1132,6 +1154,7 @@
 
 static void launch_conv(const ConvRoute& r, const ConvProblem& p, hipStream_t st) {
     g_last_conv_kernel = r.kernel;
+    g_last_conv_resident = r.wres ? 1 : 0;
     if (r.kernel == LP_CONV_KERNEL_RES2D) {
         switch (r.mode) {
             case kModeStem: return launch_stem2d(p, st);
@@ -1411,6 +1434,7 @@
 }
 
 extern "C" int lp_conv_last_kernel(void) { return lp::g_last_conv_kernel; }
+extern "C" int lp_conv_last_resident(void) { return lp::g_last_conv_resident; }
 
 extern "C" int lp_conv_fwd(const void* x, const void* w, const lp_conv_geom* geom, const float* bias, void* out_bf16, float* out_f32,
                            int ldo, int n_store, lp_stream_t stream) {
@@ -1615,6 +1639,7 @@
     hipStream_t st = (hipStream_t)stream;
     float* ws = (float*)workspace;
     g_last_conv_kernel = p.kernel;
+    g_last_conv_resident = 0;
     if (p.kernel == LP_CONV_KERNEL_WGRAD_NB) {
         if (p.bn == 128) launch_wgrad_nb<128>(p, x, dy, g, dw, ws, st);
         else launch_wgrad_nb<64>(p, x, dy, g, dw, ws, st);
@@ -1717,6 +1742,7 @@
     hipStream_t st = (hipStream_t)stream;
     float* ws = (float*)workspace;
     g_last_conv_kernel = p.kernel;
+    g_last_conv_resident = 0;
     if (p.kernel == LP_CONV_KERNEL_STEM_WGRAD_NB)
         hipLaunchKernelGGL(stem_wgrad_nb_kernel, dim3(p.split), dim3(256), 0, st, xs, dys, (unsigned)(8ull * g.B * g.Hi * g.Wi),
                            (unsigned)(128ull * M), g, M, p.per, dhw, dwo, ws);
diff --git a/lightning-pose_amd/csrc/conv_pipe.h b/lightning-pose_amd/csrc/conv_pipe.h
--- a/lightning-pose_amd/csrc/conv_pipe.h
+++ b/lightning-pose_amd/csrc/conv_pipe.h
@@ -45,7 +45,7 @@
     FastDiv h, wp, hp;
 };
 
-template <int BN, int MODE, int EK, bool HALO = false>
+template <int BN, int MODE, int EK, bool HALO = false, bool WRES = false>
 __global__ __launch_bounds__(512) void conv_pipe_kernel(const unsigned short* __restrict__ X, const unsigned short* __restrict__ Wt,
                                                         unsigned x_bytes, unsigned w_bytes, ConvGeom g, Lattice lat, FastDiv div_img,
                                                         FastDiv div_row, int M, int N, int K, int tiles_n, int ntiles, ConvEpilogue ep,
@@ -53,15 +53,19 @@
     static_assert((MODE == kModeFwd && (EK == kEkNone || EK == kEkInfer || EK == kEkGeluBwd || EK == kEkGeluFwd)) ||
                       (MODE == kModeDgrad && EK != kEkNone && EK != kEkInfer && EK != kEkGeluBwd && EK != kEkGeluFwd),
                   "trunk convolutions only");
+    static_assert(!(HALO && WRES), "the weight-resident form is the per-tap ring's");
+    static_assert(!WRES || EK == kEkNone || EK == kEkZ || EK == kEkAZB || EK == kEkPlain || EK == kEkPB, "weight-resident form: the training store passes");
     constexpr int NT = BN / 64;
     constexpr int NBL = BN / 64;
-    constexpr int kStageA = HALO ? 0 : kPM * kPRowB, kStageB = BN * kPRowB, kStage = kStageA + kStageB;
+    constexpr int kStageA = HALO ? 0 : kPM * kPRowB, kStageB = BN * kPRowB, kStage = kStageA + (WRES ? 0 : kStageB);
     constexpr int kHaloRows = BN == 64 ? 512 : 384;
     constexpr int kHaloB = kHaloRows * kPRowB, NA = kHaloRows / 64;
     constexpr int NST = HALO ? LP_HALO_STAGES : 3;
     static_assert(NST == 3 || NST == 4, "ring depth");
-    __shared__ __attribute__((aligned(16))) unsigned char smem[NST * kStage + (HALO ? 2 * kHaloB : 0)];
+    constexpr int kPanelB = WRES ? 64 * 1024 : 0;
+    __shared__ __attribute__((aligned(16))) unsigned char smem[NST * kStage + (HALO ? 2 * kHaloB : 0) + kPanelB];
     unsigned char* const halo0 = smem + NST * kStage;
+    unsigned char* const panel0 = smem + NST * kStage;
 
     const int tid = threadIdx.x, lane = tid & 63;
     const int wave = __builtin_amdgcn_readfirstlane(tid >> 6);
@@ -90,7 +94,7 @@
     auto setup = [&](int vt) {
         if (vt >= ntiles) {
 #pragma unroll
-            for (int i = 0; i < 4; ++i) vmask[i] = 0u, rowoff[i] = 0u;
+            for (int i = 0; i < 4; ++i) vmask[i] = 0u, rowoff[i] = 0u, voff[i] = ~0u;
 #pragma unroll
             for (int i = 0; i < NBL; ++i) wrow[i] = ~0u;
             tir = tis = tc = 0;
@@ -117,6 +121,10 @@
             }
             const int oy = halved ? (py[i] >> 1) : py[i], ox = halved ? (px[i] >> 1) : px[i];
             rowoff[i] = (unsigned)(((b * src_h + oy) * src_w + ox) * ck + lchunk * 8) * 2u;
+            if (WRES) {
+                voff[i] = pv ? rowoff[i] : ~0u;
+                continue;
+            }
             unsigned mask = 0;
             if (pv) {
                 for (int ir = 0; ir < lat.nr; ++ir)
@@ -137,7 +145,7 @@
             vmask[i] = mask;
         }
 #pragma unroll
-        for (int i = 0; i < NBL; ++i) wrow[i] = (unsigned)((n0 + lrow + 64 * i) * ldw + lchunk * 8) * 2u;
+        for (int i = 0; i < (WRES ? 0 : NBL); ++i) wrow[i] = (unsigned)((n0 + lrow + 64 * i) * ldw + lchunk * 8) * 2u;
         tir = tis = tc = 0;
     };
 
@@ -153,7 +161,7 @@
             if (++tir == 9) tir = 0, tc += kBK;
             return;
         }
-        if (tc == 0) {
+        if (!WRES && tc == 0) {
             const int tr = lat.r0 + lat.rstep * tir, ts = lat.s0 + lat.sstep * tis;
             const int qr = halved ? (tr >> 1) : tr, qs = halved ? (ts >> 1) : ts;
             const unsigned tapoff_b = (unsigned)(((MODE == kModeDgrad) ? -(qr * src_w + qs) : (qr * src_w + qs)) * ck) * 2u;
@@ -166,9 +174,11 @@
             }
         }
         is_soff_a = (unsigned)tc * 2u;
-        is_soff_b = wtap + is_soff_a;
-#pragma unroll
-        for (int i = 0; i < NBL; ++i) is_w[i] = wrow[i];
+        if (!WRES) {
+            is_soff_b = wtap + is_soff_a;
+#pragma unroll
+            for (int i = 0; i < NBL; ++i) is_w[i] = wrow[i];
+        }
         is_dst = smem + st * kStage + wave * (8 * kPRowB);
         tc += kBK;
         if (tc >= ck) {
@@ -194,8 +204,15 @@
     auto load_step = [&](int st) {
         prep_step(st);
 #pragma unroll
-        for (int i = 0; i < (HALO ? NBL : 4 + NBL); ++i) issue_load(i);
+        for (int i = 0; i < (HALO ? NBL : WRES ? 4 : 4 + NBL); ++i) issue_load(i);
         advance_tile();
+    };
+    auto panel_load = [&](const int n0) {
+        for (int kt = 0; kt < KT; ++kt)
+#pragma unroll
+            for (int i = 0; i < NBL; ++i)
+                buf_load16_lds(rsrc_w, panel0 + kt * kStageB + (i * 64 + wave * 8) * kPRowB, (unsigned)((n0 + lrow + 64 * i) * ldw + lchunk * 8) * 2u,
+                               (unsigned)(kt * (kBK * 2)));
     };
 
     const int hW = g.Wi, hH = g.Hi, hWp = g.Wi + 2, hHp = g.Hi + 2;
@@ -249,7 +266,7 @@
 #pragma unroll
     for (int kk = 0; kk < 4; ++kk) koff[kk] = (unsigned)(((kk * 2 + fg) ^ fsw) * 16);
     const unsigned a_row = (unsigned)((wm * 64 + fr) * kPRowB);
-    const unsigned b_row = (unsigned)(kStageA + (wn * (NT * 32) + fr) * kPRowB);
+    const unsigned b_row = (unsigned)((WRES ? 0 : kStageA) + (wn * (NT * 32) + fr) * kPRowB);
 
     f32x16 acc[2][NT];
 #ifndef LP_PIPE_FRAG_SETS
@@ -257,8 +274,9 @@
 #endif
     constexpr int NS = (MODE == kModeFwd) ? LP_PIPE_FRAG_SETS : 2;
     int ploc[2] = {0, 0}, uloc[2] = {0, 0}, mh_buf = 0, mh_tap = 0;
-    auto mma_stage = [&](int st, const bool spread) {
+    auto mma_stage = [&](int st, const bool spread, const int mkt) {
         const unsigned char* sb = smem + st * kStage;
+        const unsigned char* sbw = WRES ? panel0 + mkt * kStageB : sb;
         bf16x8 a[NS][2], b[NS][NT];
         const unsigned char* ha[2] = {smem, smem};
         unsigned hk[2][4] = {};
@@ -282,7 +300,7 @@
             }
 #pragma unroll
             for (int nt = 0; nt < NT; ++nt)
-                b[set][nt] = __builtin_bit_cast(bf16x8, *reinterpret_cast<const u16x8*>(sb + b_row + nt * (32 * kPRowB) + koff[kk]));
+                b[set][nt] = __builtin_bit_cast(bf16x8, *reinterpret_cast<const u16x8*>(sbw + b_row + nt * (32 * kPRowB) + koff[kk]));
         };
 #pragma unroll
         for (int kk = 0; kk < NS - 1; ++kk) fetch(kk, kk);
@@ -313,6 +331,8 @@
                 } else if (kk == 2) {
                     if (NBL == 2) issue_load(1);
                 }
+            } else if (spread && WRES) {
+                issue_load(kk);
             } else if (spread) {
                 constexpr int NL = 4 + NBL;
                 if (kk == 0) {
@@ -381,6 +401,7 @@
         constexpr bool gelub = EK == kEkGeluBwd;
         constexpr bool kPad = LP_FWD_CORNER_PAD != 0;
         constexpr int ROWB = NT * 64 + (kPad ? 16 : 0);
+        static_assert(!(WRES && kPad), "the padded corner does not fit a pixel-only stage");
         unsigned char* stg = stg_all + wave * (32 * ROWB);
         const int wkey = kPad ? 0 : NT == 2 ? (fr & 15) : ((fr >> 1) & 7);
         u16x8 radd[2][32 / RP] = {};
@@ -512,8 +533,12 @@
         }
     };
     auto rb_process = [&](const ReadBack& rb, const int mt, unsigned char* stg_all, const int m0, const int n0) {
-        constexpr int ROWF = NT * 128 + 16;
+        constexpr bool kSwz = WRES && NT == 2;
+        constexpr int ROWF = kSwz ? 256 : NT * 128 + 16;
+        static_assert(!WRES || 8 * 16 * ROWF <= kStage, "the data gradient's corners fit the stage consumed last");
         unsigned char* stg = stg_all + wave * (16 * ROWF);
+        const unsigned wxor = (unsigned)((fr & 15) * 256 + ((fg ^ (fr & 15)) << 4));
+        const unsigned rxor = (unsigned)(prow * 256 + (((2 * pc) ^ prow) << 4));
 #pragma unroll
         for (int h = 0; h < 2; ++h) {
             if ((fr >> 4) == h) {
@@ -522,15 +547,22 @@
 #pragma unroll
                     for (int j = 0; j < 4; ++j) {
                         const f32x4 p4 = {acc[mt][nt][4 * j], acc[mt][nt][4 * j + 1], acc[mt][nt][4 * j + 2], acc[mt][nt][4 * j + 3]};
-                        *reinterpret_cast<f32x4*>(stg + (fr & 15) * ROWF + (nt * 32 + 8 * j + 4 * fg) * 4) = p4;
+                        if (kSwz) *reinterpret_cast<f32x4*>(stg + (wxor ^ (unsigned)((nt * 8 + 2 * j) << 4))) = p4;
+                        else *reinterpret_cast<f32x4*>(stg + (fr & 15) * ROWF + (nt * 32 + 8 * j + 4 * fg) * 4) = p4;
                     }
             }
             __builtin_amdgcn_wave_barrier();
             f32x4 lo_[PH], hi_[PH];
 #pragma unroll
             for (int ps = 0; ps < PH; ++ps) {
-                lo_[ps] = *reinterpret_cast<const f32x4*>(stg + (ps * RP + prow) * ROWF + pc * 32);
-                hi_[ps] = *reinterpret_cast<const f32x4*>(stg + (ps * RP + prow) * ROWF + pc * 32 + 16);
+                if (kSwz) {
+                    const unsigned o = (unsigned)(ps * RP * ROWF) + (rxor ^ (unsigned)(((ps * RP) & 15) << 4));
+                    lo_[ps] = *reinterpret_cast<const f32x4*>(stg + o);
+                    hi_[ps] = *reinterpret_cast<const f32x4*>(stg + (o ^ 16u));
+                } else {
+                    lo_[ps] = *reinterpret_cast<const f32x4*>(stg + (ps * RP + prow) * ROWF + pc * 32);
+                    hi_[ps] = *reinterpret_cast<const f32x4*>(stg + (ps * RP + prow) * ROWF + pc * 32 + 16);
+                }
             }
             __builtin_amdgcn_wave_barrier();
 #pragma unroll
@@ -591,6 +623,12 @@
         halo_advance();
     }
     setup(ld_vt);
+    int pn0 = -1;
+    if (WRES && (int)blockIdx.x < ntiles) {
+        const int tile = xcd_remap(blockIdx.x, ntiles);
+        pn0 = (tile - (tile / tiles_n) * tiles_n) * BN;
+        panel_load(pn0);
+    }
 #pragma unroll
     for (int st = 0; st < NST - 1; ++st) load_step(st);
     int cur = 0;
@@ -610,6 +648,11 @@
                 uloc[mt] = ploc[mt] - 2 * (padded_row(mc) - rr0);
             }
         }
+        if (WRES && n0 != pn0) {
+            panel_load(n0);
+            pn0 = n0;
+            LP_WAIT_VM(0);
+        }
         if (n0 != st_n0 || seg_off != st_seg_off) {
             if (want_stats) stats_flush(reinterpret_cast<float*>(free_lds()));
             st_n0 = n0;
@@ -637,6 +680,7 @@
             else if (HALO && NST == 4) LP_WAIT_VM(2);
             else if (HALO && NBL == 2) LP_WAIT_VM(2);
             else if (HALO) LP_WAIT_VM(1);
+            else if (WRES) LP_WAIT_VM(4);
             else if (NBL == 2) LP_WAIT_VM(6);
             else LP_WAIT_VM(5);
             LP_RAW_BARRIER();
@@ -644,11 +688,11 @@
             const int nxt = cur == 0 ? NST - 1 : cur - 1;
             if (kSpread || HALO) {
                 prep_step(nxt);
-                mma_stage(cur, true);
+                mma_stage(cur, true, kt);
                 advance_tile();
             } else {
                 load_step(nxt);
-                mma_stage(cur, false);
+                mma_stage(cur, false, kt);
             }
             cur = cur == NST - 1 ? 0 : cur + 1;
             if (HALO && ++mh_tap == 9) {
diff --git a/lightning-pose_amd/csrc/lp_common.h b/lightning-pose_amd/csrc/lp_common.h
--- a/lightning-pose_amd/csrc/lp_common.h
+++ b/lightning-pose_amd/csrc/lp_common.h
@@ -270,7 +270,7 @@
 }
 
 struct LpSwitches {
-    int conv_pipe, conv_halo, conv_res2d, infer_pipe, gemm_pipe, wgrad_pipe, wgrad_nb, stem_2d, stem_wgrad_nb, pool_v2, conv_max_wgs, bn_bwd_wgs_per_cu;
+    int conv_pipe, conv_halo, pipe_wres, conv_res2d, infer_pipe, gemm_pipe, wgrad_pipe, wgrad_nb, stem_2d, stem_wgrad_nb, pool_v2, conv_max_wgs, bn_bwd_wgs_per_cu;
 };
 const LpSwitches& lp_switches();
 
diff --git a/profiles/pipe_wres_table.py b/profiles/pipe_wres_table.py
--- /dev/null
+++ b/profiles/pipe_wres_table.py
@@ -0,0 +1,65 @@
+import json
+import sys
+
+from layer_table import short
+
+PLANES = {1: 64, 2: 128, 3: 256, 4: 512}
+
+
+def shape(li: int, first: bool, conv: str, kind: str):
+    p = PLANES[li]
+    cin = (64 if li == 1 else 2 * p) if first else 4 * p
+    ci, co, stride = {"c1": (cin, p, 1), "c3": (p, 4 * p, 1), "down": (cin, 4 * p, 1 if li == 1 else 2)}[conv]
+    return (ci, co, stride) if kind == "fwd" else (co, ci, stride)
+
+
+def admits(K: int, N: int, stride: int) -> bool:
+    return stride == 1 and K * (128 if N > 64 else 64) * 2 <= 64 * 1024
+
+
+def classes(path: str) -> dict:
+    out: dict = {}
+    for tag, _gflop, us, _mb, layer in json.load(open(path)):
+        if not layer.startswith("backbone.") or "wgrad" in tag:
+            continue
+        name = short(layer)
+        if name == "stem" or name.split(".")[2] == "c2":
+            continue
+        li, blk, conv = name.split(".")
+        key = (int(li[1:]), blk == "0", conv, "dgrad" if "dgrad" in tag else "fwd")
+        rec = out.setdefault(key, [0.0, 0])
+        rec[0] += us
+        rec[1] += 1
+    return out
+
+
+def main():
+    runs: dict = {"parent": [], "ring": [], "resident": []}
+    for arg in sys.argv[1:]:
+        label, path = arg.split("=", 1)
+        runs[label].append(classes(path))
+    keys = sorted(runs["ring"][0])
+    cols = [(lab, i) for lab in ("parent", "ring", "resident") for i in range(len(runs[lab]))]
+    print("us per launch class and step (sum over the class's launches; n = launches)")
+    print(f"{'class':22s} {'K':>4s} {'N':>5s} {'n':>3s} | " + " ".join(f"{lab[:6] + str(i + 1):>9s}" for lab, i in cols) + " | ring spread   gain   verdict")
+    tot = {"ring": 0.0, "resident": 0.0, "tuned": 0.0}
+    for key in keys:
+        li, first, conv, kind = key
+        K, N, stride = shape(li, first, conv, kind)
+        vals = [runs[lab][i].get(key, [0.0, 0])[0] for lab, i in cols]
+        ring = [r[key][0] for r in runs["ring"]]
+        res = [r[key][0] for r in runs["resident"]]
+        spread = max(ring) - min(ring)
+        gain = sum(ring) / len(ring) - sum(res) / len(res)
+        ok = admits(K, N, stride)
+        verdict = "not eligible" if not ok else "FASTER" if gain > spread else "not faster"
+        tot["ring"] += sum(ring) / len(ring)
+        tot["resident"] += sum(res) / len(res)
+        tot["tuned"] += sum(res) / len(res) if verdict == "FASTER" else sum(ring) / len(ring)
+        name = f"l{li}.{'0' if first else 'x'}.{conv} {kind}"
+        print(f"{name:22s} {K:4d} {N:5d} {runs['ring'][0][key][1]:3d} | " + " ".join(f"{v:9.1f}" for v in vals) + f" | {spread:11.1f} {gain:6.1f}   {verdict}")
+    print(f"totals (ms per step): ring {tot['ring'] / 1e3:.3f}  resident everywhere {tot['resident'] / 1e3:.3f}  resident where FASTER {tot['tuned'] / 1e3:.3f}")
+
+
+if __name__ == "__main__":
+    main()
```
